# pkmtum/generative-physics-informed-pde

Measured on AMD Instinct MI355X. Metric: ELBO training-step samples/sec (64x64 grids), higher is better.
Workload: dtype f32; 1 GPU; BASELINE config 2/3: c64 grid, B_u=256 unlabeled + N_s=32 labeled per GPU, ROM 8x8, fused native step; global_batch=288, grid=64, parallelism=dp1, graph=True, graph_mode=streams, steps_per_replay=4, world=1, bn=replica

## Files before the change

generative-physics-informed-pde_amd/csrc/conv.hip:

```cpp
#include "common.h"
#include <stdlib.h>
#include <stdio.h>
#include <algorithm>
#include <string.h>
#include <string>
#include <utility>
#include <vector>
#include <atomic>
#include <mutex>

using namespace gpi;

#pragma clang fp contract(on)

namespace {

constexpr int HALO = 4;

__device__ __attribute__((aligned(256))) float g_zero_page[64];

struct Div {
    uint32_t m, one;
};

Div mkdiv(int d) {
    Div v;
    v.one = d == 1;
    v.m = d == 1 ? 0u : (uint32_t)(((1ull << 32) + (uint64_t)d - 1) / (uint64_t)d);
    return v;
}

__device__ __forceinline__ int dq(int e, Div v) { return v.one ? e : (int)__umulhi((uint32_t)e, v.m); }

#ifdef GPI_PHASE_TIMING
__device__ __attribute__((visibility("hidden"))) unsigned long long g_phase[4096 * 16];
__device__ __attribute__((visibility("hidden"))) unsigned long long g_rt[4096 * 2];
#define PHASE(i)                                                                                     \
    do {                                                                                             \
        if (threadIdx.x == 0) g_phase[(blockIdx.x & 4095) * 16 + (i)] = __builtin_amdgcn_s_memtime(); \
    } while (0)
#define RTSTAMP(i)                                                                                 \
    do {                                                                                           \
        if (threadIdx.x == 0) {                                                                    \
            g_rt[(blockIdx.x & 4095) * 2 + (i)] = __builtin_amdgcn_s_memrealtime();                \
            if ((i) == 0)                                                                          \
                g_phase[(blockIdx.x & 4095) * 16 + 15] =                                           \
                    (unsigned long long)__builtin_amdgcn_s_getreg((31 << 11) | 4) |                \
                    ((unsigned long long)__builtin_amdgcn_s_getreg((31 << 11) | 20) << 32);        \
        }                                                                                          \
    } while (0)
#else
#define PHASE(i) \
    do {         \
    } while (0)
#define RTSTAMP(i) \
    do {           \
    } while (0)
#endif

__host__ __device__ inline int fdiv2(int x) { return x >= 0 ? x / 2 : -((-x + 1) / 2); }
__host__ __device__ inline int cdiv2(int x) { return -fdiv2(-x); }
__host__ __device__ inline int pad256(int n) { return (n + 255) & ~255; }

#ifndef GPI_FWD_WAVE_ATOMICS
#define GPI_FWD_WAVE_ATOMICS 0
#endif
#ifndef GPI_FWD_WVGPR
#define GPI_FWD_WVGPR 1
#endif

struct ConvGeom {
    int th, tiles, nblocks;
    int rh, P;
    int gh, PG;
    int ph;
    const float* zero;
    int zreg;
    int npx;
    int cg;
    int fuse;
    int vsum;
    int vshift;
    int ucls;
    int lsum;
    int split;
    int xcd;
    int grid;
    int nfull, half_b, htiles;
    struct Alt {
        int th, rh, gh, ph, zreg, in_sq, in_sr, in_sc, g_sq, g_sr, g_sc;
        Div d_in4, d_g4, d_tp;
    } ha;
    int alt;
    uint32_t* sig;
    const int64_t* sig_epoch;
    int in_sq, in_sr, in_sc;
    int g_sq, g_sr, g_sc;
    Div d_in4, d_P4, d_g4, d_PG4, d_cin, d_cout, d_win, d_tp, d_wout, d_w2;
#ifdef GPI_PHASE_TIMING
    int dbg;
#endif
};

#ifdef GPI_PHASE_TIMING
#define SKIP(G, bit) (((G).dbg & (bit)) != 0)
#else
#define SKIP(G, bit) false
#endif

__host__ __device__ inline void in_rows(int k, int s, int up, int pad, int o0, int t, int& i0, int& len) {
    if (up) {
        i0 = fdiv2(o0 - pad);
        len = fdiv2(o0 + t - 1 - pad + k - 1) - i0 + 1;
    } else {
        i0 = o0 * s - pad;
        len = (t - 1) * s + k;
    }
}

__host__ __device__ inline void g_rows(int k, int s, int pad, int o0, int t, int& g0, int& len) {
    if (s == 2) {
        g0 = cdiv2(2 * o0 + pad - k + 1);
        len = fdiv2(2 * o0 + 2 * t - 1 + pad) - g0 + 1;
    } else {
        g0 = o0 + pad - (k - 1);
        len = t + k - 1;
    }
}

__host__ __device__ inline void owned_rows(int s, int up, int o0, int t, int& p0, int& len) {
    if (up) { p0 = o0 / 2; len = t / 2; }
    else if (s == 2) { p0 = 2 * o0; len = 2 * t; }
    else { p0 = o0; len = t; }
}

constexpr int ZREG = 3;

int env_int(const char* name, int dflt) {
    const char* v = getenv(name);
    return v && *v ? atoi(v) : dflt;
}


bool conv_geom(const gpi_conv_desc& d, const gpi_groups& g, ConvGeom& G, bool fwd, bool fuse = false) {
    if (g.n_groups < 1 || g.n_groups > GPI_MAX_GROUPS) return false;
    if (d.cin < 1 || d.cin > GPI_MAX_CIN || d.cout < 1 || d.cout > GPI_MAX_COUT) return false;
    if (d.k != 1 && d.k != 3 && d.k != 5 && d.k != 7) return false;
    if (d.pad > HALO || (d.w_in & 3) || (d.w_out & 3) || d.w_out > 256) return false;
    if (d.upsample) {
        if (d.stride != 1 || d.h_out != 2 * d.h_in || d.w_out != 2 * d.w_in || d.pad != d.k / 2) return false;
    } else if (d.stride == 2) {
        if (d.h_in != 2 * d.h_out || d.w_in != 2 * d.w_out || d.pad != d.k / 2) return false;
    } else if (d.stride == 1) {
        if (d.h_in != d.h_out || d.w_in != d.w_out || d.pad != d.k / 2) return false;
    } else {
        return false;
    }
    const int B = g.start[g.n_groups] - g.start[0];
    if (g.start[0] != 0 || B <= 0) return false;
    static const int t_fwd = env_int("GPI_TILE_FWD", 512), t_fwd64 = env_int("GPI_TILE_FWD64", 1024),
                     t_bwd = env_int("GPI_TILE_BWD", 512), t_s2 = env_int("GPI_TILE_S2", 128),
                     t_s2brows = env_int("GPI_TILE_S2BROWS", 4), t_s2c1 = env_int("GPI_TILE_S2C1", 512),
                     t_bwdup = env_int("GPI_TILE_BWDUP", 1024), t_bwdrows = env_int("GPI_TILE_BWDROWS", 8),
                     t_fwdrows = env_int("GPI_TILE_FWDROWS", 8), t_fuse = env_int("GPI_TILE_FUSE", 1024);
    static const int t_fwdup32 = env_int("GPI_TILE_FWDUP32", 16), t_bwdups = env_int("GPI_TILE_BWDUPS", 16),
                     t_bwd32k3 = env_int("GPI_TILE_BWD32K3", 16), t_s2c1f = env_int("GPI_TILE_S2C1F", 512),
                     t_fwdwide = env_int("GPI_TILE_FWDWIDE", 8);
    const int target =
        d.stride == 2 ? (d.cin == 1 ? (fwd ? t_s2c1f : t_s2c1) : (fwd ? t_s2 : t_s2brows * d.w_out))
        : fwd ? (d.w_out >= 64 ? t_fwd64
                               : (d.w_out >= 32 ? (d.upsample && d.w_out == 32 ? t_fwdup32
                                                   : (d.k == 3 && d.cin >= 10 && d.w_out == 32 ? t_fwdwide : t_fwdrows)) * d.w_out
                                                : t_fwd))
              : (d.upsample ? (d.w_out >= 32 ? t_bwdup / 64 * min(d.w_out, 64) : t_bwdups * d.w_out)
                            : (d.w_out >= 64 ? t_bwd
                                             : (d.w_out == 32 && d.k == 3 && d.cin <= 8 ? t_bwd32k3 : t_bwdrows) * d.w_out));
    const bool loss_bwd = !fwd && (d.epilogue == GPI_EPI_GAUSS_LOSS || d.epilogue == GPI_EPI_GAUSS_EXP_LOSS);
    G.th = (loss_bwd ? t_fuse : target) / d.w_out;
    if (G.th < 1) G.th = 1;
    if (G.th > d.h_out) G.th = d.h_out;
    if (fwd && d.stride == 1 && !d.upsample) {
        for (;;) {
            int y0, rh;
            in_rows(d.k, 1, 0, d.pad, 0, G.th, y0, rh);
            const int half = G.th / 2;
            if (4 * d.cin * rh * (d.w_in + 2 * HALO) <= 28 * 1024 || half < 1 || d.h_out % half) break;
            G.th = half;
        }
    }
    if (d.upsample && G.th < 2) G.th = 2;
    while (d.h_out % G.th) --G.th;
    if (d.upsample && (G.th & 1)) return false;
    G.tiles = d.h_out / G.th;
    G.nblocks = B * G.tiles;
    int i0;
    in_rows(d.k, d.stride, d.upsample, d.pad, 0, G.th, i0, G.rh);
    if (d.upsample) G.rh += 1;
    if (fuse) G.rh += d.k - 1;
    G.P = d.w_in + 2 * HALO;
    g_rows(d.k, d.stride, d.pad, 0, G.th, i0, G.gh);
    G.PG = d.w_out + 2 * HALO;
    owned_rows(d.stride, d.upsample, 0, G.th, i0, G.ph);
    const uint64_t lim = 1ull << 32;
    const uint64_t in4 = (uint64_t)G.rh * G.P / 4, g4 = (uint64_t)G.gh * G.PG / 4;
    const uint64_t ein = in4 * d.cin, eg = g4 * d.cout, eo = (uint64_t)G.ph * d.w_in;
    if (ein * in4 >= lim || in4 * (G.P / 4) >= lim || eg * g4 >= lim || g4 * (G.PG / 4) >= lim ||
        eo * d.w_in >= lim || 256ull * G.th * d.w_out >= lim)
        return false;
    G.zero = nullptr;
    static const int npx_cap = env_int("GPI_FWD_NPX", 4);
    G.npx = 1;
    if (fwd) {
        const int tp = G.th * d.w_out;
        while (2 * G.npx <= npx_cap && tp >= 256 * 2 * G.npx && d.w_out % (2 * G.npx) == 0) G.npx *= 2;
    }
    G.cg = 1;
    if (fwd && G.npx == 1 && d.epilogue != GPI_EPI_GAUSS_LOSS && d.epilogue != GPI_EPI_GAUSS_EXP_LOSS) {
        static const int cg_on = env_int("GPI_FWD_CG", 1);
        const int tp = G.th * d.w_out;
        if (cg_on && tp <= 128 && 256 % tp == 0 && !d.upsample && d.k <= 3) G.cg = std::min(256 / tp, d.cin);
    }
    G.zreg = (!fwd && d.gout_mode == 0 && (int64_t)d.cout * G.gh * (G.PG / 4) <= (int64_t)ZREG * 256) ? 1 : 0;
    G.split = 0;
    G.fuse = fuse ? 1 : 0;
    G.lsum = 0;
    G.vsum = 0;
    {
        static const int vshift = env_int("GPI_VWG_SHIFT", 1);
        G.vshift = (!fwd && vshift && d.k == 7 && d.stride == 2 && d.cin == 1 && d.cout <= 8) ? 1 : 0;
        static const int ucls = env_int("GPI_UP_ROWCLS", 1);
        G.ucls = (!fwd && ucls && d.upsample && d.k == 3 && d.pad == 1 && (2 * d.cin + 15) / 16 < (3 * d.cin + 15) / 16)
                     ? 1 : 0;
    }
    G.xcd = 0;
    G.alt = 0;
    G.grid = 0;
    G.sig = nullptr;
    G.sig_epoch = nullptr;
#ifdef GPI_PHASE_TIMING
    static const int dbg = env_int("GPI_DBG_SKIP", 0);
    G.dbg = dbg;
#endif
    {
        const int P4 = G.P / 4, pl = G.rh * P4, Q4 = G.PG / 4, gl = G.gh * Q4;
        G.in_sq = 256 / pl;
        G.in_sr = (256 % pl) / P4;
        G.in_sc = (256 % pl) % P4;
        G.g_sq = 256 / gl;
        G.g_sr = (256 % gl) / Q4;
        G.g_sc = (256 % gl) % Q4;
    }
    G.d_in4 = mkdiv((int)in4);
    G.d_P4 = mkdiv(G.P / 4);
    G.d_g4 = mkdiv((int)g4);
    G.d_PG4 = mkdiv(G.PG / 4);
    G.d_cin = mkdiv(d.cin);
    G.d_cout = mkdiv(d.cout);
    G.d_win = mkdiv(d.w_in);
    G.d_tp = mkdiv(G.th * d.w_out);
    G.d_wout = mkdiv(d.w_out);
    G.d_w2 = mkdiv(d.w_in >= 2 ? d.w_in / 2 : 1);
    G.nfull = G.nblocks;
    G.half_b = B;
    G.htiles = 0;
    G.ha = ConvGeom::Alt{G.th, G.rh, G.gh, G.ph, G.zreg, G.in_sq, G.in_sr, G.in_sc, G.g_sq, G.g_sr, G.g_sc,
                         G.d_in4, G.d_g4, G.d_tp};
    static const int half_tiles = env_int("GPI_HALF_TILES", 2);
    const int tot = B * G.tiles, base = tot & ~255;
    static const int half_fwd = env_int("GPI_HALF_FWD", 1);
    if (half_tiles && (fwd ? half_fwd && half_tiles > 1 && G.cg == 1 : (half_tiles > 1 || loss_bwd)) &&
        (G.th & 1) == 0 && base > 0 && tot != base && tot <= 5 * 256 && base % G.tiles == 0) {
        ConvGeom::Alt& a = G.ha;
        a.th = G.th / 2;
        int y0;
        in_rows(d.k, d.stride, d.upsample, d.pad, 0, a.th, y0, a.rh);
        if (d.upsample) a.rh += 1;
        if (fuse) a.rh += d.k - 1;
        g_rows(d.k, d.stride, d.pad, 0, a.th, y0, a.gh);
        owned_rows(d.stride, d.upsample, 0, a.th, y0, a.ph);
        a.zreg = (!fwd && d.gout_mode == 0 && (int64_t)d.cout * a.gh * (G.PG / 4) <= (int64_t)ZREG * 256) ? 1 : 0;
        const int P4 = G.P / 4, pl = a.rh * P4, Q4 = G.PG / 4, gq = a.gh * Q4;
        a.in_sq = 256 / pl;
        a.in_sr = (256 % pl) / P4;
        a.in_sc = (256 % pl) % P4;
        a.g_sq = 256 / gq;
        a.g_sr = (256 % gq) / Q4;
        a.g_sc = (256 % gq) % Q4;
        a.d_in4 = mkdiv(pl);
        a.d_g4 = mkdiv(gq);
        a.d_tp = mkdiv(a.th * d.w_out);
        const bool ok = d.gin_off < 0 || (((a.ph * d.w_in) & 15) == 0 && (d.stride != 2 || (a.ph & 1) == 0));
        if (!ok) a = ConvGeom::Alt{G.th, G.rh, G.gh, G.ph, G.zreg, G.in_sq, G.in_sr, G.in_sc, G.g_sq, G.g_sr, G.g_sc,
                                   G.d_in4, G.d_g4, G.d_tp};
        else {
        G.half_b = base / G.tiles;
        G.nfull = base;
        G.htiles = 2 * G.tiles;
        G.nblocks = base + (B - G.half_b) * G.htiles;
        }
    }
    return true;
}

#define SHAPE_D(X) X(k) X(stride) X(pad) X(upsample) X(cin) X(cout) X(h_in) X(w_in) X(h_out) X(w_out) \
    X(in_bn) X(gout_mode) X(epilogue) X(gin_accumulate)
#define SHAPE_G(X) X(th) X(tiles) X(rh) X(P) X(gh) X(PG) X(ph) X(zreg) X(npx) X(cg) X(fuse) X(vsum) X(vshift) \
    X(ucls) X(lsum) X(split) X(xcd) X(alt) X(in_sq) X(in_sr) X(in_sc) X(g_sq) X(g_sr) X(g_sc)
#define SHAPE_GD(X) X(d_in4) X(d_P4) X(d_g4) X(d_PG4) X(d_cin) X(d_cout) X(d_win) X(d_tp) X(d_wout) X(d_w2)
#define SHAPE_A(X) X(th) X(rh) X(gh) X(ph) X(zreg) X(in_sq) X(in_sr) X(in_sc) X(g_sq) X(g_sr) X(g_sc)
#define SHAPE_AD(X) X(d_in4) X(d_g4) X(d_tp)

struct ShapeC {
    int fwd, fusek, half, exf, v3, cp, npxk, upk, has_gin, drop, wout, ext_in;
#define F(n) int D_##n;
    SHAPE_D(F)
#undef F
#define F(n) int G_##n;
    SHAPE_G(F)
#undef F
#define F(n) int M_##n, O_##n;
    SHAPE_GD(F)
#undef F
#define F(n) int A_##n;
    SHAPE_A(F)
#undef F
#define F(n) int AM_##n, AO_##n;
    SHAPE_AD(F)
#undef F
};

#if defined(GPI_SHAPES_FILE)
#include GPI_SHAPES_FILE
#elif __has_include("conv_shapes.h")
#include "conv_shapes.h"
#endif
#ifndef GPI_CONV_SHAPE_LIST
#define GPI_CONV_SHAPE_LIST
#define GPI_CONV_SHAPE_COUNT 0
#endif
constexpr ShapeC kShapes[GPI_CONV_SHAPE_COUNT + 1] = {GPI_CONV_SHAPE_LIST ShapeC{}};
constexpr int kNumShapes = GPI_CONV_SHAPE_COUNT;
#ifndef GPI_CONV_SHAPE_BOUNDS
#define GPI_CONV_SHAPE_BOUNDS {0, GPI_CONV_SHAPE_COUNT, GPI_CONV_SHAPE_COUNT, GPI_CONV_SHAPE_COUNT, GPI_CONV_SHAPE_COUNT}
#endif
constexpr int kBounds[5] = GPI_CONV_SHAPE_BOUNDS;
#ifndef GPI_CONV_SHAPE_PART
#define GPI_CONV_SHAPE_PART 0
#endif

#ifndef GPI_FUSE_FOLD
#define GPI_FUSE_FOLD 6
#endif

template <int SHP>
__device__ __forceinline__ void fold_shape(gpi_conv_desc& d, ConvGeom& G) {
    if constexpr (SHP >= 0) {
        constexpr ShapeC s = kShapes[SHP];
        constexpr int fm = s.fusek ? GPI_FUSE_FOLD : 7;
        if constexpr (fm & 1) {
#define F(n) d.n = s.D_##n;
        SHAPE_D(F)
#undef F
        }
        if constexpr (fm & 2) {
#define F(n) G.n = s.G_##n;
        SHAPE_G(F)
#undef F
#define F(n) G.ha.n = s.A_##n;
        SHAPE_A(F)
#undef F
        }
        if constexpr (fm & 4) {
#define F(n) G.n = Div{(uint32_t)s.M_##n, (uint32_t)s.O_##n};
        SHAPE_GD(F)
#undef F
#define F(n) G.ha.n = Div{(uint32_t)s.AM_##n, (uint32_t)s.AO_##n};
        SHAPE_AD(F)
#undef F
        }
        if constexpr (s.has_gin) __builtin_assume(d.gin_off >= 0); else d.gin_off = -1;
        if constexpr (s.drop) __builtin_assume(d.drop_off >= 0); else d.drop_off = -1;
        if constexpr (s.wout) __builtin_assume(d.wpart_off >= 0); else d.wpart_off = -1;
        if constexpr (s.ext_in) d.in_off = -1; else __builtin_assume(d.in_off >= 0);
        if constexpr (!s.half) G.nfull = 0x7fffffff;
    }
}

__device__ __forceinline__ void glds4(const float* g, float* lds_wave_base) {
    __builtin_amdgcn_global_load_lds((const __attribute__((address_space(1))) void*)g,
                                     (__attribute__((address_space(3))) void*)lds_wave_base, 4, 0, 0);
}

__device__ __forceinline__ void glds16(const float* g, float* lds_wave_base) {
    __builtin_amdgcn_global_load_lds((const __attribute__((address_space(1))) void*)g,
                                     (__attribute__((address_space(3))) void*)lds_wave_base, 16, 0, 0);
}

template <typename Src>
__device__ __forceinline__ void stage(float* dst, int total, const float* zero, Src src) {
    const int wb = threadIdx.x & ~63;
    for (int e0 = 0; e0 < total; e0 += 256) {
        if (e0 + wb < total) {
            const int e = e0 + (int)threadIdx.x;
            const float* p = e < total ? src(e) : nullptr;
            glds4(p ? p : zero, dst + e0 + wb);
        }
    }
}

#ifndef GPI_STAGE_SEL
#define GPI_STAGE_SEL 1
#endif
struct ChunkIter {
    int q, r, c4;
    __device__ __forceinline__ void init(int e, int plane4, int P4, Div d_q4, Div d_p4) {
        q = dq(e, d_q4);
        const int rem = e - q * plane4;
        r = dq(rem, d_p4);
        c4 = rem - r * P4;
    }
    __device__ __forceinline__ void step(int sq, int sr, int sc, int P4, int nr) {
        c4 += sc;
        if (c4 >= P4) { c4 -= P4; ++r; }
        r += sr;
        if (r >= nr) { r -= nr; ++q; }
        q += sq;
    }
};

constexpr int IMG_MARGIN4 = 16;
__host__ __device__ inline int img_floats(int nq, int nr, int P) { return pad256(4 * (nq * nr * (P / 4) + IMG_MARGIN4)); }

template <typename Plane>
__device__ __forceinline__ void stage_img(float* dst, int nq, int nr, int P, Div d_q4, Div d_p4, int sq, int sr,
                                          int sc, int r0, int h, int w, const float* zero, Plane plane) {
    const int P4 = P >> 2, plane4 = nr * P4, total = nq * plane4 + IMG_MARGIN4;
    const int wb = threadIdx.x & ~63;
    const int c4lo = HALO / 4, c4hi = HALO / 4 + w / 4;
    ChunkIter it;
    it.init(threadIdx.x, plane4, P4, d_q4, d_p4);
    for (int e0 = 0; e0 < total; e0 += 256) {
        if (e0 + wb < total) {
            const int row = r0 + it.r;
            const bool ok = it.q < nq && row >= 0 && row < h && it.c4 >= c4lo && it.c4 < c4hi;
#if GPI_STAGE_SEL
            const float* pv = plane(it.q) + row * w + 4 * (it.c4 - c4lo);
            asm volatile("" : "+v"(pv));
            const float* p = ok ? pv : zero;
#else
            const float* p = ok ? plane(it.q) + row * w + 4 * (it.c4 - c4lo) : zero;
#endif
            glds16(p, dst + 4 * (e0 + wb));
        }
        it.step(sq, sr, sc, P4, nr);
    }
}

constexpr int STAT_HALF = GPI_REPLICAS / 2;
struct StatLoad {
    double v[STAT_HALF];
    double* out;
};

__device__ __forceinline__ void stat_issue(const gpi_stat* stats, int64_t n_stats, int grp, int64_t sa, int na,
                                           double* da, int64_t sb, int nb, double* db, const float* zero, StatLoad& L) {
    const int t = threadIdx.x, k = t & 3, h = (t >> 2) & 1, ch = t >> 3;
    const double* p = (const double*)zero;
    int64_t step = 0;
    L.out = nullptr;
    const int64_t rstride = n_stats * GPI_MAX_GROUPS * 4;
    const gpi_stat* sg = stats + (int64_t)grp * n_stats;
    if (ch < na) {
        p = &sg[sa + ch].sum + k + h * STAT_HALF * rstride;
        step = rstride;
        L.out = da + 4 * ch + k;
    } else if (ch - na < nb) {
        p = &sg[sb + ch - na].sum + k + h * STAT_HALF * rstride;
        step = rstride;
        L.out = db + 4 * (ch - na) + k;
    }
    const auto g = (const __attribute__((address_space(1))) double*)p;
#pragma unroll
    for (int r = 0; r < STAT_HALF; ++r) L.v[r] = g[r * step];
}

__device__ __forceinline__ void stat_finish(StatLoad& L) {
    double s0 = 0.0, s1 = 0.0;
#pragma unroll
    for (int r = 0; r < STAT_HALF; r += 2) {
        s0 += L.v[r];
        s1 += L.v[r + 1];
    }
    double s = s0 + s1;
    s += __shfl_xor(s, 4, 64);
    if (L.out && !(threadIdx.x & 4)) *L.out = s;
}

__device__ __forceinline__ gpi_stat* stat_slot(const gpi_codec_ctx& c, int64_t stat, int grp) {
    const int r = blockIdx.x % GPI_REPLICAS;
    return c.stats + ((int64_t)r * GPI_MAX_GROUPS + grp) * c.n_stats + stat;
}

__device__ __forceinline__ void mean_invstd(const double* s4, double n, float eps, float& mean, float& invstd) {
    const double m = s4[0] / n;
    double var = fma(-m, m, s4[1] / n);
    if (var < 0.0) var = 0.0;
    mean = (float)m;
    invstd = (float)(1.0 / sqrt(var + (double)eps));
}

template <int CP>
__device__ __forceinline__ void fma_vec(float (&acc)[CP], const float* w, float v) {
    if constexpr (CP % 4 == 0) {
#pragma unroll
        for (int q = 0; q < CP / 4; ++q) {
            const float4 w4 = reinterpret_cast<const float4*>(w)[q];
            acc[4 * q + 0] = fmaf(w4.x, v, acc[4 * q + 0]);
            acc[4 * q + 1] = fmaf(w4.y, v, acc[4 * q + 1]);
            acc[4 * q + 2] = fmaf(w4.z, v, acc[4 * q + 2]);
            acc[4 * q + 3] = fmaf(w4.w, v, acc[4 * q + 3]);
        }
    } else {
#pragma unroll
        for (int q = 0; q < CP / 2; ++q) {
            const float2 w2 = reinterpret_cast<const float2*>(w)[q];
            acc[2 * q + 0] = fmaf(w2.x, v, acc[2 * q + 0]);
            acc[2 * q + 1] = fmaf(w2.y, v, acc[2 * q + 1]);
        }
    }
}

template <typename T>
__device__ __forceinline__ T pin(T v) {
    asm volatile("" : "+s"(v));
    return v;
}

typedef float f32x4 __attribute__((ext_vector_type(4)));
typedef float f32x2 __attribute__((ext_vector_type(2)));

template <int NBYTES>
__device__ __forceinline__ void touch_kernargs() {
    const __attribute__((address_space(4))) uint32_t* ka =
        (const __attribute__((address_space(4))) uint32_t*)__builtin_amdgcn_kernarg_segment_ptr();
    constexpr int NL = (NBYTES + 63) / 64;
    uint32_t x[NL];
#pragma unroll
    for (int i = 0; i < NL; ++i) x[i] = ka[16 * i];
#pragma unroll
    for (int i = 0; i < NL; ++i) asm volatile("" : : "s"(x[i]));
}
constexpr int CONV_KARG_BYTES = (int)(sizeof(gpi_conv_desc) + sizeof(gpi_codec_ctx) + sizeof(ConvGeom) + 16);

__device__ __forceinline__ void entry_signal(const ConvGeom& G) {
    if (G.sig && blockIdx.x == 0 && threadIdx.x == 0)
        __hip_atomic_fetch_add(G.sig, 1u, __ATOMIC_RELAXED, __HIP_MEMORY_SCOPE_AGENT);
}

template <typename T>
__device__ __forceinline__ const __attribute__((address_space(1))) T* as_gld(const T* p) {
    return (const __attribute__((address_space(1))) T*)p;
}
template <typename T>
__device__ __forceinline__ __attribute__((address_space(1))) T* as_gst(T* p) {
    return (__attribute__((address_space(1))) T*)p;
}

struct TileIdx {
    int b, oy0, grp, gsz;
};

__device__ __forceinline__ int logical_block(const ConvGeom& G) {
    const int b = blockIdx.x;
    if (!G.xcd) return b;
    const int q = G.grid >> 3, r = G.grid & 7, x = b & 7;
    return x * q + min(x, r) + (b >> 3);
}

__device__ __forceinline__ TileIdx tile_of(const ConvGeom& G, const gpi_groups& g, int tile = -1) {
    if (tile < 0) tile = logical_block(G);
    TileIdx t;
    if (tile < G.nfull) {
        t.b = tile / G.tiles;
        t.oy0 = (tile - t.b * G.tiles) * G.th;
    } else {
        const int u = tile - G.nfull, q = u / G.htiles;
        t.b = G.half_b + q;
        t.oy0 = (u - q * G.htiles) * G.ha.th;
    }
    t.grp = group_of(g, t.b);
    t.gsz = karg_sel(g.start, t.grp + 1) - karg_sel(g.start, t.grp);
    return t;
}

__device__ __forceinline__ const float* input_base(const gpi_conv_desc& d, const gpi_codec_ctx& c, int b) {
    const int HWi = d.h_in * d.w_in;
    if (d.in_off >= 0) return c.ws + d.in_off + ((int64_t)b * d.in_ctot + d.in_c0) * HWi;
    return c.ext_in + (int64_t)(c.ext_idx ? c.ext_idx[b] : b) * c.ext_stride + (int64_t)d.in_c0 * HWi;
}

__device__ __forceinline__ void activate_img(float* img, const ConvGeom& G, const gpi_conv_desc& d, int iy0,
                                             const float* sc, const float* sh) {
    const int P4 = G.P >> 2, plane4 = G.rh * P4, total = d.cin * plane4;
    const int c4lo = HALO / 4, c4hi = HALO / 4 + d.w_in / 4;
    float4* im4 = reinterpret_cast<float4*>(img);
    ChunkIter it;
    it.init(threadIdx.x, plane4, P4, G.d_in4, G.d_P4);
    for (int e0 = threadIdx.x; e0 < total; e0 += 512) {
        float4 v[2];
        bool ok[2];
        int ci[2];
#pragma unroll
        for (int u = 0; u < 2; ++u) {
            const int row = iy0 + it.r;
            ok[u] = e0 + 256 * u < total && row >= 0 && row < d.h_in && it.c4 >= c4lo && it.c4 < c4hi;
            ci[u] = it.q;
            if (ok[u]) v[u] = im4[e0 + 256 * u];
            it.step(G.in_sq, G.in_sr, G.in_sc, P4, G.rh);
        }
#pragma unroll
        for (int u = 0; u < 2; ++u) {
            if (ok[u]) {
                const float a = sc[ci[u]], b = sh[ci[u]];
                float4 o;
                o.x = fmaxf(fmaf(v[u].x, a, b), 0.f);
                o.y = fmaxf(fmaf(v[u].y, a, b), 0.f);
                o.z = fmaxf(fmaf(v[u].z, a, b), 0.f);
                o.w = fmaxf(fmaf(v[u].w, a, b), 0.f);
                im4[e0 + 256 * u] = o;
            }
        }
    }
}

template <int NW, int OFF>
__device__ __forceinline__ void lds_window(const float* p, float (&win)[NW]) {
    constexpr int NCH = (OFF + NW + 3) / 4;
    const float4* q = reinterpret_cast<const float4*>(p - OFF);
    float buf[4 * NCH];
#pragma unroll
    for (int c = 0; c < NCH; ++c) {
        const float4 v = q[c];
        buf[4 * c] = v.x;
        buf[4 * c + 1] = v.y;
        buf[4 * c + 2] = v.z;
        buf[4 * c + 3] = v.w;
    }
#pragma unroll
    for (int t = 0; t < NW; ++t) win[t] = buf[OFF + t];
}

#ifndef GPI_PLAIN_STORES
__device__ __forceinline__ void st2(float* p, f32x2 v) {
    __hip_atomic_store((__attribute__((address_space(1))) uint64_t*)p, __builtin_bit_cast(uint64_t, v),
                       __ATOMIC_RELAXED, __HIP_MEMORY_SCOPE_AGENT);
}
__device__ __forceinline__ void st4(float* p, f32x4 v) {
    asm volatile("global_store_dwordx4 %0, %1, off sc1\n\ts_nop 1" : : "v"(p), "v"(v));
}
__device__ __forceinline__ void st1(float* p, float v) {
    __hip_atomic_store((__attribute__((address_space(1))) float*)p, v, __ATOMIC_RELAXED, __HIP_MEMORY_SCOPE_AGENT);
}
#else
__device__ __forceinline__ void st4(float* p, f32x4 v) { *as_gst((f32x4*)p) = v; }
__device__ __forceinline__ void st2(float* p, f32x2 v) { *as_gst((f32x2*)p) = v; }
__device__ __forceinline__ void st1(float* p, float v) { *as_gst(p) = v; }
#endif

template <int NPX>
__device__ __forceinline__ void store_px(float* p, const float (&v)[NPX]) {
    if constexpr (NPX == 4) {
        st4(p, f32x4{v[0], v[1], v[2], v[3]});
    } else if constexpr (NPX == 2) {
        st2(p, f32x2{v[0], v[1]});
    } else {
#pragma unroll
        for (int q = 0; q < NPX; ++q) st1(p + q, v[q]);
    }
}

constexpr int FWD_HDR = 8 * GPI_MAX_CIN + 2 * GPI_MAX_CIN + 64 + 16 + 8;

template <int K, int S, int UP, int CP, int NPX, bool HALF = false, int SHP = -1>
__global__ __launch_bounds__(256) __attribute__((amdgpu_waves_per_eu(NPX == 0 ? 1 : 5))) void conv_fwd_kernel(gpi_conv_desc d, gpi_codec_ctx c, ConvGeom G) {
    fold_shape<SHP>(d, G);
    touch_kernargs<CONV_KARG_BYTES>();
    entry_signal(G);
    if (SKIP(G, 16)) return;
    ConvGeom Gt_;
    if constexpr (HALF) {
        Gt_ = G;
        if (logical_block(G) >= G.nfull) {
            const ConvGeom::Alt& a = G.ha;
            Gt_.th = a.th; Gt_.rh = a.rh; Gt_.in_sq = a.in_sq; Gt_.in_sr = a.in_sr; Gt_.in_sc = a.in_sc;
            Gt_.d_in4 = a.d_in4; Gt_.d_tp = a.d_tp;
        }
    }
    const ConvGeom& Gt = HALF ? Gt_ : G;
    constexpr int KK = K * K;
    extern __shared__ __attribute__((aligned(16))) float smem[];
    double* gst = (double*)smem;
    float* sc = smem + 8 * GPI_MAX_CIN;
    float* sh = sc + GPI_MAX_CIN;
    float* scratch = sh + GPI_MAX_CIN;
    float* red = scratch + 64;
    float* dsl = red + 16;
    float* wT = smem + pad256(FWD_HDR);
    const int nw = d.cin * KK * CP;
    float* img = wT + pad256(nw);

    const int tid = threadIdx.x;
    RTSTAMP(0);
    PHASE(0);
    float* const ws = pin(c.ws);
    const float* const params = pin(c.params);
    const float* const zero = pin(Gt.zero);
    const int64_t w_off = pin(d.w_off);
    const TileIdx T = tile_of(Gt, c.groups);
    const int HWi = d.h_in * d.w_in, HWo = d.h_out * d.w_out;
    const float* ib = input_base(d, c, T.b);
    const bool drop = d.drop_off >= 0;
    PHASE(1);

    stage(wT, nw, zero, [&](int e) -> const float* {
        const int co = e % CP, r = e / CP;
        return co < d.cout ? params + w_off + (int64_t)co * d.cin * KK + r : nullptr;
    });
    int iy0, rh_;
    in_rows(K, S, UP, d.pad, T.oy0, Gt.th, iy0, rh_);
    stage_img(img, d.cin, Gt.rh, Gt.P, Gt.d_in4, Gt.d_P4, Gt.in_sq, Gt.in_sr, Gt.in_sc, iy0, d.h_in, d.w_in, zero,
              [&](int q) -> const float* { return ib + (int64_t)q * HWi; });
    float dsv = 1.f;
    if (drop && tid >= 64 && tid < 64 + d.cout) dsv = *as_gld(ws + d.drop_off + (int64_t)T.b * d.cout + (tid - 64));
    if (d.in_bn) {
        float gam = 0.f, bet = 0.f;
        if (tid < d.cin) {
            gam = *as_gld(params + d.gamma_off + tid);
            bet = *as_gld(params + d.beta_off + tid);
        }
        StatLoad L;
        stat_issue(c.stats, c.n_stats, T.grp, d.in_stat, d.cin, gst, 0, 0, nullptr, zero, L);
        stat_finish(L);
        __syncthreads();
        if (SKIP(G, 8) || SKIP(G, 32)) return;
        PHASE(2);
        if (tid < d.cin) {
            float mean, inv;
            mean_invstd(gst + 4 * tid, (double)T.gsz * HWi, c.bn_eps, mean, inv);
            sc[tid] = gam * inv;
            sh[tid] = fmaf(-(mean * gam), inv, bet);
        }
        __syncthreads();
        activate_img(img, Gt, d, iy0, sc, sh);
    }
    if (drop && tid >= 64 && tid < 64 + d.cout) dsl[tid - 64] = dsv;
    __syncthreads();
    PHASE(4);

    const int tp = Gt.th * d.w_out;
    float Lv = 0.f;
    float vst[2 * CP];
#pragma unroll
    for (int q = 0; q < 2 * CP; ++q) vst[q] = 0.f;
    const bool gauss = d.epilogue == GPI_EPI_GAUSS_LOSS || d.epilogue == GPI_EPI_GAUSS_EXP_LOSS;
    if constexpr (NPX > 1) {
        constexpr int PADK = K / 2;
        constexpr int NW = UP ? ((NPX - 1 + K - 1 + (PADK & 1)) >> 1) + 1 : (NPX - 1) * S + K;
        const int ng = tp / NPX;
        for (int gbase = 0; gbase < ng; gbase += 256) {
            const int g = gbase + tid;
            const bool active = g < ng;
            const int ty = dq(g * NPX, Gt.d_wout), x0 = g * NPX - ty * d.w_out;
            const int oy = T.oy0 + ty;
            float acc[NPX][CP];
#pragma unroll
            for (int p = 0; p < NPX; ++p)
#pragma unroll
                for (int co = 0; co < CP; ++co) acc[p][co] = 0.f;
            if (active && !SKIP(G, 64)) {
                const int plane = Gt.rh * Gt.P;
                const int cb = UP ? fdiv2(x0 - PADK) + HALO : x0 * S - PADK + HALO;
                for (int ci = 0; ci < d.cin; ++ci) {
                    const float* tci = img + ci * plane + cb;
                    const float* wci = wT + ci * KK * CP;
#pragma unroll
                    for (int ky = 0; ky < K; ++ky) {
                        const int ry = UP ? (fdiv2(oy - PADK + ky) - iy0) : (ty * S + ky);
                        const float* trow = tci + ry * Gt.P;
                        float win[NW];
                        if constexpr (!UP && (NPX * S) % 4 == 0) {
                            lds_window<NW, (HALO - PADK) & 3>(trow, win);
                        } else {
#pragma unroll
                            for (int t = 0; t < NW; ++t) win[t] = trow[t];
                        }
#pragma unroll
                        for (int kx = 0; kx < K; ++kx) {
                            float wv[CP];
                            const float* wp = wci + (ky * K + kx) * CP;
                            if constexpr (CP % 4 == 0) {
#pragma unroll
                                for (int q = 0; q < CP / 4; ++q) {
                                    const float4 w4 = reinterpret_cast<const float4*>(wp)[q];
                                    wv[4 * q] = w4.x;
                                    wv[4 * q + 1] = w4.y;
                                    wv[4 * q + 2] = w4.z;
                                    wv[4 * q + 3] = w4.w;
                                }
                            } else {
#pragma unroll
                                for (int q = 0; q < CP / 2; ++q) {
                                    const float2 w2 = reinterpret_cast<const float2*>(wp)[q];
                                    wv[2 * q] = w2.x;
                                    wv[2 * q + 1] = w2.y;
                                }
                            }
#pragma unroll
                            for (int p = 0; p < NPX; ++p) {
                                const float v = win[UP ? ((p + kx + (PADK & 1)) >> 1) : p * S + kx];
#pragma unroll
                                for (int co = 0; co < CP; ++co) acc[p][co] = fmaf(wv[co], v, acc[p][co]);
                            }
                        }
                    }
                }
            }
            if (drop) {
#pragma unroll
                for (int co = 0; co < CP; ++co) {
                    const float ds = co < d.cout ? dsl[co] : 1.f;
#pragma unroll
                    for (int p = 0; p < NPX; ++p) acc[p][co] *= ds;
                }
            }
            const int64_t pix0 = (int64_t)oy * d.w_out + x0;
            if (gauss) {
                if (active) {
                    int row = T.b - karg_sel(c.groups.start, T.grp);
                    if (const int32_t* ti = karg_sel(c.tgt_idx, T.grp)) row = ti[row];
                    const float* tg = karg_sel(c.tgt, T.grp) + (int64_t)row * HWo + pix0;
                    const bool ex = d.epilogue == GPI_EPI_GAUSS_EXP_LOSS;
                    const float scl = karg_sel(c.loss_scale, T.grp);
                    float g0[NPX], g1[NPX];
#pragma unroll
                    for (int p = 0; p < NPX; ++p) {
                        const float tgt = tg[p];
                        const float mu = acc[p][0], ls = acc[p][1];
                        const float e = expf(-2.f * ls);
                        const float emu = ex ? expf(mu) : 1.f;
                        const float r = ex ? expf(tgt) - emu : tgt - mu;
                        Lv += -0.5f * (2.f * ls + r * r * e + GPI_LOG2PI);
                        g0[p] = -scl * r * e * emu;
                        g1[p] = scl * (1.f - r * r * e);
                    }
                    float* go = ws + d.gout_off + (int64_t)T.b * 2 * HWo + pix0;
                    store_px<NPX>(go, g0);
                    store_px<NPX>(go + HWo, g1);
                    if (d.out_off >= 0) {
                        float m0[NPX], m1[NPX];
#pragma unroll
                        for (int p = 0; p < NPX; ++p) {
                            m0[p] = acc[p][0];
                            m1[p] = acc[p][1];
                        }
                        float* o = ws + d.out_off + ((int64_t)T.b * d.out_ctot + d.out_c0) * HWo + pix0;
                        store_px<NPX>(o, m0);
                        store_px<NPX>(o + HWo, m1);
                    }
                }
                continue;
            }
            if (active) {
                float* o = ws + d.out_off + ((int64_t)T.b * d.out_ctot + d.out_c0) * HWo + pix0;
#pragma unroll
                for (int co = 0; co < CP; ++co) {
                    if (co < d.cout) {
                        float v[NPX];
#pragma unroll
                        for (int p = 0; p < NPX; ++p) v[p] = acc[p][co];
                        store_px<NPX>(o + (int64_t)co * HWo, v);
                    }
                }
            }
            if (d.epilogue == GPI_EPI_STORE_STATS) {
#pragma unroll
                for (int co = 0; co < CP; ++co) {
#pragma unroll
                    for (int p = 0; p < NPX; ++p) {
                        const float a = (active && co < d.cout) ? acc[p][co] : 0.f;
                        vst[2 * co] += a;
                        vst[2 * co + 1] += a * a;
                    }
                }
            }
        }
    } else {
        const int cg = NPX == 0 ? Gt.cg : 1;
        for (int pbase = 0; pbase < tp; pbase += 256) {
            const int grp = NPX == 0 ? dq(tid, Gt.d_tp) : 0;
            const int pix = NPX == 0 ? tid - grp * tp : pbase + tid;
            const int ty = dq(pix, Gt.d_wout), tx = pix - ty * d.w_out;
            const int oy = T.oy0 + ty, ox = tx;
            bool active = pix < tp && grp < cg;
            float tgt = 0.f;
            if (gauss && active) {
                int row = T.b - karg_sel(c.groups.start, T.grp);
                if (const int32_t* ti = karg_sel(c.tgt_idx, T.grp)) row = ti[row];
                tgt = karg_sel(c.tgt, T.grp)[(int64_t)row * HWo + oy * d.w_out + ox];
            }
            PHASE(5);
            float acc[CP];
    #pragma unroll
            for (int co = 0; co < CP; ++co) acc[co] = 0.f;
            if (active && !SKIP(G, 64)) {
                const int plane = Gt.rh * Gt.P;
                for (int ci = grp; ci < d.cin; ci += cg) {
                    const float* tci = img + ci * plane;
                    int wofs = pad256(FWD_HDR) + ci * KK * CP;
                    if (GPI_FWD_WVGPR) asm volatile("" : "+v"(wofs));
                    const float* wci = smem + wofs;
    #pragma unroll
                    for (int ky = 0; ky < K; ++ky) {
                        const int ry = UP ? (fdiv2(oy - d.pad + ky) - iy0) : (ty * S + ky);
                        const float* trow = tci + ry * Gt.P;
    #pragma unroll
                        for (int kx = 0; kx < K; ++kx) {
                            const int col = UP ? fdiv2(ox - d.pad + kx) + HALO : ox * S - d.pad + kx + HALO;
                            fma_vec<CP>(acc, wci + (ky * K + kx) * CP, trow[col]);
                        }
                    }
                }
            }
            if (NPX == 0 && cg > 1) {
                float* part = img + img_floats(d.cin, Gt.rh, Gt.P);
                if (active && grp > 0) {
    #pragma unroll
                    for (int co = 0; co < CP; ++co) part[((grp - 1) * tp + pix) * CP + co] = acc[co];
                }
                __syncthreads();
                if (active && grp == 0) {
                    for (int g = 1; g < cg; ++g) {
    #pragma unroll
                        for (int co = 0; co < CP; ++co) acc[co] += part[((g - 1) * tp + pix) * CP + co];
                    }
                }
                active = active && grp == 0;
            }
            PHASE(6);
            if (drop) {
    #pragma unroll
                for (int co = 0; co < CP; ++co)
                    if (co < d.cout) acc[co] *= dsl[co];
            }
            if (gauss) {
                if (active) {
                    const float mu = acc[0], ls = acc[1];
                    const float e = expf(-2.f * ls);
                    const bool ex = d.epilogue == GPI_EPI_GAUSS_EXP_LOSS;
                    const float emu = ex ? expf(mu) : 1.f;
                    const float r = ex ? expf(tgt) - emu : tgt - mu;
                    Lv += -0.5f * (2.f * ls + r * r * e + GPI_LOG2PI);
                    const float scl = karg_sel(c.loss_scale, T.grp);
                    auto go = as_gst(ws + d.gout_off + (int64_t)T.b * 2 * HWo + oy * d.w_out + ox);
                    go[0] = -scl * r * e * emu;
                    go[HWo] = scl * (1.f - r * r * e);
                    if (d.out_off >= 0) {
                        auto o = as_gst(ws + d.out_off + (int64_t)T.b * d.out_ctot * HWo + (int64_t)d.out_c0 * HWo +
                                     oy * d.w_out + ox);
                        o[0] = mu;
                        o[HWo] = ls;
                    }
                }
                continue;
            }
            if (active) {
                float* o = ws + d.out_off + ((int64_t)T.b * d.out_ctot + d.out_c0) * HWo + oy * d.w_out + ox;
    #pragma unroll
                for (int co = 0; co < CP; ++co)
                    if (co < d.cout) st1(o + (int64_t)co * HWo, acc[co]);
            }
            if (d.epilogue == GPI_EPI_STORE_STATS) {
    #pragma unroll
                for (int co = 0; co < CP; ++co) {
                    const float a = (active && co < d.cout) ? acc[co] : 0.f;
                    vst[2 * co] += a;
                    vst[2 * co + 1] += a * a;
                }
            }
        }
    }

    if (d.epilogue == GPI_EPI_GAUSS_LOSS || d.epilogue == GPI_EPI_GAUSS_EXP_LOSS) {
        float v[1] = {Lv};
        block_sum<1>(v, scratch, red);
        if (tid == 0 && !SKIP(G, 4)) atomicAdd(c.loss_acc + T.grp * GPI_REPLICAS + blockIdx.x % GPI_REPLICAS, (double)red[0]);
        PHASE(7);
        RTSTAMP(1);
        return;
    }
    if (d.epilogue == GPI_EPI_STORE_STATS && !SKIP(G, 128)) {
#if GPI_FWD_WAVE_ATOMICS
        wave_sums(vst);
        const int lane = tid & 63;
        if (lane < 2 * d.cout && !SKIP(G, 4)) {
            float v = vst[0];
#pragma unroll
            for (int q = 1; q < 2 * CP; ++q) v = lane == q ? vst[q] : v;
            gpi_stat* st = c.stats + ((int64_t)((4 * blockIdx.x + (tid >> 6)) % GPI_REPLICAS) * GPI_MAX_GROUPS + T.grp) *
                                         c.n_stats + d.out_stat + (lane >> 1);
            atomicAdd((lane & 1) ? &st->sumsq : &st->sum, (double)v);
        }
#else
        block_sum<2 * CP>(vst, scratch, red);
        if (tid < 2 * d.cout && !SKIP(G, 4)) {
            gpi_stat* st = stat_slot(c, d.out_stat + (tid >> 1), T.grp);
            atomicAdd((tid & 1) ? &st->sumsq : &st->sum, (double)red[tid]);
        }
#endif
    }
    PHASE(7);
    RTSTAMP(1);
}

__device__ __forceinline__ f32x4 mfma4(float a, float b, f32x4 c) {
    return __builtin_amdgcn_mfma_f32_16x16x4f32(a, b, c, 0, 0, 0);
}

__host__ __device__ inline int pad64(int n) { return (n + 63) & ~63; }
__host__ __device__ inline int bwd_hdr(int cin, int cout) { return pad64(8 * (cin + cout) + 5 * cin + 5 * cout); }
__host__ __device__ inline bool vop_op(const gpi_conv_desc& d) {
    return d.k == 5 && d.stride == 1 && !d.upsample && d.gin_off >= 0 && d.cin <= 4 && d.cout <= 2;
}
__host__ __device__ inline int bwd_rowlen(const gpi_conv_desc& d) {
    return d.cout * d.cin * d.k * d.k + (d.in_bn ? 2 * d.cin : 0);
}
__host__ __device__ inline int vop_mid_floats(int gh, int w_out, int rowlen, bool fuse);
template <bool B>
struct BoolC {
    static constexpr bool value = B;
};

template <int V>
struct IntC {
    static constexpr int value = V;
};

#ifndef GPI_IG_PRE
#define GPI_IG_PRE 0
#endif
#ifndef GPI_IG_PAIR
#define GPI_IG_PAIR 0
#endif
#ifndef GPI_S2_IG_SERIAL
#define GPI_S2_IG_SERIAL 0
#endif
#ifndef GPI_VDG3
#define GPI_VDG3 0
#endif
#ifndef GPI_BWD_WAVES
#define GPI_BWD_WAVES 6
#endif
#ifndef GPI_BWD3_WAVES
#define GPI_BWD3_WAVES 4
#endif
constexpr int SLAB_ROWS = 4;
__host__ __device__ inline int vop_mid_floats(int gh, int w_out, int rowlen, bool fuse) {
    return pad256(512 + SLAB_ROWS * rowlen);
}

#ifndef GPI_FUSE_WAVES
#define GPI_FUSE_WAVES 5
#endif
#ifndef GPI_FUSE_SHP_WAVES
#define GPI_FUSE_SHP_WAVES 5
#endif
#ifndef GPI_FUSE_WLDS
#define GPI_FUSE_WLDS 5
#endif
#ifndef GPI_VDG_WLDS
#define GPI_VDG_WLDS 1
#endif
__host__ __device__ constexpr bool fuse_wlds(int ky) {
    return GPI_FUSE_WLDS <= 0 ? false : (GPI_FUSE_WLDS >= 5 ? true : (ky & 1 ? (ky / 2) < GPI_FUSE_WLDS : (ky / 2) < GPI_FUSE_WLDS - 2));
}

template <int K, int S, int UP, bool FUSE = false, bool HALF = false, bool V3 = false, bool EXF = false, int SHP = -1>
__global__ __launch_bounds__(256) __attribute__((amdgpu_waves_per_eu(K == 5 ? (FUSE ? (SHP >= 0 ? GPI_FUSE_SHP_WAVES : GPI_FUSE_WAVES) : 4) : (V3 ? GPI_BWD3_WAVES : GPI_BWD_WAVES)))) void conv_bwd_kernel(gpi_conv_desc d, gpi_codec_ctx c, ConvGeom G) {
    fold_shape<SHP>(d, G);
    touch_kernargs<CONV_KARG_BYTES>();
    entry_signal(G);
    if (SKIP(G, 16)) return;
    ConvGeom Gt_;
    if constexpr (HALF) {
        const int lb0 = logical_block(G);
        const bool wgr0 = G.split && (G.xcd ? (lb0 & 1) != 0 : lb0 >= G.nblocks);
        const int tile0 = !G.split ? lb0 : (G.xcd ? lb0 >> 1 : (wgr0 ? lb0 - G.nblocks : lb0));
        Gt_ = G;
        if (tile0 >= G.nfull) {
            const ConvGeom::Alt& a = G.ha;
            Gt_.th = a.th; Gt_.rh = a.rh; Gt_.gh = a.gh; Gt_.ph = a.ph; Gt_.zreg = a.zreg;
            Gt_.in_sq = a.in_sq; Gt_.in_sr = a.in_sr; Gt_.in_sc = a.in_sc;
            Gt_.g_sq = a.g_sq; Gt_.g_sr = a.g_sr; Gt_.g_sc = a.g_sc;
            Gt_.d_in4 = a.d_in4; Gt_.d_g4 = a.d_g4; Gt_.d_tp = a.d_tp;
        }
    }
    const ConvGeom& Gt = HALF ? Gt_ : G;
    constexpr int KK = K * K;
    extern __shared__ __attribute__((aligned(16))) float smem[];
    double* gst = (double*)smem;
    float* i_sc = smem + 8 * (d.cin + d.cout);
    float* i_sh = i_sc + d.cin;
    float* i_mean = i_sh + d.cin;
    float* i_inv = i_mean + d.cin;
    float* i_gam = i_inv + d.cin;
    float* o_coef = i_gam + d.cin;
    float* o_drop = o_coef + 4 * d.cout;
    const bool has_gin = d.gin_off >= 0;
    const bool obn = d.gout_mode == 0;
    const int KD = d.cout * KK;
    const int KD4 = (KD + 3) & ~3;
    const bool vop = FUSE || (K == 5 && S == 1 && !UP && has_gin && d.cin <= 4 && d.cout <= 2);
    const bool v3 = V3 && K == 3 && S == 1 && !UP && !FUSE && has_gin && d.cin <= 8 && Gt.ph * d.w_in >= 256;
    const int CIV3 = (d.cin + 3) & ~3;
    const int J = d.cin * KK;
    const int rowlen = d.cout * J + (d.in_bn ? 2 * d.cin : 0);
    float* wD = smem + bwd_hdr(d.cin, d.cout);
    const int nwd = (has_gin && !vop) ? KD4 * 16 : 0;
    float* const mid = wD;
    const int nmid = vop ? vop_mid_floats(Gt.gh, d.w_out, rowlen, FUSE) : 0;
    int* ktab = (int*)(wD + pad256(nwd) + nmid);
    float* gl = (float*)ktab + ((has_gin && !vop) ? pad256((S == 2 ? 8 : 1) * KD4) : 0);
    const int gplane = Gt.gh * Gt.PG;
    const int gimg = img_floats(d.cout, Gt.gh, Gt.PG);
    const bool zreg = Gt.zreg != 0;
    float* gz = gl + gimg;
    float* al = gz + ((obn && !zreg) ? gimg : 0);
    float* const alb = FUSE ? al + (K / 2) * Gt.P : al;
    float* red = vop ? mid + 256 : (float*)ktab;

    const int tid = threadIdx.x;
    const int lane = tid & 63, wv = tid >> 6, kq = lane >> 4, l16 = lane & 15;
    RTSTAMP(0);
    PHASE(0);
    float* const ws = pin(c.ws);
    const float* const params = pin(c.params);
    const float* const zero = pin(Gt.zero);
    const int64_t w_off = pin(d.w_off), gout_off = pin(d.gout_off), out_off = pin(d.out_off);
    const int64_t gin_off = pin(d.gin_off);
    const int lb = logical_block(G);
    const bool wg_role = Gt.split && (Gt.xcd ? (lb & 1) != 0 : lb >= Gt.nblocks);
    const bool dg_role = !wg_role;
    const bool wout = d.wpart_off >= 0;
    const bool do_wgrad = (!Gt.split || wg_role) && wout;
    const int tile = !Gt.split ? lb : (Gt.xcd ? lb >> 1 : (wg_role ? lb - Gt.nblocks : lb));
    const TileIdx T = tile_of(Gt, c.groups, tile);
    const int HWi = d.h_in * d.w_in, HWo = d.h_out * d.w_out;
    const float* ib = input_base(d, c, T.b);
    PHASE(1);

    if constexpr (FUSE) {
        float4* g4 = reinterpret_cast<float4*>(gl);
        for (int e = tid; e < gimg / 4; e += 256) g4[e] = float4{0.f, 0.f, 0.f, 0.f};
    }
    const int CIV = d.cin <= 2 ? 2 : 4;
    if (vop) {
        stage(mid, d.cout * KK * CIV, zero, [&](int e) -> const float* {
            const int ci = e % CIV, t = e / CIV, co = t / KK, tap = t - co * KK;
            return ci < d.cin ? params + w_off + ((int64_t)co * d.cin + ci) * KK + tap : nullptr;
        });
        if (FUSE)
            stage(mid + 256, d.cin * KK * 2, zero, [&](int e) -> const float* {
                const int co = e & 1, t = e >> 1, ci = t / KK, r = t - ci * KK, kx = r / K, ky = r - kx * K;
                return params + w_off + ((int64_t)co * d.cin + ci) * KK + ky * K + kx;
            });
    }
    if (has_gin && dg_role && v3)
        stage(wD, d.cout * KK * CIV3, zero, [&](int e) -> const float* {
            const int t = e / CIV3, ci = e - t * CIV3, co = t / KK, tap = t - co * KK;
            return ci < d.cin ? params + w_off + ((int64_t)co * d.cin + ci) * KK + tap : nullptr;
        });
    else if (has_gin && dg_role && !vop)
        stage(wD, nwd, zero, [&](int e) -> const float* {
            const int ci = e & 15, k = e >> 4;
            const int co = k / KK, t = k - co * KK;
            return ci < d.cin && k < KD ? params + w_off + ((int64_t)co * d.cin + ci) * KK + t : nullptr;
        });
    PHASE(12);
    int gy0, gh_;
    g_rows(K, S, d.pad, T.oy0, Gt.th, gy0, gh_);
    const int64_t gbase = ((int64_t)T.b * d.out_ctot + d.out_c0) * HWo;
    constexpr int RPF = 5;
    float tv0[FUSE ? RPF : 1];
    const float* tg = zero;
    if constexpr (FUSE) {
        int trow0 = T.b - karg_sel(c.groups.start, T.grp);
        if (const int32_t* ti = karg_sel(c.tgt_idx, T.grp)) trow0 = ti[trow0];
        tg = karg_sel(c.tgt, T.grp) + (int64_t)trow0 * HWo;
        const int nitem = ((Gt.gh + RPF - 1) / RPF) * d.w_out;
        const int rg = dq(tid, Gt.d_wout), x = tid - rg * d.w_out;
#pragma unroll
        for (int p = 0; p < RPF; ++p) {
            const int oy = gy0 + rg * RPF + p;
            const bool ok = tid < nitem && rg * RPF + p < Gt.gh && oy >= 0 && oy < d.h_out;
            tv0[p] = *as_gld(ok ? tg + oy * d.w_out + x : zero);
        }
    } else {
        stage_img(gl, d.cout, Gt.gh, Gt.PG, Gt.d_g4, Gt.d_PG4, Gt.g_sq, Gt.g_sr, Gt.g_sc, gy0, d.h_out, d.w_out, zero,
                  [&](int q) -> const float* { return ws + gout_off + gbase + (int64_t)q * HWo; });
    }
    PHASE(13);
    f32x4 zr[ZREG];
    if (obn && zreg) {
        const int P4 = Gt.PG >> 2, plane4 = Gt.gh * P4, total = d.cout * plane4;
        const int c4lo = HALO / 4, c4hi = HALO / 4 + d.w_out / 4;
        ChunkIter it;
        it.init(tid, plane4, P4, Gt.d_g4, Gt.d_PG4);
#pragma unroll
        for (int u = 0; u < ZREG; ++u) {
            const int row = gy0 + it.r;
            const bool ok = tid + 256 * u < total && row >= 0 && row < d.h_out && it.c4 >= c4lo && it.c4 < c4hi;
            const float* src = ok ? ws + out_off + gbase + (int64_t)it.q * HWo + row * d.w_out + 4 * (it.c4 - c4lo)
                                  : zero;
            zr[u] = *as_gld((const f32x4*)src);
            it.step(Gt.g_sq, Gt.g_sr, Gt.g_sc, P4, Gt.gh);
        }
    } else if (obn) {
        stage_img(gz, d.cout, Gt.gh, Gt.PG, Gt.d_g4, Gt.d_PG4, Gt.g_sq, Gt.g_sr, Gt.g_sc, gy0, d.h_out, d.w_out, zero,
                  [&](int q) -> const float* { return ws + out_off + gbase + (int64_t)q * HWo; });
    }
    PHASE(14);
    int iy0, rh_;
    in_rows(K, S, UP, d.pad, T.oy0, Gt.th, iy0, rh_);
    const int iyA = FUSE ? iy0 - K / 2 : iy0;
    stage_img(al, d.cin, Gt.rh, Gt.P, Gt.d_in4, Gt.d_P4, Gt.in_sq, Gt.in_sr, Gt.in_sc, iyA, d.h_in, d.w_in, zero,
              [&](int q) -> const float* { return ib + (int64_t)q * HWi; });
    PHASE(8);
    int py0, ph_;
    owned_rows(S, UP, T.oy0, Gt.th, py0, ph_);
    const bool vdg = vop && dg_role;
    const int nmblk = (!FUSE && has_gin && dg_role && !vdg && !v3 && !SKIP(G, 2)) ? (Gt.ph * d.w_in) >> 4 : 0;
    const int ci_l = min(l16, d.cin - 1);
    const bool cok = l16 < d.cin;
    const int64_t ibase = ((int64_t)T.b * d.in_ctot + d.in_c0 + ci_l) * HWi + (int64_t)py0 * d.w_in;
    f32x4 pv4[4];
#if GPI_IG_PRE
    f32x4 pv4b[4];
#endif
    auto own_load = [&](int round, f32x4 (&dst)[4]) {
#pragma unroll
        for (int u = 0; u < 4; ++u) {
            const int m = wv + 4 * (4 * round + u);
            const bool ok = m < nmblk && cok;
            const int64_t o = ibase + 16 * m + 4 * kq;
            if (d.gin_accumulate) dst[u] = *as_gld((const f32x4*)(ok ? ws + gin_off + o : zero));
            else dst[u] = f32x4{0.f, 0.f, 0.f, 0.f};
        }
    };
    float pv3[8][2];
    if (v3 && dg_role && d.gin_accumulate && !SKIP(G, 2)) {
        const int Q = Gt.ph * d.w_in >= 512 ? 2 : 1;
        const int gq = tid;
        const int qy = dq(Q * gq, Gt.d_win), px0 = Q * gq - qy * d.w_in;
        const bool iok = gq < (Gt.ph * d.w_in) / Q;
        const int64_t gb_in = ((int64_t)T.b * d.in_ctot + d.in_c0) * HWi + (int64_t)(py0 + qy) * d.w_in + px0;
#pragma unroll
        for (int ci = 0; ci < 8; ++ci) {
            const bool ok = iok && ci < d.cin;
            const float* pp = ok ? ws + gin_off + gb_in + (int64_t)ci * HWi : zero;
            pv3[ci][0] = *as_gld(pp);
            pv3[ci][1] = *as_gld(ok && Q == 2 ? pp + 1 : zero);
        }
    }
    if (nmblk > 0 && S != 2) {
        own_load(0, pv4);
#if GPI_IG_PRE
        if (nmblk > 16) own_load(1, pv4b);
#endif
    }
    PHASE(9);
    float gam = 0.f, bet = 0.f;
    if (d.in_bn && tid < d.cin) {
        gam = *as_gld(params + d.gamma_off + tid);
        bet = *as_gld(params + d.beta_off + tid);
    }
    const bool drop = d.drop_off >= 0;
    float odv = 1.f;
    if (drop && tid >= 128 && tid < 128 + d.cout) odv = *as_gld(ws + d.drop_off + (int64_t)T.b * d.cout + (tid - 128));
    {
        StatLoad L;
        stat_issue(c.stats, c.n_stats, T.grp, d.in_stat, d.in_bn ? d.cin : 0, gst, d.out_stat, obn ? d.cout : 0,
                   gst + 4 * d.cin, zero, L);
        PHASE(10);
        stat_finish(L);
        PHASE(11);
    }
    if (tid >= 128 && tid < 128 + d.cout) o_drop[tid - 128] = odv;
    __syncthreads();
    if (SKIP(G, 8)) return;
    PHASE(2);

    if (tid < d.cin && d.in_bn) {
        float mean, inv;
        mean_invstd(gst + 4 * tid, (double)T.gsz * HWi, c.bn_eps, mean, inv);
// ... 620 lines not shown
                for (int ci = 0; ci < CI; ++ci) s1[ci] = s2[ci] = 0.f;
                const int npq = (Gt.ph * d.w_in) / Q;
                for (int gq = tid; gq < npq; gq += 256) {
                    const int qy = dq(Q * gq, Gt.d_win), px0 = Q * gq - qy * d.w_in;
                    const int64_t gb_in = ((int64_t)T.b * d.in_ctot + d.in_c0) * HWi + (int64_t)(py0 + qy) * d.w_in + px0;
                    float pv[CI][Q];
                    if (gq == tid) {
#pragma unroll
                        for (int ci = 0; ci < CI; ++ci)
#pragma unroll
                            for (int q = 0; q < Q; ++q) pv[ci][q] = d.gin_accumulate ? pv3[ci][q] : 0.f;
                    } else {
#pragma unroll
                        for (int ci = 0; ci < CI; ++ci) {
                            const bool ok = ci < d.cin && d.gin_accumulate;
                            const float* pp = ok ? ws + gin_off + gb_in + (int64_t)ci * HWi : zero;
#pragma unroll
                            for (int q = 0; q < Q; ++q) pv[ci][q] = as_gld(pp)[ok ? q : 0];
                        }
                    }
                    f32x2 acc2[CH][Q];
#pragma unroll
                    for (int h = 0; h < CH; ++h)
#pragma unroll
                        for (int q = 0; q < Q; ++q) acc2[h][q] = f32x2{0.f, 0.f};
                    for (int co = 0; co < d.cout; ++co) {
#pragma unroll
                        for (int ky = 0; ky < K; ++ky) {
                            const float* grow = gl + co * gplane + (qy + py0 + d.pad - ky - gy0) * Gt.PG + HALO + px0 +
                                                d.pad - (K - 1);
                            float gw[K + Q - 1];
#pragma unroll
                            for (int t = 0; t < K + Q - 1; ++t) gw[t] = grow[t];
                            const float* wrow = wD + (co * K + ky) * K * CI;
#pragma unroll
                            for (int kx = 0; kx < K; ++kx) {
                                f32x4 w4[CI / 4];
#pragma unroll
                                for (int v = 0; v < CI / 4; ++v) w4[v] = *reinterpret_cast<const f32x4*>(wrow + kx * CI + 4 * v);
#pragma unroll
                                for (int q = 0; q < Q; ++q) {
                                    const float gv = gw[q + K - 1 - kx];
#pragma unroll
                                    for (int h = 0; h < CH; ++h) {
                                        const f32x2 w = f32x2{w4[h >> 1][2 * (h & 1)], w4[h >> 1][2 * (h & 1) + 1]};
                                        acc2[h][q] = __builtin_elementwise_fma(w, f32x2{gv, gv}, acc2[h][q]);
                                    }
                                }
                            }
                        }
                    }
#pragma unroll
                    for (int ci = 0; ci < CI; ++ci) {
                        if (ci >= d.cin) break;
                        const float* ap = alb + (ci * Gt.rh + (py0 - iy0 + qy)) * Gt.P + HALO + px0;
                        const float lg = d.in_bn ? i_gam[ci] : 0.f;
                        const float lb = d.in_bn ? i_sh[ci] + i_mean[ci] * i_sc[ci] : 0.f;
                        const float lr = d.in_bn ? 1.f / lg : 0.f;
                        float o[Q];
#pragma unroll
                        for (int q = 0; q < Q; ++q) {
                            const float a = acc2[ci >> 1][q][ci & 1];
                            if (d.in_bn) {
                                const float av = ap[q];
                                const float dbn = av > 0.f ? a : 0.f;
                                o[q] = pv[ci][q] + lg * dbn;
                                s1[ci] += dbn;
                                s2[ci] += dbn * ((av - lb) * lr);
                            } else {
                                o[q] = pv[ci][q] + a;
                            }
                        }
                        store_px<Q>(ws + gin_off + gb_in + (int64_t)ci * HWi, o);
                    }
                }
                if (d.in_bn) {
                    float v2[2 * CI];
#pragma unroll
                    for (int ci = 0; ci < CI; ++ci) {
                        v2[ci] = s1[ci];
                        v2[CI + ci] = s2[ci];
                    }
                    wave_sums(v2);
                    float a = 0.f, b = 0.f;
#pragma unroll
                    for (int ci = 0; ci < CI; ++ci) {
                        a = l16 == ci ? v2[ci] : a;
                        b = l16 == ci ? v2[CI + ci] : b;
                    }
                    sd = kq == 0 ? a : 0.f;
                    sdx = kq == 0 ? b : 0.f;
                }
            };
            const bool q2 = Gt.ph * d.w_in >= 512;
            if (d.cin <= 4) { if (q2) v3_rows(IntC<4>{}, IntC<2>{}); else v3_rows(IntC<4>{}, IntC<1>{}); }
            else if (d.cin <= 8) { if (q2) v3_rows(IntC<8>{}, IntC<2>{}); else v3_rows(IntC<8>{}, IntC<1>{}); }

        }
    }
#endif
    float vsd[4] = {0.f, 0.f, 0.f, 0.f}, vsdx[4] = {0.f, 0.f, 0.f, 0.f};
    if (vdg && !SKIP(G, 2)) {
        float lg[4], lb[4], lr[4];
#pragma unroll
        for (int ci = 0; ci < 4; ++ci) {
            const int cc = min(ci, d.cin - 1);
            lg[ci] = d.in_bn ? i_gam[cc] : 0.f;
            lb[ci] = d.in_bn ? i_sh[cc] + i_mean[cc] * i_sc[cc] : 0.f;
            lr[ci] = d.in_bn ? 1.f / lg[ci] : 0.f;
        }
        auto vdg_rows = [&](auto ci_c) {
            constexpr int CI = decltype(ci_c)::value;
            constexpr int CH = CI / 2;
            constexpr int Q = CI == 2 ? 4 : 2;
            constexpr int NWB = (2 * KK * CI + 63) / 64;
            float wb[NWB];
    #pragma unroll
            for (int j = 0; j < NWB; ++j) wb[j] = mid[64 * j + lane];
            const int npq = (Gt.ph * d.w_in) / Q;
            for (int gq = tid; gq < npq; gq += 256) {
                const int qy = dq(Q * gq, Gt.d_win), px0 = Q * gq - qy * d.w_in;
                const int64_t pix = (int64_t)(py0 + qy) * d.w_in + px0;
                const int64_t gbase_in = ((int64_t)T.b * d.in_ctot + d.in_c0) * HWi + pix;
                f32x2 acc2[CH][Q];
    #pragma unroll
                for (int h = 0; h < CH; ++h)
    #pragma unroll
                    for (int q = 0; q < Q; ++q) acc2[h][q] = f32x2{0.f, 0.f};
    #pragma unroll
                for (int co = 0; co < 2; ++co) {
                    if (co >= d.cout) break;
    #pragma unroll
                    for (int ky = 0; ky < K; ++ky) {
                        const float* grow = gl + co * gplane + (qy + py0 + d.pad - ky - gy0) * Gt.PG + HALO + px0 +
                                            d.pad - (K - 1);
                        float gw[K + Q - 1];
                        if constexpr (Q == 4) {
                            lds_window<K + Q - 1, (HALO + K / 2 - (K - 1)) & 3>(grow, gw);
                        } else {
    #pragma unroll
                            for (int t = 0; t < K + Q - 1; ++t) gw[t] = grow[t];
                        }
    #pragma unroll
                        for (int kx = 0; kx < K; ++kx) {
                            f32x2 w[CH];
    #pragma unroll
                            for (int h = 0; h < CH; ++h) {
                                const int i = ((co * K + ky) * K + kx) * CI + 2 * h;
                                if (GPI_VDG_WLDS) {
                                    w[h] = *reinterpret_cast<const f32x2*>(mid + i);
                                } else {
                                    w[h][0] = __int_as_float(__builtin_amdgcn_readlane(__float_as_int(wb[i >> 6]), i & 63));
                                    w[h][1] = __int_as_float(
                                        __builtin_amdgcn_readlane(__float_as_int(wb[(i + 1) >> 6]), (i + 1) & 63));
                                }
                            }
    #pragma unroll
                            for (int q = 0; q < Q; ++q) {
                                const float gv = gw[q + K - 1 - kx];
    #pragma unroll
                                for (int h = 0; h < CH; ++h)
                                    acc2[h][q] = __builtin_elementwise_fma(w[h], f32x2{gv, gv}, acc2[h][q]);
                            }
                        }
                    }
                }
                float acc[CI][Q];
    #pragma unroll
                for (int ci = 0; ci < CI; ++ci)
    #pragma unroll
                    for (int q = 0; q < Q; ++q) acc[ci][q] = acc2[ci >> 1][q][ci & 1];
    #pragma unroll
                for (int ci = 0; ci < CI; ++ci) {
                    if (ci >= d.cin) break;
                    const float* ap = alb + (ci * Gt.rh + (py0 - iy0 + qy)) * Gt.P + HALO + px0;
                    float av[Q], pv[Q], o[Q];
    #pragma unroll
                    for (int q = 0; q < Q; ++q) {
                        av[q] = ap[q];
                        pv[q] = 0.f;
                    }
                    if (d.gin_accumulate) {
                        auto pp = as_gld(ws + gin_off + gbase_in + (int64_t)ci * HWi);
    #pragma unroll
                        for (int q = 0; q < Q; ++q) pv[q] = pp[q];
                    }
    #pragma unroll
                    for (int q = 0; q < Q; ++q) {
                        if (d.in_bn) {
                            const float dbn = av[q] > 0.f ? acc[ci][q] : 0.f;
                            o[q] = pv[q] + lg[ci] * dbn;
                            vsd[ci] += dbn;
                            vsdx[ci] += dbn * ((av[q] - lb[ci]) * lr[ci]);
                        } else {
                            o[q] = pv[q] + acc[ci][q];
                        }
                    }
                    store_px<Q>(ws + gin_off + gbase_in + (int64_t)ci * HWi, o);
                }
            }
        };
        if (d.cin <= 2) vdg_rows(IntC<2>{});
        else vdg_rows(IntC<4>{});
    }
    if (d.in_bn && dg_role) {
        __syncthreads();
        if (vdg) {
            float ws8[8] = {vsd[0], vsd[1], vsd[2], vsd[3], vsdx[0], vsdx[1], vsdx[2], vsdx[3]};
            wave_sums(ws8);
#pragma unroll
            for (int ci = 0; ci < 4; ++ci) {
                const float a = ws8[ci], b = ws8[4 + ci];
                if (lane == 0 && ci < d.cin) {
                    red[wv * 32 + ci] = a;
                    red[128 + wv * 32 + ci] = b;
                    slab[d.cout * J + ci] = b;
                    slab[d.cout * J + d.cin + ci] = a;
                }
            }
        } else {
            if (!v3) {
                sd += __shfl_xor(sd, 16, 64);
                sdx += __shfl_xor(sdx, 16, 64);
                sd += __shfl_xor(sd, 32, 64);
                sdx += __shfl_xor(sdx, 32, 64);
            }
            if (kq == 0) {
                red[wv * 32 + l16] = sd;
                red[128 + wv * 32 + l16] = sdx;
                if (cok && !lsum && wout) {
                    slab[d.cout * J + l16] = sdx;
                    slab[d.cout * J + d.cin + l16] = sd;
                }
            }
        }
        __syncthreads();
        if (tid < d.cin) {
            double s_d = 0.0, s_dx = 0.0;
#pragma unroll
            for (int w = 0; w < 4; ++w) {
                s_d += (double)red[w * 32 + tid];
                s_dx += (double)red[128 + w * 32 + tid];
            }
            gpi_stat* st = stat_slot(c, d.in_stat + tid, T.grp);
            const double gm = i_gam[tid];
            if (!SKIP(G, 4)) {
                atomicAdd(&st->ssum, gm * s_d);
                atomicAdd(&st->sxsum, gm * s_dx);
            }
        }
    }
    if (!vop || wg_late) wgrad_phase();
    PHASE(6);
    if (lsum) {
        __syncthreads();
        const int MI = d.cout * K, NJ = d.cin * K;
        const int nmb = (SKIP(G, 1) || !do_wgrad) ? 0 : (MI + 15) >> 4;
        const bool two = NJ > 16;
        float* lrow = wD + wv * rowlen;
#pragma unroll
        for (int mb = 0; mb < 2; ++mb) {
            if (mb >= nmb) break;
#pragma unroll
            for (int u = 0; u < 2; ++u) {
                if (u == 1 && !two) break;
                const f32x4 a = hold[mb][u];
                const int j2 = 16 * u + l16;
#pragma unroll
                for (int r = 0; r < 4; ++r) {
                    const int i2 = 16 * mb + 4 * kq + r;
                    if (i2 < MI && j2 < NJ) {
                        const int co2 = i2 / K, kx2 = i2 - co2 * K, ci2 = j2 / K, ky2 = j2 - ci2 * K;
                        lrow[co2 * J + ci2 * KK + ky2 * K + kx2] = a[r];
                    }
                }
            }
        }
        if (d.in_bn && dg_role && kq == 0 && cok) {
            lrow[d.cout * J + l16] = sdx;
            lrow[d.cout * J + d.cin + l16] = sd;
        }
        __syncthreads();
        const int c0 = (Gt.split && !do_wgrad) ? d.cout * J : 0;
        const int c1 = !wout ? 0 : ((Gt.split && !dg_role) ? d.cout * J : rowlen);
        float* srow = c.wpart + d.wpart_off + (int64_t)tile * rowlen;
        for (int e = c0 + tid; e < c1; e += 256) {
            const float* r = wD + e;
            srow[e] = (r[0] + r[rowlen]) + (r[2 * rowlen] + r[3 * rowlen]);
        }
    }
    if (vop) {
        __syncthreads();
        float* srow = c.wpart + d.wpart_off + (int64_t)tile * rowlen;
        for (int e = tid; e < (wout ? rowlen : 0); e += 256) {
            const float* r = mid + 512 + e;
            srow[e] = (r[0] + r[rowlen]) + (r[2 * rowlen] + r[3 * rowlen]);
        }
    }
    PHASE(7);
    RTSTAMP(1);
}

size_t fwd_lds(const gpi_conv_desc& d, const ConvGeom& G, int cp) {
    return sizeof(float) * ((size_t)pad256(FWD_HDR) + pad256(d.cin * d.k * d.k * cp) + img_floats(d.cin, G.rh, G.P) +
                            (G.cg > 1 ? (size_t)(G.cg - 1) * G.th * d.w_out * cp : 0));
}

size_t bwd_lds_floats(const gpi_conv_desc& d, int rh, int P, int gh, int PG, int zreg, bool fuse) {
    const int KD4 = (d.cout * d.k * d.k + 3) & ~3;
    const int gimg = img_floats(d.cout, gh, PG);
    const bool zimg = d.gout_mode == 0 && !zreg;
    const size_t mid = vop_op(d) ? vop_mid_floats(gh, d.w_out, bwd_rowlen(d), fuse)
                                 : (d.gin_off >= 0 ? pad256(KD4 * 16) + pad256((d.stride == 2 ? 8 : 1) * KD4) : 0);
    return (size_t)bwd_hdr(d.cin, d.cout) + mid + gimg + (zimg ? gimg : 0) + img_floats(d.cin, rh, P);
}

size_t bwd_lds(const gpi_conv_desc& d, const ConvGeom& G) {
    return sizeof(float) * bwd_lds_floats(d, G.rh, G.P, G.gh, G.PG, G.zreg, G.fuse != 0);
}

bool lsum_op(const gpi_conv_desc& d, const ConvGeom& G) {
    static const int on = env_int("GPI_LSUM", 2);
    if (!on || vop_op(d) || G.fuse) return false;
    if ((on == 2 && d.h_out * d.w_out > 256) || (on == 3 && d.h_out * d.w_out > 64)) return false;
    if (d.k == 7 && d.stride == 2 && !d.upsample && d.cin == 1 && d.gin_off < 0 && d.cout <= 16) return false;
    if (d.cout * d.k > 32 || d.cin * d.k > 32) return false;
    const size_t avail = bwd_lds_floats(d, G.rh, G.P, G.gh, G.PG, G.zreg, false) - bwd_hdr(d.cin, d.cout);
    return avail >= (size_t)4 * bwd_rowlen(d);
}

bool vsum_op(const gpi_conv_desc& d, const ConvGeom& G) {
    static const int on = env_int("GPI_VSUM", 1);
    if (!on || !(d.k == 7 && d.stride == 2 && !d.upsample && d.cin == 1 && d.gin_off < 0 && d.cout <= 16)) return false;
    return (size_t)img_floats(d.cout, G.gh, G.PG) >= (size_t)4 * bwd_rowlen(d);
}

typedef void (*conv_kernel_t)(gpi_conv_desc, gpi_codec_ctx, ConvGeom);

#ifndef GPI_CONV_SHAPE_NOFOLD
#define GPI_CONV_SHAPE_NOFOLD {-1}
#endif
constexpr int kNoFold[] = GPI_CONV_SHAPE_NOFOLD;
constexpr bool no_fold(int i) {
    for (int v : kNoFold)
        if (v == i) return true;
    return false;
}

template <int I>
conv_kernel_t shape_kernel() {
    constexpr ShapeC s = kShapes[I];
    if constexpr ((s.fusek != 0 && GPI_FUSE_FOLD == 0) || no_fold(I)) return nullptr;
    else if constexpr (s.fwd != 0) return conv_fwd_kernel<s.D_k, s.D_stride, s.D_upsample, s.cp, s.npxk, s.half != 0, I>;
    else return conv_bwd_kernel<s.D_k, s.D_stride, s.upk, s.fusek != 0, s.half != 0, s.v3 != 0, s.exf != 0, I>;
}

template <int LO, int... I>
conv_kernel_t shape_kernel_at(int i, std::integer_sequence<int, I...>) {
    static const conv_kernel_t t[] = {shape_kernel<LO + I>()..., nullptr};
    return t[i];
}

}

namespace gpi_conv_parts {
__attribute__((visibility("hidden"))) void* shape_part1(int i);
__attribute__((visibility("hidden"))) void* shape_part2(int i);
__attribute__((visibility("hidden"))) void* shape_part3(int i);
#if GPI_CONV_SHAPE_PART > 0
#define GPI_PART_FN_(p) shape_part##p
#define GPI_PART_FN(p) GPI_PART_FN_(p)
void* GPI_PART_FN(GPI_CONV_SHAPE_PART)(int i) {
    constexpr int lo = kBounds[GPI_CONV_SHAPE_PART], n = kBounds[GPI_CONV_SHAPE_PART + 1] - lo;
    return (void*)shape_kernel_at<lo>(i, std::make_integer_sequence<int, n>{});
}
#endif
}

namespace {
#if GPI_CONV_SHAPE_PART == 0

template <int K, int S, int UP, int NPX, bool HALF>
conv_kernel_t pick_cp_h(int cp) {
    if (cp == 2) return conv_fwd_kernel<K, S, UP, 2, NPX, HALF>;
    if (cp == 4) return conv_fwd_kernel<K, S, UP, 4, NPX, HALF>;
    if (cp == 6) return conv_fwd_kernel<K, S, UP, 6, NPX, HALF>;
    return conv_fwd_kernel<K, S, UP, 8, NPX, HALF>;
}

template <int K, int S, int UP, int NPX>
conv_kernel_t pick_cp(int cp, bool half = false) {
    if constexpr (NPX != 0) {
        if (half) return pick_cp_h<K, S, UP, NPX, true>(cp);
    }
    return pick_cp_h<K, S, UP, NPX, false>(cp);
}

template <int K, int S, int UP>
conv_kernel_t pick(int cp, bool fwd, int npx, bool half, bool ucls = false) {
    if constexpr (UP != 0) {
        if (!fwd && ucls) return half ? conv_bwd_kernel<K, S, 2, false, true> : conv_bwd_kernel<K, S, 2>;
    }
    if constexpr (K == 3 && S == 1 && UP == 0) {
        if (!fwd && ucls) return half ? conv_bwd_kernel<3, 1, 0, false, true, true> : conv_bwd_kernel<3, 1, 0, false, false, true>;
    }
    if (!fwd) return half ? conv_bwd_kernel<K, S, UP, false, true> : conv_bwd_kernel<K, S, UP>;
    if (npx == 4) return pick_cp<K, S, UP, 4>(cp, half);
    if (npx == 2) return pick_cp<K, S, UP, 2>(cp, half);
    if constexpr (!UP && K <= 3) {
        if (npx == 0) return pick_cp<K, S, UP, 0>(cp);
    }
    return pick_cp<K, S, UP, 1>(cp, half);
}

bool v3_op(const gpi_conv_desc& d, const ConvGeom& G) {
    return GPI_VDG3 && d.k == 3 && d.stride == 1 && !d.upsample && d.gin_off >= 0 && d.cin <= 8 && G.ph * d.w_in >= 256;
}

conv_kernel_t select_kernel(const gpi_conv_desc& d, int cp, bool fwd, int npx, bool half, bool ucls) {
    const int key = d.k * 100 + d.stride * 10 + d.upsample;
    switch (key) {
        case 110: return pick<1, 1, 0>(cp, fwd, npx, half);
        case 310: return pick<3, 1, 0>(cp, fwd, npx, half, ucls);
        case 311: return pick<3, 1, 1>(cp, fwd, npx, half, ucls);
        case 320: return pick<3, 2, 0>(cp, fwd, npx, half);
        case 510: return pick<5, 1, 0>(cp, fwd, npx, half);
        case 720: return pick<7, 2, 0>(cp, fwd, npx, half);
        default: return nullptr;
    }
}

int cp_of(const gpi_conv_desc& d) {
    const int cout = d.cout;
    if (cout <= 2) return 2;
    if (cout <= 4) return 4;
    static const int cp6 = env_int("GPI_FWD_CP6", 0);
    const bool wide8 = d.k == 7 || (d.k == 3 && d.stride == 1 && !d.upsample && !cp6);
    return (cout <= 6 && !wide8) ? 6 : 8;
}

bool aligned_ok(const gpi_conv_desc& d, const gpi_codec_ctx& c, bool fwd) {
    if (((uintptr_t)c.ws & 15) || (d.in_off >= 0 && (d.in_off & 3))) return false;
    if (d.in_off < 0 && (((uintptr_t)c.ext_in & 15) || (c.ext_stride & 3))) return false;
    if (fwd) return true;
    if (d.cin > 16) return false;
    if (d.in_bn && (d.in_off < 0 || d.gin_off < 0)) return false;
    if ((d.gout_off & 3) || (d.gout_mode == 0 && (d.out_off & 3))) return false;
    if (d.gin_off >= 0 && (d.gin_off & 3)) return false;
    return true;
}

bool xcd_mode(bool fwd, bool fuse, bool split, bool half) {
    static const int mode = env_int("GPI_XCD_MODE", 9);
    return !half && (mode & (fuse ? 8 : fwd ? 1 : split ? 4 : 2)) != 0;
}

ShapeC shape_of(const gpi_conv_desc& d, const ConvGeom& G, bool fwd, bool fuse, int cp, bool exf) {
    ShapeC s{};
    const bool half = G.nfull < G.nblocks;
    s.fwd = fwd;
    s.fusek = fuse;
    s.has_gin = d.gin_off >= 0;
    s.drop = d.drop_off >= 0;
    s.wout = d.wpart_off >= 0;
    s.ext_in = d.in_off < 0;
    if (fuse) {
        s.half = half;
        s.exf = exf;
        s.upk = 0;
    } else if (!fwd) {
        const bool u = G.ucls != 0 || v3_op(d, G);
        s.half = half;
        s.upk = (d.upsample && u) ? 2 : d.upsample;
        s.v3 = d.k == 3 && d.stride == 1 && !d.upsample && u;
    } else {
        const int npx = G.cg > 1 ? 0 : G.npx;
        s.npxk = (npx == 0 && !(d.upsample == 0 && d.k <= 3)) ? 1 : npx;
        s.half = s.npxk == 0 ? 0 : half;
        s.cp = cp;
    }
#define F(n) s.D_##n = d.n;
    SHAPE_D(F)
#undef F
#define F(n) s.G_##n = G.n;
    SHAPE_G(F)
#undef F
#define F(n) s.M_##n = (int)G.n.m, s.O_##n = (int)G.n.one;
    SHAPE_GD(F)
#undef F
#define F(n) s.A_##n = G.ha.n;
    SHAPE_A(F)
#undef F
#define F(n) s.AM_##n = (int)G.ha.n.m, s.AO_##n = (int)G.ha.n.one;
    SHAPE_AD(F)
#undef F
    return s;
}

conv_kernel_t shape_kernel_any(int i) {
    if (i < 0 || i >= kNumShapes) return nullptr;
    if (i < kBounds[1]) return shape_kernel_at<0>(i, std::make_integer_sequence<int, kBounds[1]>{});
    if (i < kBounds[2]) return (conv_kernel_t)gpi_conv_parts::shape_part1(i - kBounds[1]);
    if (i < kBounds[3]) return (conv_kernel_t)gpi_conv_parts::shape_part2(i - kBounds[2]);
    return (conv_kernel_t)gpi_conv_parts::shape_part3(i - kBounds[3]);
}

std::atomic<int64_t> g_shape_planned{0}, g_shape_matched{0};
std::vector<ShapeC> g_shapes_seen;
std::mutex g_shapes_mu;

int shape_index(const ShapeC& s) {
    for (int i = 0; i < kNumShapes; ++i)
        if (memcmp(&kShapes[i], &s, sizeof(ShapeC)) == 0) return i;
    return -1;
}

int launch(const gpi_conv_desc& d, const gpi_codec_ctx& c, hipStream_t st, bool fwd, bool fuse = false,
           uint32_t* sig = nullptr, const int64_t* sig_epoch = nullptr, bool dry = false) {
    ConvGeom G;
    if (!conv_geom(d, c.groups, G, fwd, fuse)) return GPI_ERR_UNSUPPORTED;
    if (sig && !sig_epoch) return GPI_ERR_ARG;
    G.sig = sig;
    G.sig_epoch = sig_epoch;
    if (fuse && (fwd || d.k != 5 || d.stride != 1 || d.upsample || d.cout != 2 || d.cin > 4 || d.drop_off >= 0 ||
                 d.gout_mode != 1 || d.gin_off < 0 ||
                 (d.epilogue != GPI_EPI_GAUSS_LOSS && d.epilogue != GPI_EPI_GAUSS_EXP_LOSS)))
        return GPI_ERR_UNSUPPORTED;
    if ((d.epilogue == GPI_EPI_GAUSS_LOSS || d.epilogue == GPI_EPI_GAUSS_EXP_LOSS) && d.cout != 2) return GPI_ERR_ARG;
    if (d.in_off < 0 && !c.ext_in) return GPI_ERR_ARG;
    if (!aligned_ok(d, c, fwd)) return GPI_ERR_UNSUPPORTED;
    if (!fwd && d.gin_off >= 0 && ((G.ph * d.w_in) & 15)) return GPI_ERR_UNSUPPORTED;
    if (!fwd && d.gin_off >= 0 && d.stride == 2 && ((d.w_in & 7) || (G.ph & 1))) return GPI_ERR_UNSUPPORTED;
    const int cp = cp_of(d);
    const bool exf = d.epilogue == GPI_EPI_GAUSS_EXP_LOSS;
    conv_kernel_t k = fuse ? (G.nfull < G.nblocks ? (exf ? conv_bwd_kernel<5, 1, 0, true, true, false, true> : conv_bwd_kernel<5, 1, 0, true, true>)
                                                  : (exf ? conv_bwd_kernel<5, 1, 0, true, false, false, true> : conv_bwd_kernel<5, 1, 0, true>))
                           : select_kernel(d, cp, fwd, G.cg > 1 ? 0 : G.npx, G.nfull < G.nblocks,
                                           G.ucls != 0 || (!fwd && v3_op(d, G)));
    if (!k) return GPI_ERR_UNSUPPORTED;
    static const float* zero = nullptr;
    if (!zero && !dry) {
        void* p = nullptr;
        if (hipGetSymbolAddress(&p, HIP_SYMBOL(g_zero_page)) != hipSuccess) return GPI_ERR_LAUNCH;
        zero = (const float*)p;
    }
    G.zero = zero;
    if (!fwd) G.lsum = lsum_op(d, G) ? 1 : 0;
    if (!fwd) G.vsum = vsum_op(d, G) ? 1 : 0;
    const size_t lds = fwd ? fwd_lds(d, G, cp) : bwd_lds(d, G);
    if (lds > 160 * 1024) return GPI_ERR_UNSUPPORTED;
    if (!fwd && d.gin_off >= 0 && !fuse && !vop_op(d)) {
        static const int split_env = env_int("GPI_BWD_SPLIT", 1);
        const int per_cu = std::min((int)(160000 / std::max<size_t>(lds, 1)), d.k == 5 ? 4 : 6);
        G.split = (split_env && d.wpart_off >= 0 && 2 * G.nblocks <= std::min(per_cu, 4) * 256) ? 1 : 0;
    }
    const int grid = G.nblocks * (G.split ? 2 : 1);
    G.grid = grid;
    G.xcd = xcd_mode(fwd, fuse, G.split != 0, G.nfull < G.nblocks) ? 1 : 0;
    static const int fuse_alt = env_int("GPI_FUSE_ALT", 1);
    G.alt = fuse ? fuse_alt : 0;
    {
        const int shapes_on = env_int("GPI_CONV_SHAPES", 1);
        static const int record = env_int("GPI_CONV_SHAPES_RECORD", 0);
        const ShapeC s = shape_of(d, G, fwd, fuse, cp, exf);
        g_shape_planned += dry ? 0 : 1;
        const int si = shapes_on ? shape_index(s) : -1;
        const conv_kernel_t ks = si >= 0 ? shape_kernel_any(si) : nullptr;
        if (ks) {
            k = ks;
            g_shape_matched += dry ? 0 : 1;
        }
        if (record || dry) {
            std::lock_guard<std::mutex> lk(g_shapes_mu);
            bool seen = false;
            for (const ShapeC& q : g_shapes_seen) seen = seen || memcmp(&q, &s, sizeof(ShapeC)) == 0;
            if (!seen) g_shapes_seen.push_back(s);
        }
        if (dry) return GPI_OK;
    }
#ifdef GPI_PHASE_TIMING
    static const int dbg_print = env_int("GPI_DBG_PRINT", 0);
    if (dbg_print)
        fprintf(stderr, "conv %s k%d s%d up%d cin%d cout%d in%dx%d out%dx%d th%d blocks %d lds %zu\n",
                fwd ? "fwd" : "bwd", d.k, d.stride, d.upsample, d.cin, d.cout, d.h_in, d.w_in, d.h_out, d.w_out, G.th,
                G.nblocks, lds);
#endif
    if (lds > 64 * 1024) {
        if (hipFuncSetAttribute((const void*)k, hipFuncAttributeMaxDynamicSharedMemorySize, (int)lds) != hipSuccess)
            return GPI_ERR_LAUNCH;
    }
    hipLaunchKernelGGL(k, dim3(grid), dim3(256), lds, st, d, c, G);
    GPI_CHECK_LAUNCH();
    return GPI_OK;
}

#ifndef GPI_RROWS
#define GPI_RROWS 64
#endif
constexpr int RROWS = GPI_RROWS;

struct ReduceArgs {
    gpi_reduce_item it[GPI_MAX_REDUCE_ITEMS];
    int32_t first_block[GPI_MAX_REDUCE_ITEMS + 1];
    int32_t wchunks[GPI_MAX_REDUCE_ITEMS];
    int32_t n;
    int32_t rrows;
};

__global__ __launch_bounds__(256) void wgrad_reduce(ReduceArgs a, const float* __restrict__ wpart, double* gacc) {
    __shared__ float red[256];
    int k = 0;
    while (k + 1 < a.n && (int)blockIdx.x >= a.first_block[k + 1]) ++k;
    const gpi_reduce_item it = a.it[k];
    const int local = blockIdx.x - a.first_block[k];
    const int wc = local % a.wchunks[k], rc = local / a.wchunks[k];
    const int w0 = wc * 256;
    const int nw = min(256, it.numel - w0);
    const int P = 256 / nw;
    const int tid = threadIdx.x;
    const int w = tid % nw, p = tid / nw;
    const int r0 = rc * a.rrows, r1 = min(it.blocks, r0 + a.rrows);
    float s = 0.f;
    if (p < P) {
        const float* base = wpart + it.part_off + w0 + w;
        float acc[4] = {0.f, 0.f, 0.f, 0.f};
        int r = r0 + p;
        for (; r + 15 * P < r1; r += 16 * P) {
            float v[16];
#pragma unroll
            for (int u = 0; u < 16; ++u) v[u] = base[(int64_t)(r + u * P) * it.row_stride];
#pragma unroll
            for (int u = 0; u < 16; ++u) acc[u & 3] += v[u];
        }
        for (; r < r1; r += P) acc[0] += base[(int64_t)r * it.row_stride];
        s = (acc[0] + acc[1]) + (acc[2] + acc[3]);
    }
    red[tid] = s;
    __syncthreads();
    if (tid < nw) {
        double t = 0.0;
        for (int q = 0; q < P; ++q) t += (double)red[q * nw + tid];
        atomicAdd(gacc + it.w_off + w0 + tid, t);
    }
}

__global__ __launch_bounds__(256) void bn_running_kernel(const gpi_bn_running_item* items, int n_items, int max_ch,
                                                         const gpi_stat* stats, int64_t n_stats, float momentum) {
    const int t = blockIdx.x * 256 + threadIdx.x;
    const int li = t / max_ch, c = t - li * max_ch;
    if (li >= n_items) return;
    const gpi_bn_running_item it = items[li];
    if (c >= it.channels) return;
    double rm = it.running_mean[c], rv = it.running_var[c];
    for (int k = 0; k < it.n_calls; ++k) {
        double s = 0.0, s2 = 0.0;
        for (int r = 0; r < GPI_REPLICAS; ++r) {
            const gpi_stat& st = stats[((int64_t)r * GPI_MAX_GROUPS + it.group[k]) * n_stats + it.stat + c];
            s += st.sum;
            s2 += st.sumsq;
        }
        const double n = it.count[k];
        const double mean = s / n;
        double var = s2 / n - mean * mean;
        if (var < 0.0) var = 0.0;
        rm = (1.0 - momentum) * rm + momentum * mean;
        rv = (1.0 - momentum) * rv + momentum * (n > 1.0 ? var * n / (n - 1.0) : var);
    }
    it.running_mean[c] = (float)rm;
    it.running_var[c] = (float)rv;
    if (c == 0) *it.num_batches_tracked += it.n_calls;
}

#endif
}

#if GPI_CONV_SHAPE_PART == 0
extern "C" int gpi_bn_running_update(const gpi_bn_running_item* items, int n_items, int max_channels,
                                     const gpi_stat* stats, int64_t n_stats, float momentum, void* stream) {
    if (n_items < 0 || max_channels < 1 || (n_items > 0 && (!items || !stats))) return GPI_ERR_ARG;
    if (n_items == 0) return GPI_OK;
    const int threads = n_items * max_channels;
    hipLaunchKernelGGL(bn_running_kernel, dim3((threads + 255) / 256), dim3(256), 0, (hipStream_t)stream, items, n_items,
                       max_channels, stats, n_stats, momentum);
    GPI_CHECK_LAUNCH();
    return GPI_OK;
}

#ifdef GPI_PHASE_TIMING
extern "C" int gpi_debug_phase_stamps(unsigned long long* phase, unsigned long long* rt) {
    static unsigned long long zeros[4096 * 16];
    if (hipMemcpyFromSymbol(phase, HIP_SYMBOL(g_phase), sizeof(zeros)) != hipSuccess) return GPI_ERR_LAUNCH;
    if (hipMemcpyFromSymbol(rt, HIP_SYMBOL(g_rt), sizeof(unsigned long long) * 4096 * 2) != hipSuccess)
        return GPI_ERR_LAUNCH;
    if (hipMemcpyToSymbol(HIP_SYMBOL(g_phase), zeros, sizeof(zeros)) != hipSuccess) return GPI_ERR_LAUNCH;
    if (hipMemcpyToSymbol(HIP_SYMBOL(g_rt), zeros, sizeof(unsigned long long) * 4096 * 2) != hipSuccess)
        return GPI_ERR_LAUNCH;
    return GPI_OK;
}
#endif

extern "C" int gpi_conv_blocks(const gpi_conv_desc* op, const gpi_groups* groups, int32_t* blocks) {
    if (!op || !groups || !blocks) return GPI_ERR_ARG;
    ConvGeom G;
    if (!conv_geom(*op, *groups, G, false)) return GPI_ERR_UNSUPPORTED;
    *blocks = G.nblocks * ((vop_op(*op) || lsum_op(*op, G) || vsum_op(*op, G)) ? 1 : SLAB_ROWS);
    return GPI_OK;
}

extern "C" int gpi_conv_launch_info(const gpi_conv_desc* op, const gpi_groups* groups, int fwd, int32_t* info) {
// ... 130 lines not shown
```

generative-physics-informed-pde_amd/csrc/conv_shapes.h:

```cpp
#define GPI_CONV_SHAPE_COUNT 134
#define GPI_CONV_SHAPE_LIST \
    {1,0,0,0,0,8,2,0,0,0,1,1,7,2,3,0,1,6,64,64,32,32,0,0,1,0,16,2,37,72,19,40,32,0,2,1,0,0,0,0,0,0,1,0,0,14,4,1,6,6,6448900,0,238609295,0,22605092,0,429496730,0,0,1,715827883,0,67108864,0,8388608,0,134217728,0,134217728,0,16,37,19,32,0,0,14,4,1,6,6,6448900,0,22605092,0,8388608,0}, \
    {0,0,0,0,0,0,0,0,0,0,1,1,7,2,3,0,1,6,64,64,32,32,0,0,1,0,16,2,37,72,19,40,32,0,1,1,0,1,1,0,0,0,0,0,0,14,4,1,6,6,6448900,0,238609295,0,22605092,0,429496730,0,0,1,715827883,0,67108864,0,8388608,0,134217728,0,134217728,0,16,37,19,32,0,0,14,4,1,6,6,6448900,0,22605092,0,8388608,0}, \
    {1,0,0,0,0,4,1,0,1,1,1,0,3,1,1,0,6,4,32,32,32,32,1,0,1,1,8,4,10,40,10,40,8,0,1,1,0,0,0,0,0,0,1,0,2,5,6,2,5,6,42949673,0,429496730,0,42949673,0,429496730,0,715827883,0,1073741824,0,134217728,0,16777216,0,134217728,0,268435456,0,8,10,10,8,0,2,5,6,2,5,6,42949673,0,42949673,0,16777216,0}, \
    {0,0,0,0,0,0,0,0,1,1,1,0,3,1,1,0,6,4,32,32,32,32,1,0,1,1,16,2,18,40,18,40,16,1,1,1,0,0,0,0,0,1,0,0,1,7,6,1,7,6,23860930,0,429496730,0,23860930,0,429496730,0,715827883,0,1073741824,0,134217728,0,8388608,0,134217728,0,268435456,0,16,18,18,16,1,1,7,6,1,7,6,23860930,0,23860930,0,8388608,0}, \
    {1,0,0,0,0,6,1,0,1,1,1,0,1,1,0,0,10,5,32,32,32,32,1,0,1,0,8,4,8,40,8,40,8,0,1,1,0,0,0,0,0,0,1,0,3,1,6,3,1,6,53687092,0,429496730,0,53687092,0,429496730,0,429496730,0,858993460,0,134217728,0,16777216,0,134217728,0,268435456,0,8,8,8,8,0,3,1,6,3,1,6,53687092,0,53687092,0,16777216,0}, \
    {0,0,0,0,0,0,0,0,1,1,1,0,1,1,0,0,10,5,32,32,32,32,1,0,1,0,8,4,8,40,8,40,8,1,1,1,0,0,0,0,0,0,0,0,3,1,6,3,1,6,53687092,0,429496730,0,53687092,0,429496730,0,429496730,0,858993460,0,134217728,0,16777216,0,134217728,0,268435456,0,8,8,8,8,1,3,1,6,3,1,6,53687092,0,53687092,0,16777216,0}, \
    {1,0,0,0,0,6,0,0,1,1,1,0,3,2,1,0,5,5,32,32,16,16,1,0,1,0,8,2,17,40,9,24,16,0,1,2,0,0,0,0,0,0,1,0,1,8,6,4,6,4,25264514,0,429496730,0,79536432,0,715827883,0,858993460,0,858993460,0,134217728,0,33554432,0,268435456,0,268435456,0,8,17,9,16,0,1,8,6,4,6,4,25264514,0,79536432,0,33554432,0}, \
    {0,0,0,0,0,0,0,0,1,1,1,0,3,2,1,0,5,5,32,32,16,16,1,0,1,0,4,4,9,40,5,24,8,1,1,1,0,0,0,0,1,0,0,0,2,7,6,8,2,4,47721859,0,429496730,0,143165577,0,715827883,0,858993460,0,858993460,0,134217728,0,67108864,0,268435456,0,268435456,0,4,9,5,8,1,2,7,6,8,2,4,47721859,0,143165577,0,67108864,0}, \
    {1,0,0,0,0,4,1,0,1,1,1,0,3,1,1,0,5,4,16,16,16,16,1,0,1,1,16,1,18,24,18,24,16,0,1,1,0,0,0,0,0,0,1,0,2,6,4,2,6,4,39768216,0,715827883,0,39768216,0,715827883,0,858993460,0,1073741824,0,268435456,0,16777216,0,268435456,0,536870912,0,16,18,18,16,0,2,6,4,2,6,4,39768216,0,39768216,0,16777216,0}, \
    {0,0,0,0,0,0,0,0,1,1,1,0,3,1,1,0,5,4,16,16,16,16,1,0,1,1,8,2,10,24,10,24,8,1,1,1,0,0,0,0,1,1,0,0,4,2,4,4,2,4,71582789,0,715827883,0,71582789,0,715827883,0,858993460,0,1073741824,0,268435456,0,33554432,0,268435456,0,536870912,0,8,10,10,8,1,4,2,4,4,2,4,71582789,0,71582789,0,33554432,0}, \
    {1,0,0,0,0,4,1,0,1,1,1,0,3,1,1,0,9,4,16,16,16,16,1,0,1,1,16,1,18,24,18,24,16,0,1,1,0,0,0,0,0,0,1,0,2,6,4,2,6,4,39768216,0,715827883,0,39768216,0,715827883,0,477218589,0,1073741824,0,268435456,0,16777216,0,268435456,0,536870912,0,16,18,18,16,0,2,6,4,2,6,4,39768216,0,39768216,0,16777216,0}, \
    {0,0,0,0,0,0,0,0,1,1,1,0,3,1,1,0,9,4,16,16,16,16,1,0,1,1,8,2,10,24,10,24,8,1,1,1,0,0,0,0,1,1,0,0,4,2,4,4,2,4,71582789,0,715827883,0,71582789,0,715827883,0,477218589,0,1073741824,0,268435456,0,33554432,0,268435456,0,536870912,0,8,10,10,8,1,4,2,4,4,2,4,71582789,0,71582789,0,33554432,0}, \
    {1,0,0,0,0,6,1,0,1,1,1,0,1,1,0,0,13,6,16,16,16,16,1,0,1,0,16,1,16,24,16,24,16,0,1,1,0,0,0,0,0,0,1,0,2,10,4,2,10,4,44739243,0,715827883,0,44739243,0,715827883,0,330382100,0,715827883,0,268435456,0,16777216,0,268435456,0,536870912,0,16,16,16,16,0,2,10,4,2,10,4,44739243,0,44739243,0,16777216,0}, \
    {0,0,0,0,0,0,0,0,1,1,1,0,1,1,0,0,13,6,16,16,16,16,1,0,1,0,8,2,8,24,8,24,8,1,1,1,0,0,0,0,1,1,0,0,5,2,4,5,2,4,89478486,0,715827883,0,89478486,0,715827883,0,330382100,0,715827883,0,268435456,0,33554432,0,268435456,0,536870912,0,8,8,8,8,1,5,2,4,5,2,4,89478486,0,89478486,0,33554432,0}, \
    {1,0,0,0,0,6,0,0,1,1,1,0,3,2,1,0,6,6,16,16,8,8,1,0,1,0,8,1,17,24,9,16,16,0,1,4,0,0,0,0,0,0,1,0,2,8,4,7,1,0,42107523,0,715827883,0,119304648,0,1073741824,0,715827883,0,715827883,0,268435456,0,67108864,0,536870912,0,536870912,0,8,17,9,16,0,2,8,4,7,1,0,42107523,0,119304648,0,67108864,0}, \
    {0,0,0,0,0,0,0,0,1,1,1,0,3,2,1,0,6,6,16,16,8,8,1,0,1,0,4,2,9,24,5,16,8,1,1,1,0,0,0,0,1,1,0,0,4,6,4,12,4,0,79536432,0,715827883,0,214748365,0,1073741824,0,715827883,0,715827883,0,268435456,0,134217728,0,536870912,0,536870912,0,4,9,5,8,1,4,6,4,12,4,0,79536432,0,214748365,0,134217728,0}, \
    {1,0,0,0,0,4,0,0,1,1,1,0,3,1,1,0,6,4,8,8,8,8,1,0,1,1,8,1,10,16,10,16,8,0,1,4,0,0,0,0,0,0,1,0,6,4,0,6,4,0,107374183,0,1073741824,0,107374183,0,1073741824,0,715827883,0,1073741824,0,536870912,0,67108864,0,536870912,0,1073741824,0,8,10,10,8,0,6,4,0,6,4,0,107374183,0,107374183,0,67108864,0}, \
    {0,0,0,0,0,0,0,0,1,1,1,0,3,1,1,0,6,4,8,8,8,8,1,0,1,1,8,1,10,16,10,16,8,1,1,1,0,0,0,0,1,1,0,0,6,4,0,6,4,0,107374183,0,1073741824,0,107374183,0,1073741824,0,715827883,0,1073741824,0,536870912,0,67108864,0,536870912,0,1073741824,0,8,10,10,8,1,6,4,0,6,4,0,107374183,0,107374183,0,67108864,0}, \
    {1,0,0,0,0,6,0,0,1,1,1,0,1,1,0,0,10,5,8,8,8,8,1,0,1,0,8,1,8,16,8,16,8,0,1,4,0,0,0,0,0,0,1,0,8,0,0,8,0,0,134217728,0,1073741824,0,134217728,0,1073741824,0,429496730,0,858993460,0,536870912,0,67108864,0,536870912,0,1073741824,0,8,8,8,8,0,8,0,0,8,0,0,134217728,0,134217728,0,67108864,0}, \
    {0,0,0,0,0,0,0,0,1,1,1,0,1,1,0,0,10,5,8,8,8,8,1,0,1,0,8,1,8,16,8,16,8,1,1,1,0,0,0,0,1,1,0,0,8,0,0,8,0,0,134217728,0,1073741824,0,134217728,0,1073741824,0,429496730,0,858993460,0,536870912,0,67108864,0,536870912,0,1073741824,0,8,8,8,8,1,8,0,0,8,0,0,134217728,0,134217728,0,67108864,0}, \
    {1,0,0,0,0,6,0,0,1,1,1,0,3,2,1,0,5,5,8,8,4,4,1,1,0,0,4,1,9,16,5,12,8,0,1,5,0,0,0,0,0,0,1,0,7,1,0,17,0,1,119304648,0,1073741824,0,286331154,0,1431655766,0,858993460,0,858993460,0,536870912,0,268435456,0,1073741824,0,1073741824,0,4,9,5,8,0,7,1,0,17,0,1,119304648,0,286331154,0,268435456,0}, \
    {0,0,0,0,0,0,0,0,1,1,1,0,3,2,1,0,5,5,8,8,4,4,1,1,0,0,4,1,9,16,5,12,8,0,1,1,0,0,0,0,1,1,0,0,7,1,0,17,0,1,119304648,0,1073741824,0,286331154,0,1431655766,0,858993460,0,858993460,0,536870912,0,268435456,0,1073741824,0,1073741824,0,4,9,5,8,0,7,1,0,17,0,1,119304648,0,286331154,0,268435456,0}, \
    {1,0,1,0,0,8,1,0,1,0,1,0,3,1,1,0,1,6,8,8,8,8,0,0,1,0,8,1,10,16,10,16,8,0,1,1,0,0,0,0,0,0,0,0,6,4,0,6,4,0,107374183,0,1073741824,0,107374183,0,1073741824,0,0,1,715827883,0,536870912,0,67108864,0,536870912,0,1073741824,0,4,6,6,4,0,10,4,0,10,4,0,178956971,0,178956971,0,134217728,0}, \
    {0,0,1,0,0,0,0,0,1,0,1,0,3,1,1,0,1,6,8,8,8,8,0,0,1,0,8,1,10,16,10,16,8,1,1,1,0,0,0,0,1,1,0,0,6,4,0,6,4,0,107374183,0,1073741824,0,107374183,0,1073741824,0,0,1,715827883,0,536870912,0,67108864,0,536870912,0,1073741824,0,4,6,6,4,1,10,4,0,10,4,0,178956971,0,178956971,0,134217728,0}, \
    {0,0,1,0,0,0,0,0,1,1,1,0,3,1,1,0,6,4,8,8,8,8,1,0,1,1,8,1,10,16,10,16,8,1,1,1,0,0,0,0,1,1,0,0,6,4,0,6,4,0,107374183,0,1073741824,0,107374183,0,1073741824,0,715827883,0,1073741824,0,536870912,0,67108864,0,536870912,0,1073741824,0,4,6,6,4,1,10,4,0,10,4,0,178956971,0,178956971,0,134217728,0}, \
    {0,0,1,0,0,0,0,0,1,1,1,0,1,1,0,0,10,5,8,8,8,8,1,0,1,0,8,1,8,16,8,16,8,1,1,1,0,0,0,0,1,1,0,0,8,0,0,8,0,0,134217728,0,1073741824,0,134217728,0,1073741824,0,429496730,0,858993460,0,536870912,0,67108864,0,536870912,0,1073741824,0,4,4,4,4,1,16,0,0,16,0,0,268435456,0,268435456,0,134217728,0}, \
    {1,0,1,0,0,6,1,0,1,1,1,0,3,1,1,1,5,5,8,8,16,16,1,0,1,0,16,1,11,16,18,24,8,0,1,1,0,0,0,0,0,0,0,0,5,9,0,2,6,4,97612894,0,1073741824,0,39768216,0,715827883,0,858993460,0,858993460,0,536870912,0,16777216,0,268435456,0,1073741824,0,8,7,10,4,0,9,1,0,4,2,4,153391690,0,71582789,0,33554432,0}, \
    {0,0,1,0,0,0,0,1,1,1,1,0,3,1,1,1,5,5,8,8,16,16,1,0,1,0,16,1,11,16,18,24,8,1,1,1,0,0,0,0,1,1,0,0,5,9,0,2,6,4,97612894,0,1073741824,0,39768216,0,715827883,0,858993460,0,858993460,0,536870912,0,16777216,0,268435456,0,1073741824,0,8,7,10,4,1,9,1,0,4,2,4,153391690,0,71582789,0,33554432,0}, \
    {1,0,1,0,0,4,1,0,1,1,1,0,3,1,1,0,5,4,16,16,16,16,1,0,1,1,16,1,18,24,18,24,16,0,1,1,0,0,0,0,0,0,0,0,2,6,4,2,6,4,39768216,0,715827883,0,39768216,0,715827883,0,858993460,0,1073741824,0,268435456,0,16777216,0,268435456,0,536870912,0,8,10,10,8,0,4,2,4,4,2,4,71582789,0,71582789,0,33554432,0}, \
    {0,0,1,0,0,0,0,0,1,1,1,0,3,1,1,0,5,4,16,16,16,16,1,0,1,1,8,2,10,24,10,24,8,1,1,1,0,0,0,0,1,0,0,0,4,2,4,4,2,4,71582789,0,715827883,0,71582789,0,715827883,0,858993460,0,1073741824,0,268435456,0,33554432,0,268435456,0,536870912,0,4,6,6,4,1,7,0,4,7,0,4,119304648,0,119304648,0,67108864,0}, \
    {1,0,1,0,0,4,1,0,1,1,1,0,3,1,1,0,9,4,16,16,16,16,1,0,1,1,16,1,18,24,18,24,16,0,1,1,0,0,0,0,0,0,0,0,2,6,4,2,6,4,39768216,0,715827883,0,39768216,0,715827883,0,477218589,0,1073741824,0,268435456,0,16777216,0,268435456,0,536870912,0,8,10,10,8,0,4,2,4,4,2,4,71582789,0,71582789,0,33554432,0}, \
    {0,0,1,0,0,0,0,0,1,1,1,0,3,1,1,0,9,4,16,16,16,16,1,0,1,1,8,2,10,24,10,24,8,1,1,1,0,0,0,0,1,0,0,0,4,2,4,4,2,4,71582789,0,715827883,0,71582789,0,715827883,0,477218589,0,1073741824,0,268435456,0,33554432,0,268435456,0,536870912,0,4,6,6,4,1,7,0,4,7,0,4,119304648,0,119304648,0,67108864,0}, \
    {1,0,1,0,0,6,1,0,1,1,1,0,1,1,0,0,13,6,16,16,16,16,1,0,1,0,16,1,16,24,16,24,16,0,1,1,0,0,0,0,0,0,0,0,2,10,4,2,10,4,44739243,0,715827883,0,44739243,0,715827883,0,330382100,0,715827883,0,268435456,0,16777216,0,268435456,0,536870912,0,8,8,8,8,0,5,2,4,5,2,4,89478486,0,89478486,0,33554432,0}, \
    {0,0,1,0,0,0,0,0,1,1,1,0,1,1,0,0,13,6,16,16,16,16,1,0,1,0,8,2,8,24,8,24,8,1,1,1,0,0,0,0,1,0,0,0,5,2,4,5,2,4,89478486,0,715827883,0,89478486,0,715827883,0,330382100,0,715827883,0,268435456,0,33554432,0,268435456,0,536870912,0,4,4,4,4,1,10,2,4,10,2,4,178956971,0,178956971,0,67108864,0}, \
    {1,0,1,0,0,6,2,0,1,1,1,0,3,1,1,1,6,6,16,16,32,32,1,0,1,0,16,2,11,24,18,40,8,0,2,1,0,0,0,0,0,0,0,0,3,9,4,1,7,6,65075263,0,715827883,0,23860930,0,429496730,0,715827883,0,715827883,0,268435456,0,8388608,0,134217728,0,536870912,0,8,7,10,4,0,6,0,4,2,5,6,102261127,0,42949673,0,16777216,0}, \
    {0,0,1,0,0,0,0,2,1,1,1,0,3,1,1,1,6,6,16,16,32,32,1,0,1,0,16,2,11,24,18,40,8,0,1,1,0,0,0,1,0,0,0,0,3,9,4,1,7,6,65075263,0,715827883,0,23860930,0,429496730,0,715827883,0,715827883,0,268435456,0,8388608,0,134217728,0,536870912,0,8,7,10,4,1,6,0,4,2,5,6,102261127,0,42949673,0,16777216,0}, \
    {1,0,1,0,0,4,1,0,1,1,1,0,3,1,1,0,6,4,32,32,32,32,1,0,1,1,8,4,10,40,10,40,8,0,1,1,0,0,0,0,0,0,0,0,2,5,6,2,5,6,42949673,0,429496730,0,42949673,0,429496730,0,715827883,0,1073741824,0,134217728,0,16777216,0,134217728,0,268435456,0,4,6,6,4,0,4,1,6,4,1,6,71582789,0,71582789,0,33554432,0}, \
    {0,0,1,0,0,0,0,0,1,1,1,0,3,1,1,0,6,4,32,32,32,32,1,0,1,1,16,2,18,40,18,40,16,1,1,1,0,0,0,0,0,0,0,0,1,7,6,1,7,6,23860930,0,429496730,0,23860930,0,429496730,0,715827883,0,1073741824,0,134217728,0,8388608,0,134217728,0,268435456,0,8,10,10,8,1,2,5,6,2,5,6,42949673,0,42949673,0,16777216,0}, \
    {1,0,1,0,0,8,1,0,1,1,1,0,3,1,1,0,10,5,32,32,32,32,1,0,1,0,8,4,10,40,10,40,8,0,1,1,0,0,0,0,0,0,0,0,2,5,6,2,5,6,42949673,0,429496730,0,42949673,0,429496730,0,429496730,0,858993460,0,134217728,0,16777216,0,134217728,0,268435456,0,4,6,6,4,0,4,1,6,4,1,6,71582789,0,71582789,0,33554432,0}, \
    {0,0,1,0,0,0,0,0,1,1,1,0,3,1,1,0,10,5,32,32,32,32,1,0,1,0,8,4,10,40,10,40,8,1,1,1,0,0,0,0,0,0,0,0,2,5,6,2,5,6,42949673,0,429496730,0,42949673,0,429496730,0,429496730,0,858993460,0,134217728,0,16777216,0,134217728,0,268435456,0,4,6,6,4,1,4,1,6,4,1,6,71582789,0,71582789,0,33554432,0}, \
    {1,0,1,0,0,2,4,0,1,0,1,0,3,1,1,1,5,2,32,32,64,64,1,0,1,0,16,4,11,40,18,72,8,0,4,1,0,0,0,0,0,0,0,0,2,3,6,0,14,4,39045158,0,429496730,0,13256072,0,238609295,0,858993460,0,-2147483648,0,134217728,0,4194304,0,67108864,0,268435456,0,8,7,10,4,0,3,4,6,1,4,4,61356676,0,23860930,0,8388608,0}, \
    {0,0,1,0,0,0,0,1,1,0,1,0,3,1,1,1,5,2,32,32,64,64,1,0,1,0,16,4,11,40,18,72,8,1,1,1,0,0,0,0,0,0,0,0,2,3,6,0,14,4,39045158,0,429496730,0,13256072,0,238609295,0,858993460,0,-2147483648,0,134217728,0,4194304,0,67108864,0,268435456,0,8,7,10,4,1,3,4,6,1,4,4,61356676,0,23860930,0,8388608,0}, \
    {0,1,1,0,0,0,0,0,1,0,1,0,5,1,2,0,2,2,64,64,64,64,1,1,2,0,16,4,24,72,20,72,16,0,1,1,1,0,0,0,0,0,0,1,0,14,4,0,14,4,9942054,0,238609295,0,11930465,0,238609295,0,-2147483648,0,-2147483648,0,67108864,0,4194304,0,67108864,0,134217728,0,8,16,12,8,0,0,14,4,1,2,4,14913081,0,19884108,0,8388608,0}, \
    {1,0,0,0,0,8,2,0,0,0,1,1,7,2,3,0,1,6,128,128,64,64,0,0,1,0,8,8,21,136,11,72,16,0,2,1,0,0,0,0,0,0,1,0,0,7,18,1,3,4,6015361,0,126322568,0,21691755,0,238609295,0,0,1,715827883,0,33554432,0,8388608,0,67108864,0,67108864,0,8,21,11,16,0,0,7,18,1,3,4,6015361,0,21691755,0,8388608,0}, \
    {0,0,0,0,0,0,0,0,0,0,1,1,7,2,3,0,1,6,128,128,64,64,0,0,1,0,8,8,21,136,11,72,16,0,1,1,0,1,1,0,0,0,0,0,0,7,18,1,3,4,6015361,0,126322568,0,21691755,0,238609295,0,0,1,715827883,0,33554432,0,8388608,0,67108864,0,67108864,0,8,21,11,16,0,0,7,18,1,3,4,6015361,0,21691755,0,8388608,0}, \
    {1,0,0,0,0,4,2,0,1,1,1,0,3,1,1,0,6,4,64,64,64,64,1,0,1,1,8,8,10,72,10,72,8,0,2,1,0,0,0,0,0,0,1,0,1,4,4,1,4,4,23860930,0,238609295,0,23860930,0,238609295,0,715827883,0,1073741824,0,67108864,0,8388608,0,67108864,0,134217728,0,8,10,10,8,0,1,4,4,1,4,4,23860930,0,23860930,0,8388608,0}, \
    {0,0,0,0,0,0,0,0,1,1,1,0,3,1,1,0,6,4,64,64,64,64,1,0,1,1,8,8,10,72,10,72,8,1,1,1,0,0,0,0,0,0,0,0,1,4,4,1,4,4,23860930,0,238609295,0,23860930,0,238609295,0,715827883,0,1073741824,0,67108864,0,8388608,0,67108864,0,134217728,0,8,10,10,8,1,1,4,4,1,4,4,23860930,0,23860930,0,8388608,0}, \
    {1,0,0,0,0,6,2,0,1,1,1,0,1,1,0,0,10,5,64,64,64,64,1,0,1,0,8,8,8,72,8,72,8,0,2,1,0,0,0,0,0,0,1,0,1,6,4,1,6,4,29826162,0,238609295,0,29826162,0,238609295,0,429496730,0,858993460,0,67108864,0,8388608,0,67108864,0,134217728,0,8,8,8,8,0,1,6,4,1,6,4,29826162,0,29826162,0,8388608,0}, \
    {0,0,0,0,0,0,0,0,1,1,1,0,1,1,0,0,10,5,64,64,64,64,1,0,1,0,8,8,8,72,8,72,8,1,1,1,0,0,0,0,0,0,0,0,1,6,4,1,6,4,29826162,0,238609295,0,29826162,0,238609295,0,429496730,0,858993460,0,67108864,0,8388608,0,67108864,0,134217728,0,8,8,8,8,1,1,6,4,1,6,4,29826162,0,29826162,0,8388608,0}, \
    {1,0,0,0,0,6,0,0,1,1,1,0,3,2,1,0,5,5,64,64,32,32,1,0,1,0,4,8,9,72,5,40,8,0,1,2,0,0,0,0,0,0,1,0,1,5,4,5,0,6,26512144,0,238609295,0,85899346,0,429496730,0,858993460,0,858993460,0,67108864,0,33554432,0,134217728,0,134217728,0,4,9,5,8,0,1,5,4,5,0,6,26512144,0,85899346,0,33554432,0}, \
    {0,0,0,0,0,0,0,0,1,1,1,0,3,2,1,0,5,5,64,64,32,32,1,0,1,0,4,8,9,72,5,40,8,1,1,1,0,0,0,0,0,0,0,0,1,5,4,5,0,6,26512144,0,238609295,0,85899346,0,429496730,0,858993460,0,858993460,0,67108864,0,33554432,0,134217728,0,134217728,0,4,9,5,8,1,1,5,4,5,0,6,26512144,0,85899346,0,33554432,0}, \
    {1,0,0,0,0,4,1,0,1,1,1,0,3,1,1,0,5,4,32,32,32,32,1,0,1,1,8,4,10,40,10,40,8,0,1,1,0,0,0,0,0,0,1,0,2,5,6,2,5,6,42949673,0,429496730,0,42949673,0,429496730,0,858993460,0,1073741824,0,134217728,0,16777216,0,134217728,0,268435456,0,8,10,10,8,0,2,5,6,2,5,6,42949673,0,42949673,0,16777216,0}, \
    {0,0,0,0,0,0,0,0,1,1,1,0,3,1,1,0,5,4,32,32,32,32,1,0,1,1,16,2,18,40,18,40,16,1,1,1,0,0,0,0,0,1,0,0,1,7,6,1,7,6,23860930,0,429496730,0,23860930,0,429496730,0,858993460,0,1073741824,0,134217728,0,8388608,0,134217728,0,268435456,0,16,18,18,16,1,1,7,6,1,7,6,23860930,0,23860930,0,8388608,0}, \
    {1,0,0,0,0,4,1,0,1,1,1,0,3,1,1,0,9,4,32,32,32,32,1,0,1,1,8,4,10,40,10,40,8,0,1,1,0,0,0,0,0,0,1,0,2,5,6,2,5,6,42949673,0,429496730,0,42949673,0,429496730,0,477218589,0,1073741824,0,134217728,0,16777216,0,134217728,0,268435456,0,8,10,10,8,0,2,5,6,2,5,6,42949673,0,42949673,0,16777216,0}, \
    {0,0,0,0,0,0,0,0,1,1,1,0,3,1,1,0,9,4,32,32,32,32,1,0,1,1,8,4,10,40,10,40,8,1,1,1,0,0,0,0,0,0,0,0,2,5,6,2,5,6,42949673,0,429496730,0,42949673,0,429496730,0,477218589,0,1073741824,0,134217728,0,16777216,0,134217728,0,268435456,0,8,10,10,8,1,2,5,6,2,5,6,42949673,0,42949673,0,16777216,0}, \
    {1,0,0,0,0,6,1,0,1,1,1,0,1,1,0,0,13,6,32,32,32,32,1,0,1,0,8,4,8,40,8,40,8,0,1,1,0,0,0,0,0,0,1,0,3,1,6,3,1,6,53687092,0,429496730,0,53687092,0,429496730,0,330382100,0,715827883,0,134217728,0,16777216,0,134217728,0,268435456,0,8,8,8,8,0,3,1,6,3,1,6,53687092,0,53687092,0,16777216,0}, \
    {0,0,0,0,0,0,0,0,1,1,1,0,1,1,0,0,13,6,32,32,32,32,1,0,1,0,8,4,8,40,8,40,8,1,1,1,0,0,0,0,0,0,0,0,3,1,6,3,1,6,53687092,0,429496730,0,53687092,0,429496730,0,330382100,0,715827883,0,134217728,0,16777216,0,134217728,0,268435456,0,8,8,8,8,1,3,1,6,3,1,6,53687092,0,53687092,0,16777216,0}, \
    {1,0,0,0,0,6,0,0,1,1,1,0,3,2,1,0,6,6,32,32,16,16,1,0,1,0,8,2,17,40,9,24,16,0,1,2,0,0,0,0,0,0,1,0,1,8,6,4,6,4,25264514,0,429496730,0,79536432,0,715827883,0,715827883,0,715827883,0,134217728,0,33554432,0,268435456,0,268435456,0,8,17,9,16,0,1,8,6,4,6,4,25264514,0,79536432,0,33554432,0}, \
    {0,0,0,0,0,0,0,0,1,1,1,0,3,2,1,0,6,6,32,32,16,16,1,0,1,0,4,4,9,40,5,24,8,1,1,1,0,0,0,0,1,0,0,0,2,7,6,8,2,4,47721859,0,429496730,0,143165577,0,715827883,0,715827883,0,715827883,0,134217728,0,67108864,0,268435456,0,268435456,0,4,9,5,8,1,2,7,6,8,2,4,47721859,0,143165577,0,67108864,0}, \
    {1,0,0,0,0,4,1,0,1,1,1,0,3,1,1,0,6,4,16,16,16,16,1,0,1,1,16,1,18,24,18,24,16,0,1,1,0,0,0,0,0,0,1,0,2,6,4,2,6,4,39768216,0,715827883,0,39768216,0,715827883,0,715827883,0,1073741824,0,268435456,0,16777216,0,268435456,0,536870912,0,16,18,18,16,0,2,6,4,2,6,4,39768216,0,39768216,0,16777216,0}, \
    {0,0,0,0,0,0,0,0,1,1,1,0,3,1,1,0,6,4,16,16,16,16,1,0,1,1,8,2,10,24,10,24,8,1,1,1,0,0,0,0,1,1,0,0,4,2,4,4,2,4,71582789,0,715827883,0,71582789,0,715827883,0,715827883,0,1073741824,0,268435456,0,33554432,0,268435456,0,536870912,0,8,10,10,8,1,4,2,4,4,2,4,71582789,0,71582789,0,33554432,0}, \
    {1,0,0,0,0,4,1,0,1,1,1,0,3,1,1,0,10,4,16,16,16,16,1,0,1,1,16,1,18,24,18,24,16,0,1,1,0,0,0,0,0,0,1,0,2,6,4,2,6,4,39768216,0,715827883,0,39768216,0,715827883,0,429496730,0,1073741824,0,268435456,0,16777216,0,268435456,0,536870912,0,16,18,18,16,0,2,6,4,2,6,4,39768216,0,39768216,0,16777216,0}, \
    {0,0,0,0,0,0,0,0,1,1,1,0,3,1,1,0,10,4,16,16,16,16,1,0,1,1,8,2,10,24,10,24,8,1,1,1,0,0,0,0,1,1,0,0,4,2,4,4,2,4,71582789,0,715827883,0,71582789,0,715827883,0,429496730,0,1073741824,0,268435456,0,33554432,0,268435456,0,536870912,0,8,10,10,8,1,4,2,4,4,2,4,71582789,0,71582789,0,33554432,0}, \
    {1,0,0,0,0,8,1,0,1,1,1,0,1,1,0,0,14,7,16,16,16,16,1,0,1,0,16,1,16,24,16,24,16,0,1,1,0,0,0,0,0,0,1,0,2,10,4,2,10,4,44739243,0,715827883,0,44739243,0,715827883,0,306783379,0,613566757,0,268435456,0,16777216,0,268435456,0,536870912,0,16,16,16,16,0,2,10,4,2,10,4,44739243,0,44739243,0,16777216,0}, \
    {0,0,0,0,0,0,0,0,1,1,1,0,1,1,0,0,14,7,16,16,16,16,1,0,1,0,8,2,8,24,8,24,8,1,1,1,0,0,0,0,1,1,0,0,5,2,4,5,2,4,89478486,0,715827883,0,89478486,0,715827883,0,306783379,0,613566757,0,268435456,0,33554432,0,268435456,0,536870912,0,8,8,8,8,1,5,2,4,5,2,4,89478486,0,89478486,0,33554432,0}, \
    {1,0,0,0,0,8,0,0,1,1,1,0,3,2,1,0,7,7,16,16,8,8,1,0,1,0,8,1,17,24,9,16,16,0,1,4,0,0,0,0,0,0,1,0,2,8,4,7,1,0,42107523,0,715827883,0,119304648,0,1073741824,0,613566757,0,613566757,0,268435456,0,67108864,0,536870912,0,536870912,0,8,17,9,16,0,2,8,4,7,1,0,42107523,0,119304648,0,67108864,0}, \
    {0,0,0,0,0,0,0,0,1,1,1,0,3,2,1,0,7,7,16,16,8,8,1,0,1,0,4,2,9,24,5,16,8,1,1,1,0,0,0,0,1,1,0,0,4,6,4,12,4,0,79536432,0,715827883,0,214748365,0,1073741824,0,613566757,0,613566757,0,268435456,0,134217728,0,536870912,0,536870912,0,4,9,5,8,1,4,6,4,12,4,0,79536432,0,214748365,0,134217728,0}, \
    {1,0,0,0,0,4,0,0,1,1,1,0,3,1,1,0,7,4,8,8,8,8,1,0,1,1,8,1,10,16,10,16,8,0,1,4,0,0,0,0,0,0,1,0,6,4,0,6,4,0,107374183,0,1073741824,0,107374183,0,1073741824,0,613566757,0,1073741824,0,536870912,0,67108864,0,536870912,0,1073741824,0,8,10,10,8,0,6,4,0,6,4,0,107374183,0,107374183,0,67108864,0}, \
    {0,0,0,0,0,0,0,0,1,1,1,0,3,1,1,0,7,4,8,8,8,8,1,0,1,1,8,1,10,16,10,16,8,1,1,1,0,0,0,0,1,1,0,0,6,4,0,6,4,0,107374183,0,1073741824,0,107374183,0,1073741824,0,613566757,0,1073741824,0,536870912,0,67108864,0,536870912,0,1073741824,0,8,10,10,8,1,6,4,0,6,4,0,107374183,0,107374183,0,67108864,0}, \
    {1,0,0,0,0,6,0,0,1,1,1,0,1,1,0,0,11,5,8,8,8,8,1,0,1,0,8,1,8,16,8,16,8,0,1,4,0,0,0,0,0,0,1,0,8,0,0,8,0,0,134217728,0,1073741824,0,134217728,0,1073741824,0,390451573,0,858993460,0,536870912,0,67108864,0,536870912,0,1073741824,0,8,8,8,8,0,8,0,0,8,0,0,134217728,0,134217728,0,67108864,0}, \
    {0,0,0,0,0,0,0,0,1,1,1,0,1,1,0,0,11,5,8,8,8,8,1,0,1,0,8,1,8,16,8,16,8,1,1,1,0,0,0,0,1,1,0,0,8,0,0,8,0,0,134217728,0,1073741824,0,134217728,0,1073741824,0,390451573,0,858993460,0,536870912,0,67108864,0,536870912,0,1073741824,0,8,8,8,8,1,8,0,0,8,0,0,134217728,0,134217728,0,67108864,0}, \
    {1,0,1,0,0,4,1,0,1,1,1,0,3,1,1,0,10,4,32,32,32,32,1,0,1,1,8,4,10,40,10,40,8,0,1,1,0,0,0,0,0,0,0,0,2,5,6,2,5,6,42949673,0,429496730,0,42949673,0,429496730,0,429496730,0,1073741824,0,134217728,0,16777216,0,134217728,0,268435456,0,4,6,6,4,0,4,1,6,4,1,6,71582789,0,71582789,0,33554432,0}, \
    {0,0,1,0,0,0,0,0,1,1,1,0,3,1,1,0,10,4,32,32,32,32,1,0,1,1,8,4,10,40,10,40,8,1,1,1,0,0,0,0,0,0,0,0,2,5,6,2,5,6,42949673,0,429496730,0,42949673,0,429496730,0,429496730,0,1073741824,0,134217728,0,16777216,0,134217728,0,268435456,0,4,6,6,4,1,4,1,6,4,1,6,71582789,0,71582789,0,33554432,0}, \
    {1,0,1,0,0,8,1,0,1,1,1,0,1,1,0,0,14,7,32,32,32,32,1,0,1,0,8,4,8,40,8,40,8,0,1,1,0,0,0,0,0,0,0,0,3,1,6,3,1,6,53687092,0,429496730,0,53687092,0,429496730,0,306783379,0,613566757,0,134217728,0,16777216,0,134217728,0,268435456,0,4,4,4,4,0,6,1,6,6,1,6,107374183,0,107374183,0,33554432,0}, \
    {0,0,1,0,0,0,0,0,1,1,1,0,1,1,0,0,14,7,32,32,32,32,1,0,1,0,8,4,8,40,8,40,8,1,1,1,0,0,0,0,0,0,0,0,3,1,6,3,1,6,53687092,0,429496730,0,53687092,0,429496730,0,306783379,0,613566757,0,134217728,0,16777216,0,134217728,0,268435456,0,4,4,4,4,1,6,1,6,6,1,6,107374183,0,107374183,0,33554432,0}, \
    {1,0,1,0,0,8,4,0,1,1,1,0,3,1,1,1,7,7,32,32,64,64,1,0,1,0,16,4,11,40,18,72,8,0,4,1,0,0,0,0,0,0,0,0,2,3,6,0,14,4,39045158,0,429496730,0,13256072,0,238609295,0,613566757,0,613566757,0,134217728,0,4194304,0,67108864,0,268435456,0,8,7,10,4,0,3,4,6,1,4,4,61356676,0,23860930,0,8388608,0}, \
    {0,0,1,0,0,0,0,2,1,1,1,0,3,1,1,1,7,7,32,32,64,64,1,0,1,0,16,4,11,40,18,72,8,0,1,1,0,0,0,1,0,0,0,0,2,3,6,0,14,4,39045158,0,429496730,0,13256072,0,238609295,0,613566757,0,613566757,0,134217728,0,4194304,0,67108864,0,268435456,0,8,7,10,4,0,3,4,6,1,4,4,61356676,0,23860930,0,8388608,0}, \
    {1,0,0,0,0,4,2,0,1,1,1,0,3,1,1,0,7,4,64,64,64,64,1,0,1,1,8,8,10,72,10,72,8,0,2,1,0,0,0,0,0,0,1,0,1,4,4,1,4,4,23860930,0,238609295,0,23860930,0,238609295,0,613566757,0,1073741824,0,67108864,0,8388608,0,67108864,0,134217728,0,8,10,10,8,0,1,4,4,1,4,4,23860930,0,23860930,0,8388608,0}, \
    {0,0,0,0,0,0,0,0,1,1,1,0,3,1,1,0,7,4,64,64,64,64,1,0,1,1,8,8,10,72,10,72,8,1,1,1,0,0,0,0,0,0,0,0,1,4,4,1,4,4,23860930,0,238609295,0,23860930,0,238609295,0,613566757,0,1073741824,0,67108864,0,8388608,0,67108864,0,134217728,0,8,10,10,8,1,1,4,4,1,4,4,23860930,0,23860930,0,8388608,0}, \
    {1,0,0,0,0,8,1,0,1,1,1,0,3,1,1,0,11,5,64,64,64,64,1,0,1,0,4,16,6,72,6,72,4,0,1,1,0,0,0,0,0,0,1,0,2,2,4,2,2,4,39768216,0,238609295,0,39768216,0,238609295,0,390451573,0,858993460,0,67108864,0,16777216,0,67108864,0,134217728,0,4,6,6,4,0,2,2,4,2,2,4,39768216,0,39768216,0,16777216,0}, \
    {0,0,0,0,0,0,0,0,1,1,1,0,3,1,1,0,11,5,64,64,64,64,1,0,1,0,8,8,10,72,10,72,8,0,1,1,0,0,0,0,0,0,0,0,1,4,4,1,4,4,23860930,0,238609295,0,23860930,0,238609295,0,390451573,0,858993460,0,67108864,0,8388608,0,67108864,0,134217728,0,8,10,10,8,0,1,4,4,1,4,4,23860930,0,23860930,0,8388608,0}, \
    {1,0,0,0,0,2,4,0,1,0,1,0,3,1,1,1,5,2,64,64,128,128,1,0,1,0,8,16,7,72,10,136,4,0,4,1,0,0,0,0,0,0,1,0,2,0,4,0,7,18,34087043,0,238609295,0,12632257,0,126322568,0,858993460,0,-2147483648,0,67108864,0,4194304,0,33554432,0,134217728,0,8,7,10,4,0,2,0,4,0,7,18,34087043,0,12632257,0,4194304,0}, \
    {0,0,0,0,0,0,0,1,1,0,1,0,3,1,1,1,5,2,64,64,128,128,1,0,1,0,8,16,7,72,10,136,4,1,1,1,0,0,0,0,0,0,0,0,2,0,4,0,7,18,34087043,0,238609295,0,12632257,0,126322568,0,858993460,0,-2147483648,0,67108864,0,4194304,0,33554432,0,134217728,0,8,7,10,4,1,2,0,4,0,7,18,34087043,0,12632257,0,4194304,0}, \
    {0,1,0,0,0,0,0,0,1,0,1,0,5,1,2,0,2,2,128,128,128,128,1,1,2,0,8,16,16,136,12,136,8,0,1,1,1,0,0,0,0,0,1,1,0,7,18,0,7,18,7895161,0,126322568,0,10526881,0,126322568,0,-2147483648,0,-2147483648,0,33554432,0,4194304,0,33554432,0,67108864,0,8,16,12,8,0,0,7,18,0,7,18,7895161,0,10526881,0,4194304,0}, \
    {1,0,0,0,0,8,2,0,0,0,1,1,7,2,3,0,1,6,256,256,128,128,0,0,1,0,4,32,13,264,7,136,8,0,2,1,0,0,0,0,0,0,1,0,0,3,58,1,0,18,5005790,0,65075263,0,18046082,0,126322568,0,0,1,715827883,0,16777216,0,8388608,0,33554432,0,33554432,0,4,13,7,8,0,0,3,58,1,0,18,5005790,0,18046082,0,8388608,0}, \
    {0,0,0,0,0,0,0,0,0,0,1,1,7,2,3,0,1,6,256,256,128,128,0,0,1,0,4,32,13,264,7,136,8,0,1,1,0,1,1,0,0,0,0,0,0,3,58,1,0,18,5005790,0,65075263,0,18046082,0,126322568,0,0,1,715827883,0,16777216,0,8388608,0,33554432,0,33554432,0,4,13,7,8,0,0,3,58,1,0,18,5005790,0,18046082,0,8388608,0}, \
    {1,0,0,0,0,4,2,0,1,1,1,0,3,1,1,0,6,4,128,128,128,128,1,0,1,1,4,32,6,136,6,136,4,0,2,1,0,0,0,0,0,0,1,0,1,1,18,1,1,18,21053762,0,126322568,0,21053762,0,126322568,0,715827883,0,1073741824,0,33554432,0,8388608,0,33554432,0,67108864,0,4,6,6,4,0,1,1,18,1,1,18,21053762,0,21053762,0,8388608,0}, \
    {0,0,0,0,0,0,0,0,1,1,1,0,3,1,1,0,6,4,128,128,128,128,1,0,1,1,4,32,6,136,6,136,4,0,1,1,0,0,0,0,0,0,0,0,1,1,18,1,1,18,21053762,0,126322568,0,21053762,0,126322568,0,715827883,0,1073741824,0,33554432,0,8388608,0,33554432,0,67108864,0,4,6,6,4,0,1,1,18,1,1,18,21053762,0,21053762,0,8388608,0}, \
    {1,0,0,0,0,6,2,0,1,1,1,0,1,1,0,0,10,5,128,128,128,128,1,0,1,0,4,32,4,136,4,136,4,0,2,1,0,0,0,0,0,0,1,0,1,3,18,1,3,18,31580642,0,126322568,0,31580642,0,126322568,0,429496730,0,858993460,0,33554432,0,8388608,0,33554432,0,67108864,0,4,4,4,4,0,1,3,18,1,3,18,31580642,0,31580642,0,8388608,0}, \
    {0,0,0,0,0,0,0,0,1,1,1,0,1,1,0,0,10,5,128,128,128,128,1,0,1,0,4,32,4,136,4,136,4,1,1,1,0,0,0,0,0,0,0,0,1,3,18,1,3,18,31580642,0,126322568,0,31580642,0,126322568,0,429496730,0,858993460,0,33554432,0,8388608,0,33554432,0,67108864,0,4,4,4,4,1,1,3,18,1,3,18,31580642,0,31580642,0,8388608,0}, \
    {1,0,0,0,0,6,0,0,1,1,1,0,3,2,1,0,5,5,128,128,64,64,1,0,1,0,2,32,5,136,3,72,4,0,1,2,0,0,0,0,0,0,1,0,1,2,18,4,2,4,25264514,0,126322568,0,79536432,0,238609295,0,858993460,0,858993460,0,33554432,0,33554432,0,67108864,0,67108864,0,2,5,3,4,0,1,2,18,4,2,4,25264514,0,79536432,0,33554432,0}, \
    {0,0,0,0,0,0,0,0,1,1,1,0,3,2,1,0,5,5,128,128,64,64,1,0,1,0,4,16,9,136,5,72,8,1,1,1,0,0,0,0,0,0,0,0,0,7,18,2,4,4,14035841,0,126322568,0,47721859,0,238609295,0,858993460,0,858993460,0,33554432,0,16777216,0,67108864,0,67108864,0,4,9,5,8,1,0,7,18,2,4,4,14035841,0,47721859,0,16777216,0}, \
    {1,0,0,0,0,4,4,0,1,1,1,0,3,1,1,0,5,4,64,64,64,64,1,0,1,1,16,4,18,72,18,72,16,0,4,1,0,0,0,0,0,0,1,0,0,14,4,0,14,4,13256072,0,238609295,0,13256072,0,238609295,0,858993460,0,1073741824,0,67108864,0,4194304,0,67108864,0,134217728,0,16,18,18,16,0,0,14,4,0,14,4,13256072,0,13256072,0,4194304,0}, \
    {0,0,0,0,0,0,0,0,1,1,1,0,3,1,1,0,5,4,64,64,64,64,1,0,1,1,8,8,10,72,10,72,8,1,1,1,0,0,0,0,0,0,0,0,1,4,4,1,4,4,23860930,0,238609295,0,23860930,0,238609295,0,858993460,0,1073741824,0,67108864,0,8388608,0,67108864,0,134217728,0,8,10,10,8,1,1,4,4,1,4,4,23860930,0,23860930,0,8388608,0}, \
    {1,0,0,0,0,4,2,0,1,1,1,0,3,1,1,0,9,4,64,64,64,64,1,0,1,1,8,8,10,72,10,72,8,0,2,1,0,0,0,0,0,0,1,0,1,4,4,1,4,4,23860930,0,238609295,0,23860930,0,238609295,0,477218589,0,1073741824,0,67108864,0,8388608,0,67108864,0,134217728,0,8,10,10,8,0,1,4,4,1,4,4,23860930,0,23860930,0,8388608,0}, \
    {0,0,0,0,0,0,0,0,1,1,1,0,3,1,1,0,9,4,64,64,64,64,1,0,1,1,8,8,10,72,10,72,8,1,1,1,0,0,0,0,0,0,0,0,1,4,4,1,4,4,23860930,0,238609295,0,23860930,0,238609295,0,477218589,0,1073741824,0,67108864,0,8388608,0,67108864,0,134217728,0,8,10,10,8,1,1,4,4,1,4,4,23860930,0,23860930,0,8388608,0}, \
    {1,0,0,0,0,6,1,0,1,1,1,0,1,1,0,0,13,6,64,64,64,64,1,0,1,0,4,16,4,72,4,72,4,0,1,1,0,0,0,0,0,0,1,0,3,2,4,3,2,4,59652324,0,238609295,0,59652324,0,238609295,0,330382100,0,715827883,0,67108864,0,16777216,0,67108864,0,134217728,0,4,4,4,4,0,3,2,4,3,2,4,59652324,0,59652324,0,16777216,0}, \
    {0,0,0,0,0,0,0,0,1,1,1,0,1,1,0,0,13,6,64,64,64,64,1,0,1,0,8,8,8,72,8,72,8,0,1,1,0,0,0,0,0,0,0,0,1,6,4,1,6,4,29826162,0,238609295,0,29826162,0,238609295,0,330382100,0,715827883,0,67108864,0,8388608,0,67108864,0,134217728,0,8,8,8,8,0,1,6,4,1,6,4,29826162,0,29826162,0,8388608,0}, \
    {1,0,0,0,0,6,0,0,1,1,1,0,3,2,1,0,6,6,64,64,32,32,1,0,1,0,4,8,9,72,5,40,8,0,1,2,0,0,0,0,0,0,1,0,1,5,4,5,0,6,26512144,0,238609295,0,85899346,0,429496730,0,715827883,0,715827883,0,67108864,0,33554432,0,134217728,0,134217728,0,4,9,5,8,0,1,5,4,5,0,6,26512144,0,85899346,0,33554432,0}, \
    {0,0,0,0,0,0,0,0,1,1,1,0,3,2,1,0,6,6,64,64,32,32,1,0,1,0,4,8,9,72,5,40,8,1,1,1,0,0,0,0,0,0,0,0,1,5,4,5,0,6,26512144,0,238609295,0,85899346,0,429496730,0,715827883,0,715827883,0,67108864,0,33554432,0,134217728,0,134217728,0,4,9,5,8,1,1,5,4,5,0,6,26512144,0,85899346,0,33554432,0}, \
    {1,0,0,0,0,4,1,0,1,1,1,0,3,1,1,0,10,4,32,32,32,32,1,0,1,1,8,4,10,40,10,40,8,0,1,1,0,0,0,0,0,0,1,0,2,5,6,2,5,6,42949673,0,429496730,0,42949673,0,429496730,0,429496730,0,1073741824,0,134217728,0,16777216,0,134217728,0,268435456,0,8,10,10,8,0,2,5,6,2,5,6,42949673,0,42949673,0,16777216,0}, \
    {0,0,0,0,0,0,0,0,1,1,1,0,3,1,1,0,10,4,32,32,32,32,1,0,1,1,8,4,10,40,10,40,8,1,1,1,0,0,0,0,0,1,0,0,2,5,6,2,5,6,42949673,0,429496730,0,42949673,0,429496730,0,429496730,0,1073741824,0,134217728,0,16777216,0,134217728,0,268435456,0,8,10,10,8,1,2,5,6,2,5,6,42949673,0,42949673,0,16777216,0}, \
    {1,0,0,0,0,8,1,0,1,1,1,0,1,1,0,0,14,7,32,32,32,32,1,0,1,0,8,4,8,40,8,40,8,0,1,1,0,0,0,0,0,0,1,0,3,1,6,3,1,6,53687092,0,429496730,0,53687092,0,429496730,0,306783379,0,613566757,0,134217728,0,16777216,0,134217728,0,268435456,0,8,8,8,8,0,3,1,6,3,1,6,53687092,0,53687092,0,16777216,0}, \
    {0,0,0,0,0,0,0,0,1,1,1,0,1,1,0,0,14,7,32,32,32,32,1,0,1,0,8,4,8,40,8,40,8,1,1,1,0,0,0,0,0,1,0,0,3,1,6,3,1,6,53687092,0,429496730,0,53687092,0,429496730,0,306783379,0,613566757,0,134217728,0,16777216,0,134217728,0,268435456,0,8,8,8,8,1,3,1,6,3,1,6,53687092,0,53687092,0,16777216,0}, \
    {1,0,0,0,0,8,0,0,1,1,1,0,3,2,1,0,7,7,32,32,16,16,1,0,1,0,8,2,17,40,9,24,16,0,1,2,0,0,0,0,0,0,1,0,1,8,6,4,6,4,25264514,0,429496730,0,79536432,0,715827883,0,613566757,0,613566757,0,134217728,0,33554432,0,268435456,0,268435456,0,8,17,9,16,0,1,8,6,4,6,4,25264514,0,79536432,0,33554432,0}, \
    {0,0,0,0,0,0,0,0,1,1,1,0,3,2,1,0,7,7,32,32,16,16,1,0,1,0,4,4,9,40,5,24,8,1,1,1,0,0,0,0,1,1,0,0,2,7,6,8,2,4,47721859,0,429496730,0,143165577,0,715827883,0,613566757,0,613566757,0,134217728,0,67108864,0,268435456,0,268435456,0,4,9,5,8,1,2,7,6,8,2,4,47721859,0,143165577,0,67108864,0}, \
    {1,0,0,0,0,4,1,0,1,1,1,0,3,1,1,0,7,4,16,16,16,16,1,0,1,1,16,1,18,24,18,24,16,0,1,1,0,0,0,0,0,0,1,0,2,6,4,2,6,4,39768216,0,715827883,0,39768216,0,715827883,0,613566757,0,1073741824,0,268435456,0,16777216,0,268435456,0,536870912,0,16,18,18,16,0,2,6,4,2,6,4,39768216,0,39768216,0,16777216,0}, \
    {0,0,0,0,0,0,0,0,1,1,1,0,3,1,1,0,7,4,16,16,16,16,1,0,1,1,8,2,10,24,10,24,8,1,1,1,0,0,0,0,1,1,0,0,4,2,4,4,2,4,71582789,0,715827883,0,71582789,0,715827883,0,613566757,0,1073741824,0,268435456,0,33554432,0,268435456,0,536870912,0,8,10,10,8,1,4,2,4,4,2,4,71582789,0,71582789,0,33554432,0}, \
    {1,0,0,0,0,4,1,0,1,1,1,0,3,1,1,0,11,4,16,16,16,16,1,0,1,1,16,1,18,24,18,24,16,0,1,1,0,0,0,0,0,0,1,0,2,6,4,2,6,4,39768216,0,715827883,0,39768216,0,715827883,0,390451573,0,1073741824,0,268435456,0,16777216,0,268435456,0,536870912,0,16,18,18,16,0,2,6,4,2,6,4,39768216,0,39768216,0,16777216,0}, \
    {0,0,0,0,0,0,0,0,1,1,1,0,3,1,1,0,11,4,16,16,16,16,1,0,1,1,8,2,10,24,10,24,8,1,1,1,0,0,0,0,0,1,0,0,4,2,4,4,2,4,71582789,0,715827883,0,71582789,0,715827883,0,390451573,0,1073741824,0,268435456,0,33554432,0,268435456,0,536870912,0,8,10,10,8,1,4,2,4,4,2,4,71582789,0,71582789,0,33554432,0}, \
    {1,0,0,0,0,8,1,0,1,1,1,0,1,1,0,0,15,7,16,16,16,16,1,0,1,0,16,1,16,24,16,24,16,0,1,1,0,0,0,0,0,0,1,0,2,10,4,2,10,4,44739243,0,715827883,0,44739243,0,715827883,0,286331154,0,613566757,0,268435456,0,16777216,0,268435456,0,536870912,0,16,16,16,16,0,2,10,4,2,10,4,44739243,0,44739243,0,16777216,0}, \
    {0,0,0,0,0,0,0,0,1,1,1,0,1,1,0,0,15,7,16,16,16,16,1,0,1,0,8,2,8,24,8,24,8,1,1,1,0,0,0,0,1,1,0,0,5,2,4,5,2,4,89478486,0,715827883,0,89478486,0,715827883,0,286331154,0,613566757,0,268435456,0,33554432,0,268435456,0,536870912,0,8,8,8,8,1,5,2,4,5,2,4,89478486,0,89478486,0,33554432,0}, \
    {1,0,0,0,0,8,1,0,1,0,1,0,3,1,1,0,1,6,8,8,8,8,0,0,1,0,8,1,10,16,10,16,8,0,1,1,0,0,0,0,0,0,1,0,6,4,0,6,4,0,107374183,0,1073741824,0,107374183,0,1073741824,0,0,1,715827883,0,536870912,0,67108864,0,536870912,0,1073741824,0,8,10,10,8,0,6,4,0,6,4,0,107374183,0,107374183,0,67108864,0}, \
    {0,0,0,0,0,0,0,0,1,0,1,0,3,1,1,0,1,6,8,8,8,8,0,0,1,0,8,1,10,16,10,16,8,1,1,1,0,0,0,0,1,1,0,0,6,4,0,6,4,0,107374183,0,1073741824,0,107374183,0,1073741824,0,0,1,715827883,0,536870912,0,67108864,0,536870912,0,1073741824,0,8,10,10,8,1,6,4,0,6,4,0,107374183,0,107374183,0,67108864,0}, \
    {1,0,0,0,0,6,1,0,1,1,1,0,3,1,1,1,5,5,8,8,16,16,1,0,1,0,16,1,11,16,18,24,8,0,1,1,0,0,0,0,0,0,1,0,5,9,0,2,6,4,97612894,0,1073741824,0,39768216,0,715827883,0,858993460,0,858993460,0,536870912,0,16777216,0,268435456,0,1073741824,0,16,11,18,8,0,5,9,0,2,6,4,97612894,0,39768216,0,16777216,0}, \
    {0,0,0,0,0,0,0,1,1,1,1,0,3,1,1,1,5,5,8,8,16,16,1,0,1,0,16,1,11,16,18,24,8,1,1,1,0,0,0,0,1,1,0,0,5,9,0,2,6,4,97612894,0,1073741824,0,39768216,0,715827883,0,858993460,0,858993460,0,536870912,0,16777216,0,268435456,0,1073741824,0,16,11,18,8,1,5,9,0,2,6,4,97612894,0,39768216,0,16777216,0}, \
    {0,0,1,0,0,0,0,0,1,1,1,0,3,1,1,0,5,4,16,16,16,16,1,0,1,1,8,2,10,24,10,24,8,1,1,1,0,0,0,0,1,1,0,0,4,2,4,4,2,4,71582789,0,715827883,0,71582789,0,715827883,0,858993460,0,1073741824,0,268435456,0,33554432,0,268435456,0,536870912,0,4,6,6,4,1,7,0,4,7,0,4,119304648,0,119304648,0,67108864,0}, \
    {0,0,1,0,0,0,0,0,1,1,1,0,3,1,1,0,9,4,16,16,16,16,1,0,1,1,8,2,10,24,10,24,8,1,1,1,0,0,0,0,1,1,0,0,4,2,4,4,2,4,71582789,0,715827883,0,71582789,0,715827883,0,477218589,0,1073741824,0,268435456,0,33554432,0,268435456,0,536870912,0,4,6,6,4,1,7,0,4,7,0,4,119304648,0,119304648,0,67108864,0}, \
    {0,0,1,0,0,0,0,0,1,1,1,0,1,1,0,0,13,6,16,16,16,16,1,0,1,0,8,2,8,24,8,24,8,1,1,1,0,0,0,0,1,1,0,0,5,2,4,5,2,4,89478486,0,715827883,0,89478486,0,715827883,0,330382100,0,715827883,0,268435456,0,33554432,0,268435456,0,536870912,0,4,4,4,4,1,10,2,4,10,2,4,178956971,0,178956971,0,67108864,0}, \
    {0,0,1,0,0,0,0,2,1,1,1,0,3,1,1,1,6,6,16,16,32,32,1,0,1,0,16,2,11,24,18,40,8,0,1,1,0,0,0,1,0,1,0,0,3,9,4,1,7,6,65075263,0,715827883,0,23860930,0,429496730,0,715827883,0,715827883,0,268435456,0,8388608,0,134217728,0,536870912,0,8,7,10,4,1,6,0,4,2,5,6,102261127,0,42949673,0,16777216,0}, \
    {0,0,1,0,0,0,0,0,1,1,1,0,3,1,1,0,6,4,32,32,32,32,1,0,1,1,16,2,18,40,18,40,16,1,1,1,0,0,0,0,0,1,0,0,1,7,6,1,7,6,23860930,0,429496730,0,23860930,0,429496730,0,715827883,0,1073741824,0,134217728,0,8388608,0,134217728,0,268435456,0,8,10,10,8,1,2,5,6,2,5,6,42949673,0,42949673,0,16777216,0}, \
    {1,0,0,0,0,4,1,0,1,1,1,0,3,1,1,0,11,4,64,64,64,64,1,0,1,1,4,16,6,72,6,72,4,0,1,1,0,0,0,0,0,0,1,0,2,2,4,2,2,4,39768216,0,238609295,0,39768216,0,238609295,0,390451573,0,1073741824,0,67108864,0,16777216,0,67108864,0,134217728,0,4,6,6,4,0,2,2,4,2,2,4,39768216,0,39768216,0,16777216,0}, \
    {0,0,0,0,0,0,0,0,1,1,1,0,3,1,1,0,11,4,64,64,64,64,1,0,1,1,8,8,10,72,10,72,8,1,1,1,0,0,0,0,0,0,0,0,1,4,4,1,4,4,23860930,0,238609295,0,23860930,0,238609295,0,390451573,0,1073741824,0,67108864,0,8388608,0,67108864,0,134217728,0,8,10,10,8,1,1,4,4,1,4,4,23860930,0,23860930,0,8388608,0}, \
    {1,0,0,0,0,8,1,0,1,1,1,0,1,1,0,0,15,7,64,64,64,64,1,0,1,0,4,16,4,72,4,72,4,0,1,1,0,0,0,0,0,0,1,0,3,2,4,3,2,4,59652324,0,238609295,0,59652324,0,238609295,0,286331154,0,613566757,0,67108864,0,16777216,0,67108864,0,134217728,0,4,4,4,4,0,3,2,4,3,2,4,59652324,0,59652324,0,16777216,0}, \
    {0,0,0,0,0,0,0,0,1,1,1,0,1,1,0,0,15,7,64,64,64,64,1,0,1,0,8,8,8,72,8,72,8,0,1,1,0,0,0,0,0,0,0,0,1,6,4,1,6,4,29826162,0,238609295,0,29826162,0,238609295,0,286331154,0,613566757,0,67108864,0,8388608,0,67108864,0,134217728,0,8,8,8,8,0,1,6,4,1,6,4,29826162,0,29826162,0,8388608,0}, \
    {1,0,0,0,0,8,4,0,1,1,1,0,3,1,1,1,7,7,64,64,128,128,1,0,1,0,8,16,7,72,10,136,4,0,4,1,0,0,0,0,0,0,1,0,2,0,4,0,7,18,34087043,0,238609295,0,12632257,0,126322568,0,613566757,0,613566757,0,67108864,0,4194304,0,33554432,0,134217728,0,8,7,10,4,0,2,0,4,0,7,18,34087043,0,12632257,0,4194304,0}, \
    {0,0,0,0,0,0,0,2,1,1,1,0,3,1,1,1,7,7,64,64,128,128,1,0,1,0,8,16,7,72,10,136,4,0,1,1,0,0,0,1,0,0,0,0,2,0,4,0,7,18,34087043,0,238609295,0,12632257,0,126322568,0,613566757,0,613566757,0,67108864,0,4194304,0,33554432,0,134217728,0,8,7,10,4,0,2,0,4,0,7,18,34087043,0,12632257,0,4194304,0}, \
    {1,0,0,0,0,4,2,0,1,1,1,0,3,1,1,0,7,4,128,128,128,128,1,0,1,1,4,32,6,136,6,136,4,0,2,1,0,0,0,0,0,0,1,0,1,1,18,1,1,18,21053762,0,126322568,0,21053762,0,126322568,0,613566757,0,1073741824,0,33554432,0,8388608,0,33554432,0,67108864,0,4,6,6,4,0,1,1,18,1,1,18,21053762,0,21053762,0,8388608,0}, \
    {0,0,0,0,0,0,0,0,1,1,1,0,3,1,1,0,7,4,128,128,128,128,1,0,1,1,4,32,6,136,6,136,4,0,1,1,0,0,0,0,0,0,0,0,1,1,18,1,1,18,21053762,0,126322568,0,21053762,0,126322568,0,613566757,0,1073741824,0,33554432,0,8388608,0,33554432,0,67108864,0,4,6,6,4,0,1,1,18,1,1,18,21053762,0,21053762,0,8388608,0}, \
    {1,0,0,0,0,8,1,0,1,1,1,0,3,1,1,0,11,5,128,128,128,128,1,0,1,0,2,64,4,136,4,136,2,0,1,1,0,0,0,0,0,0,1,0,1,3,18,1,3,18,31580642,0,126322568,0,31580642,0,126322568,0,390451573,0,858993460,0,33554432,0,16777216,0,33554432,0,67108864,0,2,4,4,2,0,1,3,18,1,3,18,31580642,0,31580642,0,16777216,0}, \
    {0,0,0,0,0,0,0,0,1,1,1,0,3,1,1,0,11,5,128,128,128,128,1,0,1,0,4,32,6,136,6,136,4,0,1,1,0,0,0,0,0,0,0,0,1,1,18,1,1,18,21053762,0,126322568,0,21053762,0,126322568,0,390451573,0,858993460,0,33554432,0,8388608,0,33554432,0,67108864,0,4,6,6,4,0,1,1,18,1,1,18,21053762,0,21053762,0,8388608,0}, \
    {1,0,0,0,0,2,4,0,1,0,1,0,3,1,1,1,5,2,128,128,256,256,1,0,1,0,4,64,5,136,6,264,2,0,4,1,0,0,0,0,0,0,1,0,1,2,18,0,3,58,25264514,0,126322568,0,10845878,0,65075263,0,858993460,0,-2147483648,0,33554432,0,4194304,0,16777216,0,67108864,0,4,5,6,2,0,1,2,18,0,3,58,25264514,0,10845878,0,4194304,0}, \
    {0,0,0,0,0,0,0,1,1,0,1,0,3,1,1,1,5,2,128,128,256,256,1,0,1,0,4,64,5,136,6,264,2,0,1,1,0,0,0,0,0,0,0,0,1,2,18,0,3,58,25264514,0,126322568,0,10845878,0,65075263,0,858993460,0,-2147483648,0,33554432,0,4194304,0,16777216,0,67108864,0,4,5,6,2,0,1,2,18,0,3,58,25264514,0,10845878,0,4194304,0}, \
    {0,1,0,0,0,0,0,0,1,0,1,0,5,1,2,0,2,2,256,256,256,256,1,1,2,0,4,64,12,264,8,264,4,0,1,1,1,0,0,0,0,0,1,1,0,3,58,0,3,58,5422939,0,65075263,0,8134408,0,65075263,0,-2147483648,0,-2147483648,0,16777216,0,4194304,0,16777216,0,33554432,0,4,12,8,4,0,0,3,58,0,3,58,5422939,0,8134408,0,4194304,0},
#define GPI_CONV_SHAPE_BOUNDS {0, 43, 74, 104, 134}
#define GPI_CONV_SHAPE_NOFOLD {92, 126, 133}
```

Before: 655,900 samples/s.

## Add row-pair forward conv variant splitting output channels across half-blocks

Adds a new forward 3x3 stride-1 convolution path for 16- and 32-wide outputs with 3–8 output channels. Each thread now computes two vertically adjacent output rows for half of the output channels, so input window rows are shared between the two rows. Weights are restaged in a split, padded layout, and the statistics epilogue gains a DPP-based reduction. The aim is more input reuse and less work per thread. The cost is a new kernel instantiation and some extra LDS for the padded weights, and the shape table is updated to select it by default.

```diff
diff --git a/generative-physics-informed-pde_amd/csrc/conv.hip b/generative-physics-informed-pde_amd/csrc/conv.hip
--- a/generative-physics-informed-pde_amd/csrc/conv.hip
+++ b/generative-physics-informed-pde_amd/csrc/conv.hip
@@ -141,6 +141,15 @@
     return v && *v ? atoi(v) : dflt;
 }
 
+constexpr int NPX_ROWS2 = -2;
+__host__ __device__ constexpr int fwd_wci(int kk, int cp, int npx) {
+    return npx == NPX_ROWS2 ? 2 * ((kk * ((cp / 2 + 1) & ~1) + 3) & ~3) : kk * cp;
+}
+bool fwd_rows2(const gpi_conv_desc& d, const ConvGeom& G) {
+    return d.k == 3 && d.stride == 1 && d.cout >= 3 && d.cout <= 8 && G.th * d.w_out == 256 &&
+           (d.w_out == 16 || d.w_out == 32) && d.epilogue != GPI_EPI_GAUSS_LOSS && d.epilogue != GPI_EPI_GAUSS_EXP_LOSS;
+}
+
 
 bool conv_geom(const gpi_conv_desc& d, const gpi_groups& g, ConvGeom& G, bool fwd, bool fuse = false) {
     if (g.n_groups < 1 || g.n_groups > GPI_MAX_GROUPS) return false;
@@ -219,6 +228,10 @@
         static const int cg_on = env_int("GPI_FWD_CG", 1);
         const int tp = G.th * d.w_out;
         if (cg_on && tp <= 128 && 256 % tp == 0 && !d.upsample && d.k <= 3) G.cg = std::min(256 / tp, d.cin);
+    }
+    if (fwd && G.npx == 1 && G.cg == 1) {
+        static const int rows2 = env_int("GPI_FWD_ROWS2", 1);
+        if (rows2 && fwd_rows2(d, G)) G.npx = NPX_ROWS2;
     }
     G.zreg = (!fwd && d.gout_mode == 0 && (int64_t)d.cout * G.gh * (G.PG / 4) <= (int64_t)ZREG * 256) ? 1 : 0;
     G.split = 0;
@@ -705,8 +718,11 @@
     float* scratch = sh + GPI_MAX_CIN;
     float* red = scratch + 64;
     float* dsl = red + 16;
+    constexpr bool ROWS2 = NPX == NPX_ROWS2;
+    constexpr int WCI = fwd_wci(KK, CP, NPX), HC = CP / 2, HS = (HC + 1) & ~1, WH = (KK * HS + 3) & ~3;
+    static_assert(!ROWS2 || (K == 3 && S == 1 && WCI == 2 * WH), "the row-pair form is the 3x3 / stride-1 forward's");
     float* wT = smem + pad256(FWD_HDR);
-    const int nw = d.cin * KK * CP;
+    const int nw = d.cin * WCI;
     float* img = wT + pad256(nw);
 
     const int tid = threadIdx.x;
@@ -723,6 +739,12 @@
     PHASE(1);
 
     stage(wT, nw, zero, [&](int e) -> const float* {
+        if constexpr (ROWS2) {
+            const int ci = e / WCI, q = e - ci * WCI, hf = q / WH, i = q - hf * WH, tap = i / HS, j = i - tap * HS;
+            const int c2 = (d.cout + 1) >> 1;
+            const bool ok = tap < KK && j < (hf ? d.cout - c2 : c2);
+            return ok ? params + w_off + ((int64_t)(hf * c2 + j) * d.cin + ci) * KK + tap : nullptr;
+        }
         const int co = e % CP, r = e / CP;
         return co < d.cout ? params + w_off + (int64_t)co * d.cin * KK + r : nullptr;
     });
@@ -892,6 +914,127 @@
                         vst[2 * co + 1] += a * a;
                     }
                 }
+            }
+        }
+    } else if constexpr (ROWS2) {
+        const int hf = tid >> 7, g = tid & 127;
+        const int c2 = (d.cout + 1) >> 1;
+        const int nh = hf ? d.cout - c2 : c2, c0 = hf * c2;
+        const int py = dq(g, Gt.d_wout), ox = g - py * d.w_out;
+        const int ty = 2 * py, oy = T.oy0 + ty;
+        const bool active = 2 * g < tp;
+        PHASE(5);
+        float acc[2][HC];
+#pragma unroll
+        for (int p = 0; p < 2; ++p)
+#pragma unroll
+            for (int j = 0; j < HC; ++j) acc[p][j] = 0.f;
+        if (active && !SKIP(G, 64)) {
+            constexpr int NR = UP ? 3 : 4;
+            const int plane = Gt.rh * Gt.P;
+            const int r0 = UP ? fdiv2(oy - 1) - iy0 : ty;
+            const int cb = (UP ? fdiv2(ox - 1) : ox - 1) + HALO;
+            const float* t0 = img + r0 * Gt.P + cb;
+#pragma unroll 1
+            for (int ci = 0; ci < d.cin; ++ci) {
+                const float* tci = t0 + ci * plane;
+                int wofs = pad256(FWD_HDR) + ci * WCI + hf * WH;
+                if (GPI_FWD_WVGPR) asm volatile("" : "+v"(wofs));
+                float wv[WH];
+#pragma unroll
+                for (int q = 0; q < WH / 4; ++q) {
+                    const f32x4 w4 = *reinterpret_cast<const f32x4*>(__builtin_assume_aligned(smem + wofs + 4 * q, 16));
+                    float w0 = w4[0], w1 = w4[1], w2 = w4[2], w3 = w4[3];
+                    asm("" : "+v"(w0), "+v"(w1), "+v"(w2), "+v"(w3));
+                    wv[4 * q] = w0, wv[4 * q + 1] = w1, wv[4 * q + 2] = w2, wv[4 * q + 3] = w3;
+                }
+                float win[NR][K];
+#pragma unroll
+                for (int r = 0; r < NR; ++r) {
+                    const float* trow = tci + r * Gt.P;
+                    if constexpr (UP) {
+                        const float v0 = trow[0], v1 = trow[1];
+                        win[r][0] = v0;
+                        win[r][1] = (ox & 1) ? v0 : v1;
+                        win[r][2] = v1;
+                    } else {
+#pragma unroll
+                        for (int kx = 0; kx < K; ++kx) win[r][kx] = trow[kx];
+                    }
+                }
+#pragma unroll
+                for (int ky = 0; ky < K; ++ky) {
+#pragma unroll
+                    for (int kx = 0; kx < K; ++kx) {
+#pragma unroll
+                        for (int p = 0; p < 2; ++p) {
+                            const float v = win[UP ? ((p + ky + 1) >> 1) : p + ky][kx];
+#pragma unroll
+                            for (int j = 0; j < HC; ++j) acc[p][j] = fmaf(wv[(ky * K + kx) * HS + j], v, acc[p][j]);
+                        }
+                    }
+                }
+            }
+        }
+        PHASE(6);
+        if (drop) {
+#pragma unroll
+            for (int j = 0; j < HC; ++j) {
+                if (j < c2 && j < nh) {
+                    const float ds = dsl[c0 + j];
+                    acc[0][j] *= ds;
+                    acc[1][j] *= ds;
+                }
+            }
+        }
+        if (active) {
+            float* o = ws + d.out_off + ((int64_t)T.b * d.out_ctot + d.out_c0 + c0) * HWo + oy * d.w_out + ox;
+#pragma unroll
+            for (int j = 0; j < HC; ++j) {
+                if (j < c2 && j < nh) {
+                    st1(o + (int64_t)j * HWo, acc[0][j]);
+                    st1(o + (int64_t)j * HWo + d.w_out, acc[1][j]);
+                }
+            }
+        }
+        if (d.epilogue == GPI_EPI_STORE_STATS && !SKIP(G, 128)) {
+            float s0[2 * HC], s1[2 * HC], y[2 * HC];
+#pragma unroll
+            for (int j = 0; j < HC; ++j) {
+                const bool ok = active && j < c2 && j < nh;
+                const float a0 = ok ? acc[0][j] : 0.f, a1 = ok ? acc[1][j] : 0.f;
+                s0[2 * j] = a0, s0[2 * j + 1] = a0 * a0;
+                s1[2 * j] = a1, s1[2 * j + 1] = a1 * a1;
+            }
+            dpp_step<0xb1, 0xf>(s0), dpp_step<0xb1, 0xf>(s1);
+            dpp_step<0x4e, 0xf>(s0), dpp_step<0x4e, 0xf>(s1);
+            dpp_step<0x124, 0xf>(s0), dpp_step<0x124, 0xf>(s1);
+            dpp_step<0x128, 0xf>(s0), dpp_step<0x128, 0xf>(s1);
+            if (d.w_out == 32) {
+                dpp_step<0x142, 0xa>(s0), dpp_step<0x142, 0xa>(s1);
+#pragma unroll
+                for (int q = 0; q < 2 * HC; ++q) y[q] = s1[q] + s0[q];
+            } else {
+#pragma unroll
+                for (int q = 0; q < 2 * HC; ++q) y[q] = s1[q] + s0[q];
+                dpp_step<0x142, 0xa>(y);
+            }
+            const int u = (tid >> 6) & 1;
+#pragma unroll
+            for (int q = 0; q < 2 * HC; ++q) {
+                const float lo = __int_as_float(__builtin_amdgcn_readlane(__float_as_int(y[q]), 31));
+                const float hi = __int_as_float(__builtin_amdgcn_readlane(__float_as_int(y[q]), 63));
+                if ((tid & 63) == 0 && (q >> 1) < c2 && (q >> 1) < nh) {
+                    scratch[(2 * c0 + q) * 4 + 2 * u] = lo;
+                    scratch[(2 * c0 + q) * 4 + 2 * u + 1] = hi;
+                }
+            }
+            __syncthreads();
+            if (tid < 2 * d.cout && !SKIP(G, 4)) {
+                float s = 0.f;
+                for (int w = 0; w < 4; ++w) s += scratch[tid * 4 + w];
+                gpi_stat* st = stat_slot(c, d.out_stat + (tid >> 1), T.grp);
+                atomicAdd((tid & 1) ? &st->sumsq : &st->sum, (double)s);
             }
         }
     } else {
@@ -990,7 +1133,7 @@
         }
     }
 
-    if (d.epilogue == GPI_EPI_GAUSS_LOSS || d.epilogue == GPI_EPI_GAUSS_EXP_LOSS) {
+    if (!ROWS2 && (d.epilogue == GPI_EPI_GAUSS_LOSS || d.epilogue == GPI_EPI_GAUSS_EXP_LOSS)) {
         float v[1] = {Lv};
         block_sum<1>(v, scratch, red);
         if (tid == 0 && !SKIP(G, 4)) atomicAdd(c.loss_acc + T.grp * GPI_REPLICAS + blockIdx.x % GPI_REPLICAS, (double)red[0]);
@@ -998,7 +1141,7 @@
         RTSTAMP(1);
         return;
     }
-    if (d.epilogue == GPI_EPI_STORE_STATS && !SKIP(G, 128)) {
+    if (!ROWS2 && d.epilogue == GPI_EPI_STORE_STATS && !SKIP(G, 128)) {
 #if GPI_FWD_WAVE_ATOMICS
         wave_sums(vst);
         const int lane = tid & 63;
@@ -2225,7 +2368,8 @@
 }
 
 size_t fwd_lds(const gpi_conv_desc& d, const ConvGeom& G, int cp) {
-    return sizeof(float) * ((size_t)pad256(FWD_HDR) + pad256(d.cin * d.k * d.k * cp) + img_floats(d.cin, G.rh, G.P) +
+    return sizeof(float) * ((size_t)pad256(FWD_HDR) + pad256(d.cin * fwd_wci(d.k * d.k, cp, G.npx)) +
+                            img_floats(d.cin, G.rh, G.P) +
                             (G.cg > 1 ? (size_t)(G.cg - 1) * G.th * d.w_out * cp : 0));
 }
 
@@ -2328,6 +2472,13 @@
         if (!fwd && ucls) return half ? conv_bwd_kernel<3, 1, 0, false, true, true> : conv_bwd_kernel<3, 1, 0, false, false, true>;
     }
     if (!fwd) return half ? conv_bwd_kernel<K, S, UP, false, true> : conv_bwd_kernel<K, S, UP>;
+    if constexpr (K == 3 && S == 1) {
+        if (npx == NPX_ROWS2) {
+            if (cp == 4) return half ? conv_fwd_kernel<K, S, UP, 4, NPX_ROWS2, true> : conv_fwd_kernel<K, S, UP, 4, NPX_ROWS2>;
+            if (cp == 6) return half ? conv_fwd_kernel<K, S, UP, 6, NPX_ROWS2, true> : conv_fwd_kernel<K, S, UP, 6, NPX_ROWS2>;
+            return half ? conv_fwd_kernel<K, S, UP, 8, NPX_ROWS2, true> : conv_fwd_kernel<K, S, UP, 8, NPX_ROWS2>;
+        }
+    }
     if (npx == 4) return pick_cp<K, S, UP, 4>(cp, half);
     if (npx == 2) return pick_cp<K, S, UP, 2>(cp, half);
     if constexpr (!UP && K <= 3) {
diff --git a/generative-physics-informed-pde_amd/csrc/conv_shapes.h b/generative-physics-informed-pde_amd/csrc/conv_shapes.h
--- a/generative-physics-informed-pde_amd/csrc/conv_shapes.h
+++ b/generative-physics-informed-pde_amd/csrc/conv_shapes.h
@@ -2,15 +2,15 @@
 #define GPI_CONV_SHAPE_LIST \
     {1,0,0,0,0,8,2,0,0,0,1,1,7,2,3,0,1,6,64,64,32,32,0,0,1,0,16,2,37,72,19,40,32,0,2,1,0,0,0,0,0,0,1,0,0,14,4,1,6,6,6448900,0,238609295,0,22605092,0,429496730,0,0,1,715827883,0,67108864,0,8388608,0,134217728,0,134217728,0,16,37,19,32,0,0,14,4,1,6,6,6448900,0,22605092,0,8388608,0}, \
     {0,0,0,0,0,0,0,0,0,0,1,1,7,2,3,0,1,6,64,64,32,32,0,0,1,0,16,2,37,72,19,40,32,0,1,1,0,1,1,0,0,0,0,0,0,14,4,1,6,6,6448900,0,238609295,0,22605092,0,429496730,0,0,1,715827883,0,67108864,0,8388608,0,134217728,0,134217728,0,16,37,19,32,0,0,14,4,1,6,6,6448900,0,22605092,0,8388608,0}, \
-    {1,0,0,0,0,4,1,0,1,1,1,0,3,1,1,0,6,4,32,32,32,32,1,0,1,1,8,4,10,40,10,40,8,0,1,1,0,0,0,0,0,0,1,0,2,5,6,2,5,6,42949673,0,429496730,0,42949673,0,429496730,0,715827883,0,1073741824,0,134217728,0,16777216,0,134217728,0,268435456,0,8,10,10,8,0,2,5,6,2,5,6,42949673,0,42949673,0,16777216,0}, \
+    {1,0,0,0,0,4,-2,0,1,1,1,0,3,1,1,0,6,4,32,32,32,32,1,0,1,1,8,4,10,40,10,40,8,0,-2,1,0,0,0,0,0,0,1,0,2,5,6,2,5,6,42949673,0,429496730,0,42949673,0,429496730,0,715827883,0,1073741824,0,134217728,0,16777216,0,134217728,0,268435456,0,8,10,10,8,0,2,5,6,2,5,6,42949673,0,42949673,0,16777216,0}, \
     {0,0,0,0,0,0,0,0,1,1,1,0,3,1,1,0,6,4,32,32,32,32,1,0,1,1,16,2,18,40,18,40,16,1,1,1,0,0,0,0,0,1,0,0,1,7,6,1,7,6,23860930,0,429496730,0,23860930,0,429496730,0,715827883,0,1073741824,0,134217728,0,8388608,0,134217728,0,268435456,0,16,18,18,16,1,1,7,6,1,7,6,23860930,0,23860930,0,8388608,0}, \
     {1,0,0,0,0,6,1,0,1,1,1,0,1,1,0,0,10,5,32,32,32,32,1,0,1,0,8,4,8,40,8,40,8,0,1,1,0,0,0,0,0,0,1,0,3,1,6,3,1,6,53687092,0,429496730,0,53687092,0,429496730,0,429496730,0,858993460,0,134217728,0,16777216,0,134217728,0,268435456,0,8,8,8,8,0,3,1,6,3,1,6,53687092,0,53687092,0,16777216,0}, \
     {0,0,0,0,0,0,0,0,1,1,1,0,1,1,0,0,10,5,32,32,32,32,1,0,1,0,8,4,8,40,8,40,8,1,1,1,0,0,0,0,0,0,0,0,3,1,6,3,1,6,53687092,0,429496730,0,53687092,0,429496730,0,429496730,0,858993460,0,134217728,0,16777216,0,134217728,0,268435456,0,8,8,8,8,1,3,1,6,3,1,6,53687092,0,53687092,0,16777216,0}, \
     {1,0,0,0,0,6,0,0,1,1,1,0,3,2,1,0,5,5,32,32,16,16,1,0,1,0,8,2,17,40,9,24,16,0,1,2,0,0,0,0,0,0,1,0,1,8,6,4,6,4,25264514,0,429496730,0,79536432,0,715827883,0,858993460,0,858993460,0,134217728,0,33554432,0,268435456,0,268435456,0,8,17,9,16,0,1,8,6,4,6,4,25264514,0,79536432,0,33554432,0}, \
     {0,0,0,0,0,0,0,0,1,1,1,0,3,2,1,0,5,5,32,32,16,16,1,0,1,0,4,4,9,40,5,24,8,1,1,1,0,0,0,0,1,0,0,0,2,7,6,8,2,4,47721859,0,429496730,0,143165577,0,715827883,0,858993460,0,858993460,0,134217728,0,67108864,0,268435456,0,268435456,0,4,9,5,8,1,2,7,6,8,2,4,47721859,0,143165577,0,67108864,0}, \
-    {1,0,0,0,0,4,1,0,1,1,1,0,3,1,1,0,5,4,16,16,16,16,1,0,1,1,16,1,18,24,18,24,16,0,1,1,0,0,0,0,0,0,1,0,2,6,4,2,6,4,39768216,0,715827883,0,39768216,0,715827883,0,858993460,0,1073741824,0,268435456,0,16777216,0,268435456,0,536870912,0,16,18,18,16,0,2,6,4,2,6,4,39768216,0,39768216,0,16777216,0}, \
+    {1,0,0,0,0,4,-2,0,1,1,1,0,3,1,1,0,5,4,16,16,16,16,1,0,1,1,16,1,18,24,18,24,16,0,-2,1,0,0,0,0,0,0,1,0,2,6,4,2,6,4,39768216,0,715827883,0,39768216,0,715827883,0,858993460,0,1073741824,0,268435456,0,16777216,0,268435456,0,536870912,0,16,18,18,16,0,2,6,4,2,6,4,39768216,0,39768216,0,16777216,0}, \
     {0,0,0,0,0,0,0,0,1,1,1,0,3,1,1,0,5,4,16,16,16,16,1,0,1,1,8,2,10,24,10,24,8,1,1,1,0,0,0,0,1,1,0,0,4,2,4,4,2,4,71582789,0,715827883,0,71582789,0,715827883,0,858993460,0,1073741824,0,268435456,0,33554432,0,268435456,0,536870912,0,8,10,10,8,1,4,2,4,4,2,4,71582789,0,71582789,0,33554432,0}, \
-    {1,0,0,0,0,4,1,0,1,1,1,0,3,1,1,0,9,4,16,16,16,16,1,0,1,1,16,1,18,24,18,24,16,0,1,1,0,0,0,0,0,0,1,0,2,6,4,2,6,4,39768216,0,715827883,0,39768216,0,715827883,0,477218589,0,1073741824,0,268435456,0,16777216,0,268435456,0,536870912,0,16,18,18,16,0,2,6,4,2,6,4,39768216,0,39768216,0,16777216,0}, \
+    {1,0,0,0,0,4,-2,0,1,1,1,0,3,1,1,0,9,4,16,16,16,16,1,0,1,1,16,1,18,24,18,24,16,0,-2,1,0,0,0,0,0,0,1,0,2,6,4,2,6,4,39768216,0,715827883,0,39768216,0,715827883,0,477218589,0,1073741824,0,268435456,0,16777216,0,268435456,0,536870912,0,16,18,18,16,0,2,6,4,2,6,4,39768216,0,39768216,0,16777216,0}, \
     {0,0,0,0,0,0,0,0,1,1,1,0,3,1,1,0,9,4,16,16,16,16,1,0,1,1,8,2,10,24,10,24,8,1,1,1,0,0,0,0,1,1,0,0,4,2,4,4,2,4,71582789,0,715827883,0,71582789,0,715827883,0,477218589,0,1073741824,0,268435456,0,33554432,0,268435456,0,536870912,0,8,10,10,8,1,4,2,4,4,2,4,71582789,0,71582789,0,33554432,0}, \
     {1,0,0,0,0,6,1,0,1,1,1,0,1,1,0,0,13,6,16,16,16,16,1,0,1,0,16,1,16,24,16,24,16,0,1,1,0,0,0,0,0,0,1,0,2,10,4,2,10,4,44739243,0,715827883,0,44739243,0,715827883,0,330382100,0,715827883,0,268435456,0,16777216,0,268435456,0,536870912,0,16,16,16,16,0,2,10,4,2,10,4,44739243,0,44739243,0,16777216,0}, \
     {0,0,0,0,0,0,0,0,1,1,1,0,1,1,0,0,13,6,16,16,16,16,1,0,1,0,8,2,8,24,8,24,8,1,1,1,0,0,0,0,1,1,0,0,5,2,4,5,2,4,89478486,0,715827883,0,89478486,0,715827883,0,330382100,0,715827883,0,268435456,0,33554432,0,268435456,0,536870912,0,8,8,8,8,1,5,2,4,5,2,4,89478486,0,89478486,0,33554432,0}, \
@@ -26,19 +26,19 @@
     {0,0,1,0,0,0,0,0,1,0,1,0,3,1,1,0,1,6,8,8,8,8,0,0,1,0,8,1,10,16,10,16,8,1,1,1,0,0,0,0,1,1,0,0,6,4,0,6,4,0,107374183,0,1073741824,0,107374183,0,1073741824,0,0,1,715827883,0,536870912,0,67108864,0,536870912,0,1073741824,0,4,6,6,4,1,10,4,0,10,4,0,178956971,0,178956971,0,134217728,0}, \
     {0,0,1,0,0,0,0,0,1,1,1,0,3,1,1,0,6,4,8,8,8,8,1,0,1,1,8,1,10,16,10,16,8,1,1,1,0,0,0,0,1,1,0,0,6,4,0,6,4,0,107374183,0,1073741824,0,107374183,0,1073741824,0,715827883,0,1073741824,0,536870912,0,67108864,0,536870912,0,1073741824,0,4,6,6,4,1,10,4,0,10,4,0,178956971,0,178956971,0,134217728,0}, \
     {0,0,1,0,0,0,0,0,1,1,1,0,1,1,0,0,10,5,8,8,8,8,1,0,1,0,8,1,8,16,8,16,8,1,1,1,0,0,0,0,1,1,0,0,8,0,0,8,0,0,134217728,0,1073741824,0,134217728,0,1073741824,0,429496730,0,858993460,0,536870912,0,67108864,0,536870912,0,1073741824,0,4,4,4,4,1,16,0,0,16,0,0,268435456,0,268435456,0,134217728,0}, \
-    {1,0,1,0,0,6,1,0,1,1,1,0,3,1,1,1,5,5,8,8,16,16,1,0,1,0,16,1,11,16,18,24,8,0,1,1,0,0,0,0,0,0,0,0,5,9,0,2,6,4,97612894,0,1073741824,0,39768216,0,715827883,0,858993460,0,858993460,0,536870912,0,16777216,0,268435456,0,1073741824,0,8,7,10,4,0,9,1,0,4,2,4,153391690,0,71582789,0,33554432,0}, \
+    {1,0,1,0,0,6,-2,0,1,1,1,0,3,1,1,1,5,5,8,8,16,16,1,0,1,0,16,1,11,16,18,24,8,0,-2,1,0,0,0,0,0,0,0,0,5,9,0,2,6,4,97612894,0,1073741824,0,39768216,0,715827883,0,858993460,0,858993460,0,536870912,0,16777216,0,268435456,0,1073741824,0,8,7,10,4,0,9,1,0,4,2,4,153391690,0,71582789,0,33554432,0}, \
     {0,0,1,0,0,0,0,1,1,1,1,0,3,1,1,1,5,5,8,8,16,16,1,0,1,0,16,1,11,16,18,24,8,1,1,1,0,0,0,0,1,1,0,0,5,9,0,2,6,4,97612894,0,1073741824,0,39768216,0,715827883,0,858993460,0,858993460,0,536870912,0,16777216,0,268435456,0,1073741824,0,8,7,10,4,1,9,1,0,4,2,4,153391690,0,71582789,0,33554432,0}, \
-    {1,0,1,0,0,4,1,0,1,1,1,0,3,1,1,0,5,4,16,16,16,16,1,0,1,1,16,1,18,24,18,24,16,0,1,1,0,0,0,0,0,0,0,0,2,6,4,2,6,4,39768216,0,715827883,0,39768216,0,715827883,0,858993460,0,1073741824,0,268435456,0,16777216,0,268435456,0,536870912,0,8,10,10,8,0,4,2,4,4,2,4,71582789,0,71582789,0,33554432,0}, \
+    {1,0,1,0,0,4,-2,0,1,1,1,0,3,1,1,0,5,4,16,16,16,16,1,0,1,1,16,1,18,24,18,24,16,0,-2,1,0,0,0,0,0,0,0,0,2,6,4,2,6,4,39768216,0,715827883,0,39768216,0,715827883,0,858993460,0,1073741824,0,268435456,0,16777216,0,268435456,0,536870912,0,8,10,10,8,0,4,2,4,4,2,4,71582789,0,71582789,0,33554432,0}, \
     {0,0,1,0,0,0,0,0,1,1,1,0,3,1,1,0,5,4,16,16,16,16,1,0,1,1,8,2,10,24,10,24,8,1,1,1,0,0,0,0,1,0,0,0,4,2,4,4,2,4,71582789,0,715827883,0,71582789,0,715827883,0,858993460,0,1073741824,0,268435456,0,33554432,0,268435456,0,536870912,0,4,6,6,4,1,7,0,4,7,0,4,119304648,0,119304648,0,67108864,0}, \
-    {1,0,1,0,0,4,1,0,1,1,1,0,3,1,1,0,9,4,16,16,16,16,1,0,1,1,16,1,18,24,18,24,16,0,1,1,0,0,0,0,0,0,0,0,2,6,4,2,6,4,39768216,0,715827883,0,39768216,0,715827883,0,477218589,0,1073741824,0,268435456,0,16777216,0,268435456,0,536870912,0,8,10,10,8,0,4,2,4,4,2,4,71582789,0,71582789,0,33554432,0}, \
+    {1,0,1,0,0,4,-2,0,1,1,1,0,3,1,1,0,9,4,16,16,16,16,1,0,1,1,16,1,18,24,18,24,16,0,-2,1,0,0,0,0,0,0,0,0,2,6,4,2,6,4,39768216,0,715827883,0,39768216,0,715827883,0,477218589,0,1073741824,0,268435456,0,16777216,0,268435456,0,536870912,0,8,10,10,8,0,4,2,4,4,2,4,71582789,0,71582789,0,33554432,0}, \
     {0,0,1,0,0,0,0,0,1,1,1,0,3,1,1,0,9,4,16,16,16,16,1,0,1,1,8,2,10,24,10,24,8,1,1,1,0,0,0,0,1,0,0,0,4,2,4,4,2,4,71582789,0,715827883,0,71582789,0,715827883,0,477218589,0,1073741824,0,268435456,0,33554432,0,268435456,0,536870912,0,4,6,6,4,1,7,0,4,7,0,4,119304648,0,119304648,0,67108864,0}, \
     {1,0,1,0,0,6,1,0,1,1,1,0,1,1,0,0,13,6,16,16,16,16,1,0,1,0,16,1,16,24,16,24,16,0,1,1,0,0,0,0,0,0,0,0,2,10,4,2,10,4,44739243,0,715827883,0,44739243,0,715827883,0,330382100,0,715827883,0,268435456,0,16777216,0,268435456,0,536870912,0,8,8,8,8,0,5,2,4,5,2,4,89478486,0,89478486,0,33554432,0}, \
     {0,0,1,0,0,0,0,0,1,1,1,0,1,1,0,0,13,6,16,16,16,16,1,0,1,0,8,2,8,24,8,24,8,1,1,1,0,0,0,0,1,0,0,0,5,2,4,5,2,4,89478486,0,715827883,0,89478486,0,715827883,0,330382100,0,715827883,0,268435456,0,33554432,0,268435456,0,536870912,0,4,4,4,4,1,10,2,4,10,2,4,178956971,0,178956971,0,67108864,0}, \
     {1,0,1,0,0,6,2,0,1,1,1,0,3,1,1,1,6,6,16,16,32,32,1,0,1,0,16,2,11,24,18,40,8,0,2,1,0,0,0,0,0,0,0,0,3,9,4,1,7,6,65075263,0,715827883,0,23860930,0,429496730,0,715827883,0,715827883,0,268435456,0,8388608,0,134217728,0,536870912,0,8,7,10,4,0,6,0,4,2,5,6,102261127,0,42949673,0,16777216,0}, \
     {0,0,1,0,0,0,0,2,1,1,1,0,3,1,1,1,6,6,16,16,32,32,1,0,1,0,16,2,11,24,18,40,8,0,1,1,0,0,0,1,0,0,0,0,3,9,4,1,7,6,65075263,0,715827883,0,23860930,0,429496730,0,715827883,0,715827883,0,268435456,0,8388608,0,134217728,0,536870912,0,8,7,10,4,1,6,0,4,2,5,6,102261127,0,42949673,0,16777216,0}, \
-    {1,0,1,0,0,4,1,0,1,1,1,0,3,1,1,0,6,4,32,32,32,32,1,0,1,1,8,4,10,40,10,40,8,0,1,1,0,0,0,0,0,0,0,0,2,5,6,2,5,6,42949673,0,429496730,0,42949673,0,429496730,0,715827883,0,1073741824,0,134217728,0,16777216,0,134217728,0,268435456,0,4,6,6,4,0,4,1,6,4,1,6,71582789,0,71582789,0,33554432,0}, \
+    {1,0,1,0,0,4,-2,0,1,1,1,0,3,1,1,0,6,4,32,32,32,32,1,0,1,1,8,4,10,40,10,40,8,0,-2,1,0,0,0,0,0,0,0,0,2,5,6,2,5,6,42949673,0,429496730,0,42949673,0,429496730,0,715827883,0,1073741824,0,134217728,0,16777216,0,134217728,0,268435456,0,4,6,6,4,0,4,1,6,4,1,6,71582789,0,71582789,0,33554432,0}, \
     {0,0,1,0,0,0,0,0,1,1,1,0,3,1,1,0,6,4,32,32,32,32,1,0,1,1,16,2,18,40,18,40,16,1,1,1,0,0,0,0,0,0,0,0,1,7,6,1,7,6,23860930,0,429496730,0,23860930,0,429496730,0,715827883,0,1073741824,0,134217728,0,8388608,0,134217728,0,268435456,0,8,10,10,8,1,2,5,6,2,5,6,42949673,0,42949673,0,16777216,0}, \
-    {1,0,1,0,0,8,1,0,1,1,1,0,3,1,1,0,10,5,32,32,32,32,1,0,1,0,8,4,10,40,10,40,8,0,1,1,0,0,0,0,0,0,0,0,2,5,6,2,5,6,42949673,0,429496730,0,42949673,0,429496730,0,429496730,0,858993460,0,134217728,0,16777216,0,134217728,0,268435456,0,4,6,6,4,0,4,1,6,4,1,6,71582789,0,71582789,0,33554432,0}, \
+    {1,0,1,0,0,8,-2,0,1,1,1,0,3,1,1,0,10,5,32,32,32,32,1,0,1,0,8,4,10,40,10,40,8,0,-2,1,0,0,0,0,0,0,0,0,2,5,6,2,5,6,42949673,0,429496730,0,42949673,0,429496730,0,429496730,0,858993460,0,134217728,0,16777216,0,134217728,0,268435456,0,4,6,6,4,0,4,1,6,4,1,6,71582789,0,71582789,0,33554432,0}, \
     {0,0,1,0,0,0,0,0,1,1,1,0,3,1,1,0,10,5,32,32,32,32,1,0,1,0,8,4,10,40,10,40,8,1,1,1,0,0,0,0,0,0,0,0,2,5,6,2,5,6,42949673,0,429496730,0,42949673,0,429496730,0,429496730,0,858993460,0,134217728,0,16777216,0,134217728,0,268435456,0,4,6,6,4,1,4,1,6,4,1,6,71582789,0,71582789,0,33554432,0}, \
     {1,0,1,0,0,2,4,0,1,0,1,0,3,1,1,1,5,2,32,32,64,64,1,0,1,0,16,4,11,40,18,72,8,0,4,1,0,0,0,0,0,0,0,0,2,3,6,0,14,4,39045158,0,429496730,0,13256072,0,238609295,0,858993460,0,-2147483648,0,134217728,0,4194304,0,67108864,0,268435456,0,8,7,10,4,0,3,4,6,1,4,4,61356676,0,23860930,0,8388608,0}, \
     {0,0,1,0,0,0,0,1,1,0,1,0,3,1,1,1,5,2,32,32,64,64,1,0,1,0,16,4,11,40,18,72,8,1,1,1,0,0,0,0,0,0,0,0,2,3,6,0,14,4,39045158,0,429496730,0,13256072,0,238609295,0,858993460,0,-2147483648,0,134217728,0,4194304,0,67108864,0,268435456,0,8,7,10,4,1,3,4,6,1,4,4,61356676,0,23860930,0,8388608,0}, \
@@ -51,17 +51,17 @@
     {0,0,0,0,0,0,0,0,1,1,1,0,1,1,0,0,10,5,64,64,64,64,1,0,1,0,8,8,8,72,8,72,8,1,1,1,0,0,0,0,0,0,0,0,1,6,4,1,6,4,29826162,0,238609295,0,29826162,0,238609295,0,429496730,0,858993460,0,67108864,0,8388608,0,67108864,0,134217728,0,8,8,8,8,1,1,6,4,1,6,4,29826162,0,29826162,0,8388608,0}, \
     {1,0,0,0,0,6,0,0,1,1,1,0,3,2,1,0,5,5,64,64,32,32,1,0,1,0,4,8,9,72,5,40,8,0,1,2,0,0,0,0,0,0,1,0,1,5,4,5,0,6,26512144,0,238609295,0,85899346,0,429496730,0,858993460,0,858993460,0,67108864,0,33554432,0,134217728,0,134217728,0,4,9,5,8,0,1,5,4,5,0,6,26512144,0,85899346,0,33554432,0}, \
     {0,0,0,0,0,0,0,0,1,1,1,0,3,2,1,0,5,5,64,64,32,32,1,0,1,0,4,8,9,72,5,40,8,1,1,1,0,0,0,0,0,0,0,0,1,5,4,5,0,6,26512144,0,238609295,0,85899346,0,429496730,0,858993460,0,858993460,0,67108864,0,33554432,0,134217728,0,134217728,0,4,9,5,8,1,1,5,4,5,0,6,26512144,0,85899346,0,33554432,0}, \
-    {1,0,0,0,0,4,1,0,1,1,1,0,3,1,1,0,5,4,32,32,32,32,1,0,1,1,8,4,10,40,10,40,8,0,1,1,0,0,0,0,0,0,1,0,2,5,6,2,5,6,42949673,0,429496730,0,42949673,0,429496730,0,858993460,0,1073741824,0,134217728,0,16777216,0,134217728,0,268435456,0,8,10,10,8,0,2,5,6,2,5,6,42949673,0,42949673,0,16777216,0}, \
+    {1,0,0,0,0,4,-2,0,1,1,1,0,3,1,1,0,5,4,32,32,32,32,1,0,1,1,8,4,10,40,10,40,8,0,-2,1,0,0,0,0,0,0,1,0,2,5,6,2,5,6,42949673,0,429496730,0,42949673,0,429496730,0,858993460,0,1073741824,0,134217728,0,16777216,0,134217728,0,268435456,0,8,10,10,8,0,2,5,6,2,5,6,42949673,0,42949673,0,16777216,0}, \
     {0,0,0,0,0,0,0,0,1,1,1,0,3,1,1,0,5,4,32,32,32,32,1,0,1,1,16,2,18,40,18,40,16,1,1,1,0,0,0,0,0,1,0,0,1,7,6,1,7,6,23860930,0,429496730,0,23860930,0,429496730,0,858993460,0,1073741824,0,134217728,0,8388608,0,134217728,0,268435456,0,16,18,18,16,1,1,7,6,1,7,6,23860930,0,23860930,0,8388608,0}, \
-    {1,0,0,0,0,4,1,0,1,1,1,0,3,1,1,0,9,4,32,32,32,32,1,0,1,1,8,4,10,40,10,40,8,0,1,1,0,0,0,0,0,0,1,0,2,5,6,2,5,6,42949673,0,429496730,0,42949673,0,429496730,0,477218589,0,1073741824,0,134217728,0,16777216,0,134217728,0,268435456,0,8,10,10,8,0,2,5,6,2,5,6,42949673,0,42949673,0,16777216,0}, \
+    {1,0,0,0,0,4,-2,0,1,1,1,0,3,1,1,0,9,4,32,32,32,32,1,0,1,1,8,4,10,40,10,40,8,0,-2,1,0,0,0,0,0,0,1,0,2,5,6,2,5,6,42949673,0,429496730,0,42949673,0,429496730,0,477218589,0,1073741824,0,134217728,0,16777216,0,134217728,0,268435456,0,8,10,10,8,0,2,5,6,2,5,6,42949673,0,42949673,0,16777216,0}, \
     {0,0,0,0,0,0,0,0,1,1,1,0,3,1,1,0,9,4,32,32,32,32,1,0,1,1,8,4,10,40,10,40,8,1,1,1,0,0,0,0,0,0,0,0,2,5,6,2,5,6,42949673,0,429496730,0,42949673,0,429496730,0,477218589,0,1073741824,0,134217728,0,16777216,0,134217728,0,268435456,0,8,10,10,8,1,2,5,6,2,5,6,42949673,0,42949673,0,16777216,0}, \
     {1,0,0,0,0,6,1,0,1,1,1,0,1,1,0,0,13,6,32,32,32,32,1,0,1,0,8,4,8,40,8,40,8,0,1,1,0,0,0,0,0,0,1,0,3,1,6,3,1,6,53687092,0,429496730,0,53687092,0,429496730,0,330382100,0,715827883,0,134217728,0,16777216,0,134217728,0,268435456,0,8,8,8,8,0,3,1,6,3,1,6,53687092,0,53687092,0,16777216,0}, \
     {0,0,0,0,0,0,0,0,1,1,1,0,1,1,0,0,13,6,32,32,32,32,1,0,1,0,8,4,8,40,8,40,8,1,1,1,0,0,0,0,0,0,0,0,3,1,6,3,1,6,53687092,0,429496730,0,53687092,0,429496730,0,330382100,0,715827883,0,134217728,0,16777216,0,134217728,0,268435456,0,8,8,8,8,1,3,1,6,3,1,6,53687092,0,53687092,0,16777216,0}, \
     {1,0,0,0,0,6,0,0,1,1,1,0,3,2,1,0,6,6,32,32,16,16,1,0,1,0,8,2,17,40,9,24,16,0,1,2,0,0,0,0,0,0,1,0,1,8,6,4,6,4,25264514,0,429496730,0,79536432,0,715827883,0,715827883,0,715827883,0,134217728,0,33554432,0,268435456,0,268435456,0,8,17,9,16,0,1,8,6,4,6,4,25264514,0,79536432,0,33554432,0}, \
     {0,0,0,0,0,0,0,0,1,1,1,0,3,2,1,0,6,6,32,32,16,16,1,0,1,0,4,4,9,40,5,24,8,1,1,1,0,0,0,0,1,0,0,0,2,7,6,8,2,4,47721859,0,429496730,0,143165577,0,715827883,0,715827883,0,715827883,0,134217728,0,67108864,0,268435456,0,268435456,0,4,9,5,8,1,2,7,6,8,2,4,47721859,0,143165577,0,67108864,0}, \
-    {1,0,0,0,0,4,1,0,1,1,1,0,3,1,1,0,6,4,16,16,16,16,1,0,1,1,16,1,18,24,18,24,16,0,1,1,0,0,0,0,0,0,1,0,2,6,4,2,6,4,39768216,0,715827883,0,39768216,0,715827883,0,715827883,0,1073741824,0,268435456,0,16777216,0,268435456,0,536870912,0,16,18,18,16,0,2,6,4,2,6,4,39768216,0,39768216,0,16777216,0}, \
+    {1,0,0,0,0,4,-2,0,1,1,1,0,3,1,1,0,6,4,16,16,16,16,1,0,1,1,16,1,18,24,18,24,16,0,-2,1,0,0,0,0,0,0,1,0,2,6,4,2,6,4,39768216,0,715827883,0,39768216,0,715827883,0,715827883,0,1073741824,0,268435456,0,16777216,0,268435456,0,536870912,0,16,18,18,16,0,2,6,4,2,6,4,39768216,0,39768216,0,16777216,0}, \
     {0,0,0,0,0,0,0,0,1,1,1,0,3,1,1,0,6,4,16,16,16,16,1,0,1,1,8,2,10,24,10,24,8,1,1,1,0,0,0,0,1,1,0,0,4,2,4,4,2,4,71582789,0,715827883,0,71582789,0,715827883,0,715827883,0,1073741824,0,268435456,0,33554432,0,268435456,0,536870912,0,8,10,10,8,1,4,2,4,4,2,4,71582789,0,71582789,0,33554432,0}, \
-    {1,0,0,0,0,4,1,0,1,1,1,0,3,1,1,0,10,4,16,16,16,16,1,0,1,1,16,1,18,24,18,24,16,0,1,1,0,0,0,0,0,0,1,0,2,6,4,2,6,4,39768216,0,715827883,0,39768216,0,715827883,0,429496730,0,1073741824,0,268435456,0,16777216,0,268435456,0,536870912,0,16,18,18,16,0,2,6,4,2,6,4,39768216,0,39768216,0,16777216,0}, \
+    {1,0,0,0,0,4,-2,0,1,1,1,0,3,1,1,0,10,4,16,16,16,16,1,0,1,1,16,1,18,24,18,24,16,0,-2,1,0,0,0,0,0,0,1,0,2,6,4,2,6,4,39768216,0,715827883,0,39768216,0,715827883,0,429496730,0,1073741824,0,268435456,0,16777216,0,268435456,0,536870912,0,16,18,18,16,0,2,6,4,2,6,4,39768216,0,39768216,0,16777216,0}, \
     {0,0,0,0,0,0,0,0,1,1,1,0,3,1,1,0,10,4,16,16,16,16,1,0,1,1,8,2,10,24,10,24,8,1,1,1,0,0,0,0,1,1,0,0,4,2,4,4,2,4,71582789,0,715827883,0,71582789,0,715827883,0,429496730,0,1073741824,0,268435456,0,33554432,0,268435456,0,536870912,0,8,10,10,8,1,4,2,4,4,2,4,71582789,0,71582789,0,33554432,0}, \
     {1,0,0,0,0,8,1,0,1,1,1,0,1,1,0,0,14,7,16,16,16,16,1,0,1,0,16,1,16,24,16,24,16,0,1,1,0,0,0,0,0,0,1,0,2,10,4,2,10,4,44739243,0,715827883,0,44739243,0,715827883,0,306783379,0,613566757,0,268435456,0,16777216,0,268435456,0,536870912,0,16,16,16,16,0,2,10,4,2,10,4,44739243,0,44739243,0,16777216,0}, \
     {0,0,0,0,0,0,0,0,1,1,1,0,1,1,0,0,14,7,16,16,16,16,1,0,1,0,8,2,8,24,8,24,8,1,1,1,0,0,0,0,1,1,0,0,5,2,4,5,2,4,89478486,0,715827883,0,89478486,0,715827883,0,306783379,0,613566757,0,268435456,0,33554432,0,268435456,0,536870912,0,8,8,8,8,1,5,2,4,5,2,4,89478486,0,89478486,0,33554432,0}, \
@@ -71,7 +71,7 @@
     {0,0,0,0,0,0,0,0,1,1,1,0,3,1,1,0,7,4,8,8,8,8,1,0,1,1,8,1,10,16,10,16,8,1,1,1,0,0,0,0,1,1,0,0,6,4,0,6,4,0,107374183,0,1073741824,0,107374183,0,1073741824,0,613566757,0,1073741824,0,536870912,0,67108864,0,536870912,0,1073741824,0,8,10,10,8,1,6,4,0,6,4,0,107374183,0,107374183,0,67108864,0}, \
     {1,0,0,0,0,6,0,0,1,1,1,0,1,1,0,0,11,5,8,8,8,8,1,0,1,0,8,1,8,16,8,16,8,0,1,4,0,0,0,0,0,0,1,0,8,0,0,8,0,0,134217728,0,1073741824,0,134217728,0,1073741824,0,390451573,0,858993460,0,536870912,0,67108864,0,536870912,0,1073741824,0,8,8,8,8,0,8,0,0,8,0,0,134217728,0,134217728,0,67108864,0}, \
     {0,0,0,0,0,0,0,0,1,1,1,0,1,1,0,0,11,5,8,8,8,8,1,0,1,0,8,1,8,16,8,16,8,1,1,1,0,0,0,0,1,1,0,0,8,0,0,8,0,0,134217728,0,1073741824,0,134217728,0,1073741824,0,390451573,0,858993460,0,536870912,0,67108864,0,536870912,0,1073741824,0,8,8,8,8,1,8,0,0,8,0,0,134217728,0,134217728,0,67108864,0}, \
-    {1,0,1,0,0,4,1,0,1,1,1,0,3,1,1,0,10,4,32,32,32,32,1,0,1,1,8,4,10,40,10,40,8,0,1,1,0,0,0,0,0,0,0,0,2,5,6,2,5,6,42949673,0,429496730,0,42949673,0,429496730,0,429496730,0,1073741824,0,134217728,0,16777216,0,134217728,0,268435456,0,4,6,6,4,0,4,1,6,4,1,6,71582789,0,71582789,0,33554432,0}, \
+    {1,0,1,0,0,4,-2,0,1,1,1,0,3,1,1,0,10,4,32,32,32,32,1,0,1,1,8,4,10,40,10,40,8,0,-2,1,0,0,0,0,0,0,0,0,2,5,6,2,5,6,42949673,0,429496730,0,42949673,0,429496730,0,429496730,0,1073741824,0,134217728,0,16777216,0,134217728,0,268435456,0,4,6,6,4,0,4,1,6,4,1,6,71582789,0,71582789,0,33554432,0}, \
     {0,0,1,0,0,0,0,0,1,1,1,0,3,1,1,0,10,4,32,32,32,32,1,0,1,1,8,4,10,40,10,40,8,1,1,1,0,0,0,0,0,0,0,0,2,5,6,2,5,6,42949673,0,429496730,0,42949673,0,429496730,0,429496730,0,1073741824,0,134217728,0,16777216,0,134217728,0,268435456,0,4,6,6,4,1,4,1,6,4,1,6,71582789,0,71582789,0,33554432,0}, \
     {1,0,1,0,0,8,1,0,1,1,1,0,1,1,0,0,14,7,32,32,32,32,1,0,1,0,8,4,8,40,8,40,8,0,1,1,0,0,0,0,0,0,0,0,3,1,6,3,1,6,53687092,0,429496730,0,53687092,0,429496730,0,306783379,0,613566757,0,134217728,0,16777216,0,134217728,0,268435456,0,4,4,4,4,0,6,1,6,6,1,6,107374183,0,107374183,0,33554432,0}, \
     {0,0,1,0,0,0,0,0,1,1,1,0,1,1,0,0,14,7,32,32,32,32,1,0,1,0,8,4,8,40,8,40,8,1,1,1,0,0,0,0,0,0,0,0,3,1,6,3,1,6,53687092,0,429496730,0,53687092,0,429496730,0,306783379,0,613566757,0,134217728,0,16777216,0,134217728,0,268435456,0,4,4,4,4,1,6,1,6,6,1,6,107374183,0,107374183,0,33554432,0}, \
@@ -100,21 +100,21 @@
     {0,0,0,0,0,0,0,0,1,1,1,0,1,1,0,0,13,6,64,64,64,64,1,0,1,0,8,8,8,72,8,72,8,0,1,1,0,0,0,0,0,0,0,0,1,6,4,1,6,4,29826162,0,238609295,0,29826162,0,238609295,0,330382100,0,715827883,0,67108864,0,8388608,0,67108864,0,134217728,0,8,8,8,8,0,1,6,4,1,6,4,29826162,0,29826162,0,8388608,0}, \
     {1,0,0,0,0,6,0,0,1,1,1,0,3,2,1,0,6,6,64,64,32,32,1,0,1,0,4,8,9,72,5,40,8,0,1,2,0,0,0,0,0,0,1,0,1,5,4,5,0,6,26512144,0,238609295,0,85899346,0,429496730,0,715827883,0,715827883,0,67108864,0,33554432,0,134217728,0,134217728,0,4,9,5,8,0,1,5,4,5,0,6,26512144,0,85899346,0,33554432,0}, \
     {0,0,0,0,0,0,0,0,1,1,1,0,3,2,1,0,6,6,64,64,32,32,1,0,1,0,4,8,9,72,5,40,8,1,1,1,0,0,0,0,0,0,0,0,1,5,4,5,0,6,26512144,0,238609295,0,85899346,0,429496730,0,715827883,0,715827883,0,67108864,0,33554432,0,134217728,0,134217728,0,4,9,5,8,1,1,5,4,5,0,6,26512144,0,85899346,0,33554432,0}, \
-    {1,0,0,0,0,4,1,0,1,1,1,0,3,1,1,0,10,4,32,32,32,32,1,0,1,1,8,4,10,40,10,40,8,0,1,1,0,0,0,0,0,0,1,0,2,5,6,2,5,6,42949673,0,429496730,0,42949673,0,429496730,0,429496730,0,1073741824,0,134217728,0,16777216,0,134217728,0,268435456,0,8,10,10,8,0,2,5,6,2,5,6,42949673,0,42949673,0,16777216,0}, \
+    {1,0,0,0,0,4,-2,0,1,1,1,0,3,1,1,0,10,4,32,32,32,32,1,0,1,1,8,4,10,40,10,40,8,0,-2,1,0,0,0,0,0,0,1,0,2,5,6,2,5,6,42949673,0,429496730,0,42949673,0,429496730,0,429496730,0,1073741824,0,134217728,0,16777216,0,134217728,0,268435456,0,8,10,10,8,0,2,5,6,2,5,6,42949673,0,42949673,0,16777216,0}, \
     {0,0,0,0,0,0,0,0,1,1,1,0,3,1,1,0,10,4,32,32,32,32,1,0,1,1,8,4,10,40,10,40,8,1,1,1,0,0,0,0,0,1,0,0,2,5,6,2,5,6,42949673,0,429496730,0,42949673,0,429496730,0,429496730,0,1073741824,0,134217728,0,16777216,0,134217728,0,268435456,0,8,10,10,8,1,2,5,6,2,5,6,42949673,0,42949673,0,16777216,0}, \
     {1,0,0,0,0,8,1,0,1,1,1,0,1,1,0,0,14,7,32,32,32,32,1,0,1,0,8,4,8,40,8,40,8,0,1,1,0,0,0,0,0,0,1,0,3,1,6,3,1,6,53687092,0,429496730,0,53687092,0,429496730,0,306783379,0,613566757,0,134217728,0,16777216,0,134217728,0,268435456,0,8,8,8,8,0,3,1,6,3,1,6,53687092,0,53687092,0,16777216,0}, \
     {0,0,0,0,0,0,0,0,1,1,1,0,1,1,0,0,14,7,32,32,32,32,1,0,1,0,8,4,8,40,8,40,8,1,1,1,0,0,0,0,0,1,0,0,3,1,6,3,1,6,53687092,0,429496730,0,53687092,0,429496730,0,306783379,0,613566757,0,134217728,0,16777216,0,134217728,0,268435456,0,8,8,8,8,1,3,1,6,3,1,6,53687092,0,53687092,0,16777216,0}, \
     {1,0,0,0,0,8,0,0,1,1,1,0,3,2,1,0,7,7,32,32,16,16,1,0,1,0,8,2,17,40,9,24,16,0,1,2,0,0,0,0,0,0,1,0,1,8,6,4,6,4,25264514,0,429496730,0,79536432,0,715827883,0,613566757,0,613566757,0,134217728,0,33554432,0,268435456,0,268435456,0,8,17,9,16,0,1,8,6,4,6,4,25264514,0,79536432,0,33554432,0}, \
     {0,0,0,0,0,0,0,0,1,1,1,0,3,2,1,0,7,7,32,32,16,16,1,0,1,0,4,4,9,40,5,24,8,1,1,1,0,0,0,0,1,1,0,0,2,7,6,8,2,4,47721859,0,429496730,0,143165577,0,715827883,0,613566757,0,613566757,0,134217728,0,67108864,0,268435456,0,268435456,0,4,9,5,8,1,2,7,6,8,2,4,47721859,0,143165577,0,67108864,0}, \
-    {1,0,0,0,0,4,1,0,1,1,1,0,3,1,1,0,7,4,16,16,16,16,1,0,1,1,16,1,18,24,18,24,16,0,1,1,0,0,0,0,0,0,1,0,2,6,4,2,6,4,39768216,0,715827883,0,39768216,0,715827883,0,613566757,0,1073741824,0,268435456,0,16777216,0,268435456,0,536870912,0,16,18,18,16,0,2,6,4,2,6,4,39768216,0,39768216,0,16777216,0}, \
+    {1,0,0,0,0,4,-2,0,1,1,1,0,3,1,1,0,7,4,16,16,16,16,1,0,1,1,16,1,18,24,18,24,16,0,-2,1,0,0,0,0,0,0,1,0,2,6,4,2,6,4,39768216,0,715827883,0,39768216,0,715827883,0,613566757,0,1073741824,0,268435456,0,16777216,0,268435456,0,536870912,0,16,18,18,16,0,2,6,4,2,6,4,39768216,0,39768216,0,16777216,0}, \
     {0,0,0,0,0,0,0,0,1,1,1,0,3,1,1,0,7,4,16,16,16,16,1,0,1,1,8,2,10,24,10,24,8,1,1,1,0,0,0,0,1,1,0,0,4,2,4,4,2,4,71582789,0,715827883,0,71582789,0,715827883,0,613566757,0,1073741824,0,268435456,0,33554432,0,268435456,0,536870912,0,8,10,10,8,1,4,2,4,4,2,4,71582789,0,71582789,0,33554432,0}, \
-    {1,0,0,0,0,4,1,0,1,1,1,0,3,1,1,0,11,4,16,16,16,16,1,0,1,1,16,1,18,24,18,24,16,0,1,1,0,0,0,0,0,0,1,0,2,6,4,2,6,4,39768216,0,715827883,0,39768216,0,715827883,0,390451573,0,1073741824,0,268435456,0,16777216,0,268435456,0,536870912,0,16,18,18,16,0,2,6,4,2,6,4,39768216,0,39768216,0,16777216,0}, \
+    {1,0,0,0,0,4,-2,0,1,1,1,0,3,1,1,0,11,4,16,16,16,16,1,0,1,1,16,1,18,24,18,24,16,0,-2,1,0,0,0,0,0,0,1,0,2,6,4,2,6,4,39768216,0,715827883,0,39768216,0,715827883,0,390451573,0,1073741824,0,268435456,0,16777216,0,268435456,0,536870912,0,16,18,18,16,0,2,6,4,2,6,4,39768216,0,39768216,0,16777216,0}, \
     {0,0,0,0,0,0,0,0,1,1,1,0,3,1,1,0,11,4,16,16,16,16,1,0,1,1,8,2,10,24,10,24,8,1,1,1,0,0,0,0,0,1,0,0,4,2,4,4,2,4,71582789,0,715827883,0,71582789,0,715827883,0,390451573,0,1073741824,0,268435456,0,33554432,0,268435456,0,536870912,0,8,10,10,8,1,4,2,4,4,2,4,71582789,0,71582789,0,33554432,0}, \
     {1,0,0,0,0,8,1,0,1,1,1,0,1,1,0,0,15,7,16,16,16,16,1,0,1,0,16,1,16,24,16,24,16,0,1,1,0,0,0,0,0,0,1,0,2,10,4,2,10,4,44739243,0,715827883,0,44739243,0,715827883,0,286331154,0,613566757,0,268435456,0,16777216,0,268435456,0,536870912,0,16,16,16,16,0,2,10,4,2,10,4,44739243,0,44739243,0,16777216,0}, \
     {0,0,0,0,0,0,0,0,1,1,1,0,1,1,0,0,15,7,16,16,16,16,1,0,1,0,8,2,8,24,8,24,8,1,1,1,0,0,0,0,1,1,0,0,5,2,4,5,2,4,89478486,0,715827883,0,89478486,0,715827883,0,286331154,0,613566757,0,268435456,0,33554432,0,268435456,0,536870912,0,8,8,8,8,1,5,2,4,5,2,4,89478486,0,89478486,0,33554432,0}, \
     {1,0,0,0,0,8,1,0,1,0,1,0,3,1,1,0,1,6,8,8,8,8,0,0,1,0,8,1,10,16,10,16,8,0,1,1,0,0,0,0,0,0,1,0,6,4,0,6,4,0,107374183,0,1073741824,0,107374183,0,1073741824,0,0,1,715827883,0,536870912,0,67108864,0,536870912,0,1073741824,0,8,10,10,8,0,6,4,0,6,4,0,107374183,0,107374183,0,67108864,0}, \
     {0,0,0,0,0,0,0,0,1,0,1,0,3,1,1,0,1,6,8,8,8,8,0,0,1,0,8,1,10,16,10,16,8,1,1,1,0,0,0,0,1,1,0,0,6,4,0,6,4,0,107374183,0,1073741824,0,107374183,0,1073741824,0,0,1,715827883,0,536870912,0,67108864,0,536870912,0,1073741824,0,8,10,10,8,1,6,4,0,6,4,0,107374183,0,107374183,0,67108864,0}, \
-    {1,0,0,0,0,6,1,0,1,1,1,0,3,1,1,1,5,5,8,8,16,16,1,0,1,0,16,1,11,16,18,24,8,0,1,1,0,0,0,0,0,0,1,0,5,9,0,2,6,4,97612894,0,1073741824,0,39768216,0,715827883,0,858993460,0,858993460,0,536870912,0,16777216,0,268435456,0,1073741824,0,16,11,18,8,0,5,9,0,2,6,4,97612894,0,39768216,0,16777216,0}, \
+    {1,0,0,0,0,6,-2,0,1,1,1,0,3,1,1,1,5,5,8,8,16,16,1,0,1,0,16,1,11,16,18,24,8,0,-2,1,0,0,0,0,0,0,1,0,5,9,0,2,6,4,97612894,0,1073741824,0,39768216,0,715827883,0,858993460,0,858993460,0,536870912,0,16777216,0,268435456,0,1073741824,0,16,11,18,8,0,5,9,0,2,6,4,97612894,0,39768216,0,16777216,0}, \
     {0,0,0,0,0,0,0,1,1,1,1,0,3,1,1,1,5,5,8,8,16,16,1,0,1,0,16,1,11,16,18,24,8,1,1,1,0,0,0,0,1,1,0,0,5,9,0,2,6,4,97612894,0,1073741824,0,39768216,0,715827883,0,858993460,0,858993460,0,536870912,0,16777216,0,268435456,0,1073741824,0,16,11,18,8,1,5,9,0,2,6,4,97612894,0,39768216,0,16777216,0}, \
     {0,0,1,0,0,0,0,0,1,1,1,0,3,1,1,0,5,4,16,16,16,16,1,0,1,1,8,2,10,24,10,24,8,1,1,1,0,0,0,0,1,1,0,0,4,2,4,4,2,4,71582789,0,715827883,0,71582789,0,715827883,0,858993460,0,1073741824,0,268435456,0,33554432,0,268435456,0,536870912,0,4,6,6,4,1,7,0,4,7,0,4,119304648,0,119304648,0,67108864,0}, \
     {0,0,1,0,0,0,0,0,1,1,1,0,3,1,1,0,9,4,16,16,16,16,1,0,1,1,8,2,10,24,10,24,8,1,1,1,0,0,0,0,1,1,0,0,4,2,4,4,2,4,71582789,0,715827883,0,71582789,0,715827883,0,477218589,0,1073741824,0,268435456,0,33554432,0,268435456,0,536870912,0,4,6,6,4,1,7,0,4,7,0,4,119304648,0,119304648,0,67108864,0}, \
```

Measured after the change: 662,600 samples/s, median of 6. 1.0% higher.
